# KTH-RPL/HiMo

Hardware: AMD Instinct MI355X
Metric: lidar_frames_per_sec_120k (higher is better)
Workload: dtype f16x2 (two-term split fp16, x = h + l with exact subnormals, on the matrix cores; float32 accumulate; ~22-bit products); 1 GPU; per-frame pipeline: pillarise 3 sweeps (512x512 grid) -> SeFlow++-style encoder/decoder + GRU head (random-init, self-specified: reference network source absent) -> per-point flow -> ego-motion removal + dt0 + flow2compDis -> comp_dis; points_per_frame=120000, sweeps_per_frame=3, parallelism=frames sharded x1, refined_output=False, batches_in_flight=3, matrix_arithmetic=f16x2, samples_per_backbone_launch=16, collectives=none (single process)

## Files before the change

himo_amd/csrc/pillar.hip:

```cpp
#include "himo_common.h"
#include "bf16x3.h"
#include <math.h>
#include <algorithm>
#include <vector>

namespace himo {

struct GridSpec {
    float xmin, ymin, zmin;
    float vx, vy, vz;
    float cx0, cy0, cz0;
    int W, H;
};

struct PillarArgs {
    int64_t n;
    const float* pts; int stride;
    float R[9], t[3];
    GridSpec g;
    const float* pfn_w;
    const float* pfn_scale;
    const float* pfn_shift;
    float* xyz_t;
    int* pid;
    float* offsets;
    float* image; int image_pitch;
    int image_split;
    int* cell_count;
    int* block_sum;
    int* cell_cursor;
    int* order2;
    float4* cell_rec;
    unsigned long long* occ;
};

constexpr int kMaxSweeps = 12;
struct PillarBatch { PillarArgs s[kMaxSweeps]; };

__global__ __launch_bounds__(256) void pillar_clear_kernel(PillarBatch m, int n_vec4) {
    int4* p = reinterpret_cast<int4*>(m.s[blockIdx.y].cell_count);
    for (int i = blockIdx.x * 256 + threadIdx.x; i < n_vec4; i += gridDim.x * 256) p[i] = make_int4(0, 0, 0, 0);
}

__global__ __launch_bounds__(256) void pillar_assign_kernel(PillarBatch m) {
    const PillarArgs& a = m.s[blockIdx.y];
    const int64_t i = (int64_t)blockIdx.x * 256 + threadIdx.x;
    if (i >= a.n) return;
    const float* p = a.pts + i * a.stride;
    const float x = p[0], y = p[1], z = p[2];
    const float tx = ((x * a.R[0] + y * a.R[1]) + z * a.R[2]) + a.t[0];
    const float ty = ((x * a.R[3] + y * a.R[4]) + z * a.R[5]) + a.t[1];
    const float tz = ((x * a.R[6] + y * a.R[7]) + z * a.R[8]) + a.t[2];
    a.xyz_t[i * 3] = tx; a.xyz_t[i * 3 + 1] = ty; a.xyz_t[i * 3 + 2] = tz;
    const float fx = floorf((tx - a.g.xmin) / a.g.vx);
    const float fy = floorf((ty - a.g.ymin) / a.g.vy);
    const float fz = floorf((tz - a.g.zmin) / a.g.vz);
    const bool ok = fx >= 0.f && fx < (float)a.g.W && fy >= 0.f && fy < (float)a.g.H && fz >= 0.f && fz < 1.f;
    int cell = -1;
    if (ok) {
        cell = (int)fy * a.g.W + (int)fx;
        a.order2[i] = atomicAdd(&a.cell_count[cell], 1);
    } else {
        a.offsets[i * 3] = 0.f; a.offsets[i * 3 + 1] = 0.f; a.offsets[i * 3 + 2] = 0.f;
    }
    a.pid[i] = cell;
}

constexpr int kScanBlock = 1024;

__global__ __launch_bounds__(256) void cell_scan_local_kernel(PillarBatch m) {
    int* v = m.s[blockIdx.y].cell_count;
    int* block_sum = m.s[blockIdx.y].block_sum;
    const int n = m.s[blockIdx.y].g.W * m.s[blockIdx.y].g.H;
    __shared__ int wsum[4];
    const int base = blockIdx.x * kScanBlock + threadIdx.x * 4;
    int x[4];
#pragma unroll
    for (int k = 0; k < 4; ++k) x[k] = base + k < n ? v[base + k] : 0;
    const int mine = x[0] + x[1] + x[2] + x[3];
    int incl = mine;
    const int lane = threadIdx.x & 63;
    for (int off = 1; off < 64; off <<= 1) {
        const int y = __shfl_up(incl, off, 64);
        if (lane >= off) incl += y;
    }
    if (lane == 63) wsum[threadIdx.x >> 6] = incl;
    __syncthreads();
    int run = incl - mine;
    for (int w = 0; w < (int)(threadIdx.x >> 6); ++w) run += wsum[w];
#pragma unroll
    for (int k = 0; k < 4; ++k) { if (base + k < n) v[base + k] = run; run += x[k]; }
    if (threadIdx.x == 255) block_sum[blockIdx.x] = run;
}

__global__ __launch_bounds__(1024) void cell_scan_top_kernel(PillarBatch m, int nblk) {
    int* block_sum = m.s[blockIdx.y].block_sum;
    __shared__ int part[1024];
    const int x = (int)threadIdx.x < nblk ? block_sum[threadIdx.x] : 0;
    part[threadIdx.x] = x;
    __syncthreads();
    for (int off = 1; off < 1024; off <<= 1) {
        const int y = threadIdx.x >= off ? part[threadIdx.x - off] : 0;
        __syncthreads();
        part[threadIdx.x] += y;
        __syncthreads();
    }
    if ((int)threadIdx.x < nblk) block_sum[threadIdx.x] = part[threadIdx.x] - x;
    if (threadIdx.x == 1023) block_sum[nblk] = part[1023];
}

__device__ inline int cell_offset(const PillarArgs& a, int cell);

__device__ inline int cell_offset(const PillarArgs& a, int cell) {
    const int n_cells = a.g.W * a.g.H;
    return cell >= n_cells ? a.block_sum[(n_cells + kScanBlock - 1) / kScanBlock]
                           : a.cell_count[cell] + a.block_sum[cell / kScanBlock];
}

__global__ __launch_bounds__(256) void pillar_fill_kernel(PillarBatch m) {
    const PillarArgs& a = m.s[blockIdx.y];
    const int64_t i = (int64_t)blockIdx.x * 256 + threadIdx.x;
    if (i >= a.n) return;
    const int cell = a.pid[i];
    if (cell < 0) return;
    const int at = cell_offset(a, cell) + a.order2[i];
    a.cell_rec[at] = make_float4(a.xyz_t[i * 3], a.xyz_t[i * 3 + 1], a.xyz_t[i * 3 + 2], __int_as_float((int)i));
}

constexpr int kCellsPerBlock = 8;

constexpr int kFeatCells = 64;

__device__ inline float shfl32(float v, int src) { return __shfl(v, src, 32); }
__device__ inline int shfl32(int v, int src) { return __shfl(v, src, 32); }

__global__ __launch_bounds__(256) void pillar_feature_kernel(PillarBatch m) {
    const PillarArgs& a = m.s[blockIdx.y];
    __shared__ int s_beg[kFeatCells + 1];
    __shared__ int s_list[kFeatCells];
    __shared__ int s_nlist;
    const int sub = threadIdx.x >> 5, c = threadIdx.x & 31;
    const int n_cells = a.g.W * a.g.H;
    const int cell0 = blockIdx.x * kFeatCells;
    static_assert(kFeatCells == 64, "one 64-bit occupancy word per block");
    const unsigned long long was = a.occ ? a.occ[blockIdx.x] : ~0ull;
    if (threadIdx.x <= kFeatCells) s_beg[threadIdx.x] = cell_offset(a, min(cell0 + (int)threadIdx.x, n_cells));
    __syncthreads();
    if (threadIdx.x < 64) {
        const int cnt = cell0 + (int)threadIdx.x < n_cells ? s_beg[threadIdx.x + 1] - s_beg[threadIdx.x] : 0;
        const unsigned long long one = __ballot(cnt == 1), many = __ballot(cnt > 1);
        const unsigned long long below = (1ull << threadIdx.x) - 1ull;
        if (cnt == 1) s_list[__popcll(one & below)] = threadIdx.x;
        if (cnt > 1) s_list[__popcll(one) + __popcll(many & below)] = threadIdx.x;
        if (threadIdx.x == 0) { s_nlist = __popcll(one | many); if (a.occ) a.occ[blockIdx.x] = one | many; }
    }
#pragma unroll
    for (int i = 0; i < kFeatCells / 32; ++i) {
        const int lc = i * 32 + (threadIdx.x >> 3);
        if (cell0 + lc < n_cells && s_beg[lc + 1] == s_beg[lc] && ((was >> lc) & 1ull))
            *reinterpret_cast<float4*>(a.image + (int64_t)(cell0 + lc) * a.image_pitch + (threadIdx.x & 7) * 4) = make_float4(0.f, 0.f, 0.f, 0.f);
    }
    __syncthreads();
    const int nlist = s_nlist;
    float w[9];
#pragma unroll
    for (int k = 0; k < 9; ++k) w[k] = a.pfn_w[k * 32 + c];
    const float scale = a.pfn_scale[c], shift = a.pfn_shift[c];

    for (int k = sub; k < nlist; k += kCellsPerBlock) {
        const int lc = s_list[k];
        const int cell = cell0 + lc;
        const int beg = s_beg[lc];
        const int cnt = s_beg[lc + 1] - beg;
        const int iy = cell / a.g.W, ix = cell - iy * a.g.W;
        const float ccx = (float)ix * a.g.vx + a.g.cx0, ccy = (float)iy * a.g.vy + a.g.cy0, ccz = 0.f * a.g.vz + a.g.cz0;
        const float fc = (float)cnt;
        float acc = 0.f;
        if (cnt == 1) {
            const float4 rc = a.cell_rec[beg];
            const int pj = __float_as_int(rc.w);
            const float x = rc.x, y = rc.y, z = rc.z;
            if (c == 0) a.order2[beg] = pj;
            const float f6[3] = {x - ccx, y - ccy, z - ccz};
            float v = x * w[0];
            v = fmaf(y, w[1], v); v = fmaf(z, w[2], v);
            v = fmaf(x - x, w[3], v); v = fmaf(y - y, w[4], v); v = fmaf(z - z, w[5], v);
            v = fmaf(f6[0], w[6], v); v = fmaf(f6[1], w[7], v); v = fmaf(f6[2], w[8], v);
            v = v * scale + shift;
            acc = 0.f + fmaxf(v, 0.f);
            if (c < 3) a.offsets[(int64_t)pj * 3 + c] = f6[c];
        } else if (cnt <= 32) {
            const bool have = c < cnt;
            const float4 rc = a.cell_rec[beg + (have ? c : 0)];
            const int idx = have ? __float_as_int(rc.w) : 0x7fffffff;
            const float ux = rc.x, uy = rc.y, uz = rc.z;
            int rank = 0;
            for (int j = 0; j < cnt; ++j) rank += shfl32(idx, j) < idx;
            int src = 0;
            for (int j = 0; j < cnt; ++j)
                if (shfl32(rank, j) == c) src = j;
            const int sidx = shfl32(idx, src);
            const float px = shfl32(ux, src), py = shfl32(uy, src), pz = shfl32(uz, src);
            if (have) a.order2[beg + c] = sidx;
            float sx = 0.f, sy = 0.f, sz = 0.f;
            for (int j = 0; j < cnt; ++j) { sx += shfl32(px, j); sy += shfl32(py, j); sz += shfl32(pz, j); }
            const float mx = sx / fc, my = sy / fc, mz = sz / fc;
            for (int j = 0; j < cnt; ++j) {
                const float x = shfl32(px, j), y = shfl32(py, j), z = shfl32(pz, j);
                const int pj = shfl32(sidx, j);
                const float f[9] = {x, y, z, x - mx, y - my, z - mz, x - ccx, y - ccy, z - ccz};
                float v = f[0] * w[0];
#pragma unroll
                for (int q = 1; q < 9; ++q) v = fmaf(f[q], w[q], v);
                v = v * scale + shift;
                acc += fmaxf(v, 0.f);
                if (c < 3) a.offsets[(int64_t)pj * 3 + c] = f[6 + c];
            }
        } else {
            for (int j0 = 0; j0 < cnt; j0 += 32) {
                const bool have = j0 + c < cnt;
                const int idx = have ? __float_as_int(a.cell_rec[beg + j0 + c].w) : 0x7fffffff;
                int rank = 0;
                for (int k0 = 0; k0 < cnt; k0 += 32) {
                    const int other = k0 + c < cnt ? __float_as_int(a.cell_rec[beg + k0 + c].w) : 0x7fffffff;
                    const int lim = min(32, cnt - k0);
                    for (int j = 0; j < lim; ++j) rank += shfl32(other, j) < idx;
                }
                if (have) a.order2[beg + rank] = idx;
            }
            __threadfence_block();
            float sx = 0.f, sy = 0.f, sz = 0.f;
            for (int j0 = 0; j0 < cnt; j0 += 32) {
                const bool have = j0 + c < cnt;
                const float* p = a.xyz_t + (int64_t)(have ? a.order2[beg + j0 + c] : 0) * 3;
                const float ux = have ? p[0] : 0.f, uy = have ? p[1] : 0.f, uz = have ? p[2] : 0.f;
                const int lim = min(32, cnt - j0);
                for (int j = 0; j < lim; ++j) { sx += shfl32(ux, j); sy += shfl32(uy, j); sz += shfl32(uz, j); }
            }
            const float mx = sx / fc, my = sy / fc, mz = sz / fc;
            for (int j0 = 0; j0 < cnt; j0 += 32) {
                const bool have = j0 + c < cnt;
                const int pidx = have ? a.order2[beg + j0 + c] : 0;
                const float* p = a.xyz_t + (int64_t)pidx * 3;
                const float ux = have ? p[0] : 0.f, uy = have ? p[1] : 0.f, uz = have ? p[2] : 0.f;
                const int lim = min(32, cnt - j0);
                for (int j = 0; j < lim; ++j) {
                    const float x = shfl32(ux, j), y = shfl32(uy, j), z = shfl32(uz, j);
                    const int pj = shfl32(pidx, j);
                    const float f[9] = {x, y, z, x - mx, y - my, z - mz, x - ccx, y - ccy, z - ccz};
                    float v = f[0] * w[0];
#pragma unroll
                    for (int q = 1; q < 9; ++q) v = fmaf(f[q], w[q], v);
                    v = v * scale + shift;
                    acc += fmaxf(v, 0.f);
                    if (c < 3) a.offsets[(int64_t)pj * 3 + c] = f[6 + c];
                }
            }
        }
        const float feat = acc / fc;
        if (a.image_split) {
            unsigned h, l;
            split2_rounded(feat, h, l);
            const bool odd = c & 1;
            const unsigned recv = (unsigned)__builtin_amdgcn_mov_dpp((int)(odd ? h : l), 0xB1, 0xF, 0xF, true);
            unsigned* rec = reinterpret_cast<unsigned*>(a.image + (int64_t)cell * a.image_pitch + (c & ~15));
            rec[(odd ? 8 : 0) + ((c & 15) >> 1)] = odd ? (recv | (l << 16)) : (h | (recv << 16));
        } else {
            a.image[(int64_t)cell * a.image_pitch + c] = feat;
        }
    }
}

struct PillarBwdArgs {
    GridSpec g;
    const int* cell_count; const int* block_sum; const int* order2;
    const float4* cell_rec;
    const float* xyz_t;
    const float* pfn_w; const float* pfn_scale; const float* pfn_shift;
    const float* d_image; int image_pitch;
    float* partial;
    const float* dhx; int dhx_pitch;
    float* d_b0; int b0_pitch; int group0, group1, n_groups;
    float* d_dec; int dec_pitch;
};

__device__ inline int cell_offset_b(const PillarBwdArgs& a, int cell) {
    const int n_cells = a.g.W * a.g.H;
    return cell >= n_cells ? a.block_sum[(n_cells + kScanBlock - 1) / kScanBlock]
                           : a.cell_count[cell] + a.block_sum[cell / kScanBlock];
}

__global__ __launch_bounds__(1024) void pfn_backward_reduce_kernel(const float* __restrict__ partial, int n_blocks, float* __restrict__ dw,
                                                                   int accumulate) {
    __shared__ float sh[32][32];
    const int c = threadIdx.x & 31, grp = threadIdx.x >> 5, k = blockIdx.x;
    {
        float t[4] = {0.f, 0.f, 0.f, 0.f};
        int b = grp;
        for (; b + 96 < n_blocks; b += 128) {
#pragma unroll
            for (int q = 0; q < 4; ++q) t[q] += partial[(int64_t)(b + 32 * q) * 288 + k * 32 + c];
        }
        for (; b < n_blocks; b += 32) t[0] += partial[(int64_t)b * 288 + k * 32 + c];
        sh[grp][c] = (t[0] + t[1]) + (t[2] + t[3]);
    }
    __syncthreads();
    if (grp == 0) {
        float r = sh[0][c];
#pragma unroll
        for (int g = 1; g < 32; ++g) r += sh[g][c];
        dw[k * 32 + c] = accumulate ? dw[k * 32 + c] + r : r;
    }
}

struct PfnBnArgs {
    PillarBwdArgs b;
    double* partial;
    const float* mean; const float* invstd;
    const float* coef;
};

struct PfnBnBatch { PfnBnArgs s[kMaxSweeps]; };
template <int KIND>
__global__ __launch_bounds__(256) void pfn_walk_kernel(PfnBnBatch m) {
    const PfnBnArgs& p = m.s[blockIdx.y];
    const PillarBwdArgs& a = p.b;
    constexpr int kChunk = 256;
    __shared__ int s_beg[kChunk + 1];
    __shared__ int s_list[kChunk];
    __shared__ int s_wn[4];
    constexpr bool kStats = KIND < 2;
    __shared__ double red_d[kStats ? 2 : 1][kStats ? kCellsPerBlock : 1][32];
    __shared__ float red_f[kStats ? 1 : kCellsPerBlock][kStats ? 1 : 9][32];
    const int sub = threadIdx.x >> 5, c = threadIdx.x & 31, wv = threadIdx.x >> 6, lane = threadIdx.x & 63;
    const int n_cells = a.g.W * a.g.H;
    float w[9], dw[9];
#pragma unroll
    for (int k = 0; k < 9; ++k) { w[k] = a.pfn_w[k * 32 + c]; dw[k] = 0.f; }
    const float scale = KIND ? a.pfn_scale[c] : 0.f, shift = KIND ? a.pfn_shift[c] : 0.f;
    const float mean = (KIND == 1 || KIND == 2) ? p.mean[c] : 0.f, invstd = (KIND == 1 || KIND == 2) ? p.invstd[c] : 0.f;
    const float k2 = KIND == 2 ? p.coef[c] : 0.f, k3 = KIND == 2 ? p.coef[32 + c] : 0.f;
    double s0 = 0.0, s1 = 0.0;
    for (int cell0 = blockIdx.x * kChunk; cell0 < n_cells; cell0 += gridDim.x * kChunk) {
        s_beg[threadIdx.x] = cell_offset_b(a, min(cell0 + (int)threadIdx.x, n_cells));
        if (threadIdx.x == 0) s_beg[kChunk] = cell_offset_b(a, min(cell0 + kChunk, n_cells));
        __syncthreads();
        const int my_cnt = cell0 + (int)threadIdx.x < n_cells ? s_beg[threadIdx.x + 1] - s_beg[threadIdx.x] : 0;
        const unsigned long long occ = __ballot(my_cnt > 0);
        if (lane == 0) s_wn[wv] = __popcll(occ);
        __syncthreads();
        int base = 0, nlist = 0;
#pragma unroll
        for (int u = 0; u < 4; ++u) { if (u < wv) base += s_wn[u]; nlist += s_wn[u]; }
        if (my_cnt > 0) s_list[base + __popcll(occ & ((1ull << lane) - 1ull))] = threadIdx.x;
        __syncthreads();
        for (int k = sub; k < nlist; k += kCellsPerBlock) {
            const int lc = s_list[k];
            const int cell = cell0 + lc;
            const int beg = s_beg[lc], cnt = s_beg[lc + 1] - beg;
            const float fc = (float)cnt;
            const float gi = KIND ? a.d_image[(int64_t)cell * a.image_pitch + c] / fc : 0.f;
            const int iy = cell / a.g.W, ix = cell - iy * a.g.W;
            const float ccx = (float)ix * a.g.vx + a.g.cx0, ccy = (float)iy * a.g.vy + a.g.cy0, ccz = 0.f * a.g.vz + a.g.cz0;
            auto point = [&](float x, float y, float z, float mx, float my, float mz) {
                const float f[9] = {x, y, z, x - mx, y - my, z - mz, x - ccx, y - ccy, z - ccz};
                float v = f[0] * w[0];
#pragma unroll
                for (int q = 1; q < 9; ++q) v = fmaf(f[q], w[q], v);
                if (KIND == 0) {
                    s0 += v; s1 += (double)v * v;
                } else if (KIND == 1) {
                    const float g = (v * scale + shift) > 0.f ? gi : 0.f;
                    s0 += g; s1 += (double)g * ((v - mean) * invstd);
                } else if (KIND == 2) {
                    const float g = (v * scale + shift) > 0.f ? gi : 0.f;
                    const float dy = scale * ((g - k2) - ((v - mean) * invstd) * k3);
#pragma unroll
                    for (int q = 0; q < 9; ++q) dw[q] += f[q] * dy;
                } else {
                    if ((v * scale + shift) > 0.f) {
                        const float g = gi * scale;
#pragma unroll
                        for (int q = 0; q < 9; ++q) dw[q] += f[q] * g;
                    }
                }
            };
            if (cnt == 1) {
                const float4 rc = a.cell_rec[beg];
                point(rc.x, rc.y, rc.z, rc.x, rc.y, rc.z);
                continue;
            }
            float sx = 0.f, sy = 0.f, sz = 0.f;
            float ux = 0.f, uy = 0.f, uz = 0.f;
            for (int j0 = 0; j0 < cnt; j0 += 32) {
                const bool have = j0 + c < cnt;
                const float* q = a.xyz_t + (int64_t)(have ? a.order2[beg + j0 + c] : 0) * 3;
                ux = have ? q[0] : 0.f; uy = have ? q[1] : 0.f; uz = have ? q[2] : 0.f;
                const int lim = min(32, cnt - j0);
                for (int j = 0; j < lim; ++j) { sx += shfl32(ux, j); sy += shfl32(uy, j); sz += shfl32(uz, j); }
            }
            const float mx = sx / fc, my = sy / fc, mz = sz / fc;
            for (int j0 = 0; j0 < cnt; j0 += 32) {
                if (cnt > 32) {
                    const bool have = j0 + c < cnt;
                    const float* q = a.xyz_t + (int64_t)(have ? a.order2[beg + j0 + c] : 0) * 3;
                    ux = have ? q[0] : 0.f; uy = have ? q[1] : 0.f; uz = have ? q[2] : 0.f;
                }
                const int lim = min(32, cnt - j0);
                for (int j = 0; j < lim; ++j) point(shfl32(ux, j), shfl32(uy, j), shfl32(uz, j), mx, my, mz);
            }
        }
        __syncthreads();
    }
    if (kStats) {
        red_d[0][sub][c] = s0; red_d[1][sub][c] = s1;
        __syncthreads();
        if (threadIdx.x < 64) {
            const int which = threadIdx.x >> 5;
            double t = red_d[which][0][c];
#pragma unroll
            for (int q = 1; q < kCellsPerBlock; ++q) t += red_d[which][q][c];
            p.partial[((int64_t)blockIdx.x * 2 + which) * 32 + c] = t;
        }
    } else {
#pragma unroll
        for (int k = 0; k < 9; ++k) red_f[sub][k][c] = dw[k];
        __syncthreads();
        for (int e = threadIdx.x; e < 9 * 32; e += 256) {
            float t = 0.f;
#pragma unroll
            for (int q = 0; q < kCellsPerBlock; ++q) t += red_f[q][e / 32][e % 32];
            a.partial[(int64_t)blockIdx.x * 288 + e] = t;
        }
    }
}

constexpr int kMaxGroup = 16;
struct PfnGroup { const double* partial[kMaxGroup]; const int* block_sum[kMaxGroup]; int n; };

template <int MODE>
__global__ __launch_bounds__(1024) void pfn_bn_finalize_kernel(PfnGroup grp_src, int n_blocks, int n_cells, const float* __restrict__ gamma,
                                                              const float* __restrict__ beta, float eps, float momentum,
                                                              float* __restrict__ running_mean, float* __restrict__ running_var,
                                                              float* __restrict__ out0, float* __restrict__ out1, float* __restrict__ out2,
                                                              float* __restrict__ out3, int accumulate) {
    __shared__ double sh[2][16][32];
    const int c = threadIdx.x & 31, which = (threadIdx.x >> 5) & 1, grp = threadIdx.x >> 6;
    {
        double all = 0.0;
        for (int m = 0; m < grp_src.n; ++m) {
            const double* __restrict__ partial = grp_src.partial[m];
            double t[4] = {0, 0, 0, 0};
            int b = grp;
            for (; b + 48 < n_blocks; b += 64) {
#pragma unroll
                for (int k = 0; k < 4; ++k) t[k] += partial[((int64_t)(b + 16 * k) * 2 + which) * 32 + c];
            }
            for (; b < n_blocks; b += 16) t[0] += partial[((int64_t)b * 2 + which) * 32 + c];
            all += (t[0] + t[1]) + (t[2] + t[3]);
        }
        sh[which][grp][c] = all;
    }
    __syncthreads();
    if (threadIdx.x >= 32) return;
    double count = 0.0;
    for (int m = 0; m < grp_src.n; ++m) count += (double)grp_src.block_sum[m][(n_cells + kScanBlock - 1) / kScanBlock];
    double a0 = 0.0, a1 = 0.0;
#pragma unroll
    for (int g = 0; g < 16; ++g) { a0 += sh[0][g][c]; a1 += sh[1][g][c]; }
    if (MODE == 0) {
        if (count < 1.0) {
            const float sc = gamma[c] / sqrtf((running_var ? running_var[c] : 1.f) + eps);
            out0[c] = sc; out1[c] = beta[c] - (running_mean ? running_mean[c] : 0.f) * sc; out2[c] = 0.f; out3[c] = 0.f;
            return;
        }
        const double mean = a0 / count;
        double var = a1 / count - mean * mean;
        if (var < 0.0) var = 0.0;
        const float invstd = (float)(1.0 / sqrt(var + (double)eps));
        const float sc = gamma[c] * invstd;
        out0[c] = sc;
        out1[c] = beta[c] - (float)mean * sc;
        out2[c] = (float)mean;
        out3[c] = invstd;
        if (running_mean) {
            const double unbiased = count > 1.0 ? var * count / (count - 1.0) : var;
            running_mean[c] = (float)((1.0 - (double)momentum) * (double)running_mean[c] + (double)momentum * mean);
            running_var[c] = (float)((1.0 - (double)momentum) * (double)running_var[c] + (double)momentum * unbiased);
        }
    } else {
        out0[c] = accumulate ? out0[c] + (float)a1 : (float)a1;
        out1[c] = accumulate ? out1[c] + (float)a0 : (float)a0;
        out2[c] = count > 0.0 ? (float)(a0 / count) : 0.f;
        out3[c] = count > 0.0 ? (float)(a1 / count) : 0.f;
    }
}

__global__ __launch_bounds__(256) void head_scatter_kernel(PillarBwdArgs a) {
    const int sub = threadIdx.x >> 5, c = threadIdx.x & 31;
    const int cell = blockIdx.x * kCellsPerBlock + sub;
    if (cell >= a.g.W * a.g.H) return;
    const int beg = cell_offset_b(a, cell);
    const int cnt = cell_offset_b(a, cell + 1) - beg;
    float s0 = 0.f, s1 = 0.f, s2 = 0.f, s3 = 0.f;
    for (int j = 0; j < cnt; ++j) {
        const float* r = a.dhx + (int64_t)a.order2[beg + j] * a.dhx_pitch;
        s0 += r[c]; s1 += r[32 + c]; s2 += r[64 + c]; s3 += r[96 + c];
    }
    float* b0 = a.d_b0 + (int64_t)cell * a.b0_pitch;
    for (int g = 0; g < a.n_groups; ++g) b0[g * 32 + c] = g == a.group0 ? s0 : g == a.group1 ? s1 : 0.f;
    float* dec = a.d_dec + (int64_t)cell * a.dec_pitch;
    dec[c] = s2; dec[32 + c] = s3;
}

}

using namespace himo;

static size_t ws_cells(int cells) { return round_up((size_t)cells * 4, 16); }
static size_t ws_blocks(int cells) { return round_up(((size_t)(cells + kScanBlock - 1) / kScanBlock + 1) * 4, 16); }
static size_t ws_points(int64_t n) { return round_up((size_t)(n > 0 ? n : 1) * 4, 16); }
static size_t pillar_ws(int64_t n, int cells) { return 2 * ws_cells(cells) + ws_blocks(cells) + 2 * ws_points(n) + 3 * ws_points(n); }
static size_t ws_occ(int cells) { return round_up(((size_t)cells + 63) / 64 * 8, 16); }

constexpr int64_t kMaxCells = (int64_t)kScanBlock * 1024;
static int64_t grid_cells(int grid_w, int grid_h) { return (int64_t)grid_w * (int64_t)grid_h; }
static int grid_status(int grid_w, int grid_h) {
    if (grid_w < 1 || grid_h < 1) return HIMO_ERR_INVALID_ARGUMENT;
    return grid_cells(grid_w, grid_h) > kMaxCells ? HIMO_ERR_UNSUPPORTED : HIMO_OK;
}

extern "C" size_t himo_pillar_workspace_bytes(int64_t max_points, int grid_w, int grid_h) {
    if (max_points < 0 || max_points > 0x7fffffff || grid_status(grid_w, grid_h) != HIMO_OK) return 0;
    const int cells = (int)grid_cells(grid_w, grid_h);
    return pillar_ws(max_points, cells) + 64 + ws_occ(cells);
}

extern "C" int himo_pillar_occupancy_reset(void* d_workspace, size_t workspace_bytes, int grid_w, int grid_h, void* stream) {
    if (!d_workspace || grid_w < 1 || grid_h < 1) return HIMO_ERR_INVALID_ARGUMENT;
    if (grid_status(grid_w, grid_h) != HIMO_OK) return HIMO_ERR_UNSUPPORTED;
    const int cells = (int)grid_cells(grid_w, grid_h);
    if (workspace_bytes < ws_occ(cells)) return HIMO_ERR_INVALID_ARGUMENT;
    const size_t nb = ws_occ(cells);
    HIMO_HIP(hipMemsetAsync(reinterpret_cast<char*>(d_workspace) + (workspace_bytes - nb), 0xFF, nb, (hipStream_t)stream));
    return HIMO_OK;
}

static int pillar_args(PillarArgs& a, int64_t n, const float* d_pts, int pc_stride, const float* h_transform, const float* h_range,
                       const float* h_voxel, const float* h_centre_offset, int grid_w, int grid_h, const float* d_pfn_weight,
                       const float* d_pfn_scale, const float* d_pfn_shift, float* d_xyz_t, int32_t* d_pid, float* d_offsets,
                       float* d_image, int image_pitch, void* d_workspace, size_t workspace_bytes, bool incremental = false) {
    if (n < 0 || pc_stride < 3 || grid_w < 1 || grid_h < 1 || !h_transform || !h_range || !h_voxel || !h_centre_offset)
        return HIMO_ERR_INVALID_ARGUMENT;
    if (!d_pfn_weight || !d_pfn_scale || !d_pfn_shift || !d_image || !d_workspace) return HIMO_ERR_INVALID_ARGUMENT;
    if (n > 0 && (!d_pts || !d_xyz_t || !d_pid || !d_offsets)) return HIMO_ERR_INVALID_ARGUMENT;
    if (n > 0x7fffffff || image_pitch < 32) return HIMO_ERR_UNSUPPORTED;
    if ((image_pitch & 3) || (reinterpret_cast<uintptr_t>(d_image) & 15)) return HIMO_ERR_UNSUPPORTED;
    if (grid_cells(grid_w, grid_h) > kMaxCells) return HIMO_ERR_UNSUPPORTED;
    const int cells = (int)grid_cells(grid_w, grid_h);
    if (workspace_bytes < pillar_ws(n, cells) || !aligned16(d_workspace)) return HIMO_ERR_WORKSPACE;
    if (incremental && ((workspace_bytes & 15) || workspace_bytes < pillar_ws(n, cells) + ws_occ(cells))) return HIMO_ERR_WORKSPACE;
    a = PillarArgs{};
    a.n = n; a.pts = d_pts; a.stride = pc_stride;
    for (int i = 0; i < 9; ++i) a.R[i] = h_transform[(i / 3) * 4 + (i % 3)];
    for (int i = 0; i < 3; ++i) a.t[i] = h_transform[i * 4 + 3];
    a.g.xmin = h_range[0]; a.g.ymin = h_range[1]; a.g.zmin = h_range[2];
    a.g.vx = h_voxel[0]; a.g.vy = h_voxel[1]; a.g.vz = h_voxel[2];
    a.g.cx0 = h_centre_offset[0]; a.g.cy0 = h_centre_offset[1]; a.g.cz0 = h_centre_offset[2];
    a.g.W = grid_w; a.g.H = grid_h;
    a.pfn_w = d_pfn_weight; a.pfn_scale = d_pfn_scale; a.pfn_shift = d_pfn_shift;
    a.xyz_t = d_xyz_t; a.pid = d_pid; a.offsets = d_offsets; a.image = d_image; a.image_pitch = image_pitch;
    char* ws = reinterpret_cast<char*>(d_workspace);
    a.cell_count = reinterpret_cast<int*>(ws);
    a.cell_cursor = reinterpret_cast<int*>(ws + ws_cells(cells));
    a.block_sum = reinterpret_cast<int*>(ws + 2 * ws_cells(cells));
    a.cell_rec = reinterpret_cast<float4*>(ws + 2 * ws_cells(cells) + ws_blocks(cells));
    a.order2 = reinterpret_cast<int*>(ws + 2 * ws_cells(cells) + ws_blocks(cells) + 4 * ws_points(n));
    if (incremental) a.occ = reinterpret_cast<unsigned long long*>(ws + (workspace_bytes - ws_occ(cells)));
    return HIMO_OK;
}

static int sweeps_status(int n_sweeps, const himo_sweep* h_sweeps, int image_pitch, int image_split, bool check_shared) {
    if (n_sweeps < 1 || n_sweeps > kMaxSweeps || !h_sweeps) return HIMO_ERR_INVALID_ARGUMENT;
    if (image_split && (image_pitch & 15)) return HIMO_ERR_INVALID_ARGUMENT;
    for (int i = 0; i < n_sweeps; ++i) {
        if (image_split && (reinterpret_cast<uintptr_t>(h_sweeps[i].d_image) & 63)) return HIMO_ERR_INVALID_ARGUMENT;
        for (int j = 0; check_shared && j < i; ++j)
            if (h_sweeps[j].d_workspace == h_sweeps[i].d_workspace) return HIMO_ERR_INVALID_ARGUMENT;
    }
    return HIMO_OK;
}

static int pillar_launch(const PillarBatch& m, int count, hipStream_t s) {
    const int cells = m.s[0].g.W * m.s[0].g.H;
    const int nblk = (cells + kScanBlock - 1) / kScanBlock;
    int64_t nmax = 0;
    for (int i = 0; i < count; ++i)
        if (m.s[i].n > nmax) nmax = m.s[i].n;
    {
        const int n_vec4 = (int)(ws_cells(cells) / 16);
        hipLaunchKernelGGL(pillar_clear_kernel, dim3(std::min((n_vec4 + 255) / 256, 512), count), dim3(256), 0, s, m, n_vec4);
    }
    HIMO_LAUNCH_CHECK("pillar_clear_kernel");
    const unsigned pblocks = (unsigned)((nmax + 255) / 256);
    if (nmax > 0) {
        ProfScope ps("pillar_assign_kernel", s);
        hipLaunchKernelGGL(pillar_assign_kernel, dim3(pblocks, count), dim3(256), 0, s, m);
    }
    HIMO_LAUNCH_CHECK("pillar_assign_kernel");
    {
        ProfScope ps("cell_scan_kernels", s);
        hipLaunchKernelGGL(cell_scan_local_kernel, dim3(nblk, count), dim3(256), 0, s, m);
        hipLaunchKernelGGL(cell_scan_top_kernel, dim3(1, count), dim3(1024), 0, s, m, nblk);
    }
    HIMO_LAUNCH_CHECK("cell_scan_kernels");
    if (nmax > 0) {
        ProfScope ps("pillar_fill_kernel", s);
        hipLaunchKernelGGL(pillar_fill_kernel, dim3(pblocks, count), dim3(256), 0, s, m);
    }
    HIMO_LAUNCH_CHECK("pillar_fill_kernel");
    {
        ProfScope ps("pillar_feature_kernel", s);
        hipLaunchKernelGGL(pillar_feature_kernel, dim3((cells + kFeatCells - 1) / kFeatCells, count), dim3(256), 0, s, m);
    }
    HIMO_LAUNCH_CHECK("pillar_feature_kernel");
    return HIMO_OK;
}

extern "C" int himo_pillarize(int64_t n, const float* d_pts, int pc_stride, const float* h_transform,
                              const float* h_range, const float* h_voxel, const float* h_centre_offset,
                              int grid_w, int grid_h,
                              const float* d_pfn_weight, const float* d_pfn_scale, const float* d_pfn_shift,
                              float* d_xyz_t, int32_t* d_pid, float* d_offsets, float* d_image, int image_pitch,
                              void* d_workspace, size_t workspace_bytes, void* stream) {
    PillarBatch m{};
    const int st = pillar_args(m.s[0], n, d_pts, pc_stride, h_transform, h_range, h_voxel, h_centre_offset, grid_w, grid_h, d_pfn_weight,
                               d_pfn_scale, d_pfn_shift, d_xyz_t, d_pid, d_offsets, d_image, image_pitch, d_workspace, workspace_bytes);
    if (st != HIMO_OK) return st;
    return pillar_launch(m, 1, (hipStream_t)stream);
}

extern "C" int himo_pillarize_multi(int n_sweeps, const himo_sweep* h_sweeps, const float* h_range, const float* h_voxel,
                                    const float* h_centre_offset, int grid_w, int grid_h, const float* d_pfn_weight,
                                    const float* d_pfn_scale, const float* d_pfn_shift, int image_pitch, size_t workspace_bytes,
                                    void* stream) {
    return himo_pillarize_multi_ex(n_sweeps, h_sweeps, h_range, h_voxel, h_centre_offset, grid_w, grid_h, d_pfn_weight, d_pfn_scale,
                                   d_pfn_shift, image_pitch, workspace_bytes, 0, stream);
}

extern "C" int himo_pillarize_multi_ex(int n_sweeps, const himo_sweep* h_sweeps, const float* h_range, const float* h_voxel,
                                       const float* h_centre_offset, int grid_w, int grid_h, const float* d_pfn_weight,
                                       const float* d_pfn_scale, const float* d_pfn_shift, int image_pitch, size_t workspace_bytes,
                                       int image_split, void* stream) {
    const bool incremental = (image_split & 2) != 0;
    image_split &= 1;
    const int st0 = sweeps_status(n_sweeps, h_sweeps, image_pitch, image_split, true);
    if (st0 != HIMO_OK) return st0;
    PillarBatch m{};
    for (int i = 0; i < n_sweeps; ++i) {
        const himo_sweep& w = h_sweeps[i];
        const int st = pillar_args(m.s[i], w.n, w.d_pts, w.pc_stride, w.transform, h_range, h_voxel, h_centre_offset, grid_w, grid_h,
                                   d_pfn_weight, d_pfn_scale, d_pfn_shift, w.d_xyz_t, w.d_pid, w.d_offsets, w.d_image, image_pitch,
                                   w.d_workspace, workspace_bytes, incremental);
        if (st != HIMO_OK) return st;
        m.s[i].image_split = image_split ? 1 : 0;
    }
    return pillar_launch(m, n_sweeps, (hipStream_t)stream);
}

static void carve_bwd(PillarBwdArgs& a, int64_t n, int cells, void* d_workspace) {
    char* ws = reinterpret_cast<char*>(d_workspace);
    a.cell_count = reinterpret_cast<const int*>(ws);
    a.block_sum = reinterpret_cast<const int*>(ws + 2 * ws_cells(cells));
    a.cell_rec = reinterpret_cast<const float4*>(ws + 2 * ws_cells(cells) + ws_blocks(cells));
    a.order2 = reinterpret_cast<const int*>(ws + 2 * ws_cells(cells) + ws_blocks(cells) + 4 * ws_points(n));
}

constexpr int kPfnBwdBlocks = 1024;

extern "C" size_t himo_pfn_backward_workspace_bytes(void) { return (size_t)kPfnBwdBlocks * 288 * 4 + 64; }

extern "C" int himo_pfn_backward(int64_t n, const float* h_voxel, const float* h_centre_offset, int grid_w, int grid_h,
                                 const float* d_pfn_weight, const float* d_pfn_scale, const float* d_pfn_shift,
                                 const float* d_xyz_t, const void* d_pillar_workspace, const float* d_dimage, int image_pitch,
                                 float* d_dweight, unsigned flags, void* d_workspace, size_t workspace_bytes, void* stream) {
    if (n < 0 || !h_voxel || !h_centre_offset || grid_w < 1 || grid_h < 1 || !d_pfn_weight || !d_pfn_scale || !d_pfn_shift ||
        !d_pillar_workspace || !d_dimage || !d_dweight || !d_workspace || image_pitch < 32)
        return HIMO_ERR_INVALID_ARGUMENT;
    if (n > 0 && !d_xyz_t) return HIMO_ERR_INVALID_ARGUMENT;
    if (n > 0x7fffffff || grid_status(grid_w, grid_h) != HIMO_OK) return HIMO_ERR_UNSUPPORTED;
    if (workspace_bytes < himo_pfn_backward_workspace_bytes()) return HIMO_ERR_WORKSPACE;
    PillarBwdArgs a{};
    a.g.vx = h_voxel[0]; a.g.vy = h_voxel[1]; a.g.vz = h_voxel[2];
    a.g.cx0 = h_centre_offset[0]; a.g.cy0 = h_centre_offset[1]; a.g.cz0 = h_centre_offset[2];
    a.g.W = grid_w; a.g.H = grid_h;
    carve_bwd(a, n, grid_w * grid_h, const_cast<void*>(d_pillar_workspace));
    a.xyz_t = d_xyz_t; a.pfn_w = d_pfn_weight; a.pfn_scale = d_pfn_scale; a.pfn_shift = d_pfn_shift;
    a.d_image = d_dimage; a.image_pitch = image_pitch;
    a.partial = reinterpret_cast<float*>(d_workspace);
    hipStream_t s = (hipStream_t)stream;
    {
        ProfScope ps("pfn_backward_kernel", s);
        PfnBnBatch m{};
        m.s[0].b = a;
        hipLaunchKernelGGL(pfn_walk_kernel<3>, dim3(kPfnBwdBlocks), dim3(256), 0, s, m);
    }
    hipLaunchKernelGGL(pfn_backward_reduce_kernel, dim3(9), dim3(1024), 0, s, a.partial, kPfnBwdBlocks, d_dweight, (flags & 1u) ? 1 : 0);
    HIMO_LAUNCH_CHECK("pfn_backward kernels");
    return HIMO_OK;
}

extern "C" size_t himo_pfn_bn_workspace_bytes(void) {
    return round_up((size_t)kPfnBwdBlocks * 288 * 4, 64) + (size_t)kPfnBwdBlocks * 2 * 32 * sizeof(double) + 64 * sizeof(float) + 64;
}

static int pfn_bn_args(PfnBnArgs& p, int64_t n, const float* h_voxel, const float* h_centre_offset, int grid_w, int grid_h,
                       const float* d_pfn_weight, const float* d_xyz_t, const void* d_pillar_workspace, void* d_workspace,
                       size_t workspace_bytes) {
    if (n < 0 || !h_voxel || !h_centre_offset || grid_w < 1 || grid_h < 1 || !d_pfn_weight || !d_pillar_workspace || !d_workspace)
        return HIMO_ERR_INVALID_ARGUMENT;
    if (n > 0 && !d_xyz_t) return HIMO_ERR_INVALID_ARGUMENT;
    if (n > 0x7fffffff || grid_status(grid_w, grid_h) != HIMO_OK) return HIMO_ERR_UNSUPPORTED;
    if (workspace_bytes < himo_pfn_bn_workspace_bytes() || !aligned16(d_workspace)) return HIMO_ERR_WORKSPACE;
    p = PfnBnArgs{};
    PillarBwdArgs& a = p.b;
    a.g.vx = h_voxel[0]; a.g.vy = h_voxel[1]; a.g.vz = h_voxel[2];
    a.g.cx0 = h_centre_offset[0]; a.g.cy0 = h_centre_offset[1]; a.g.cz0 = h_centre_offset[2];
    a.g.W = grid_w; a.g.H = grid_h;
    carve_bwd(a, n, grid_w * grid_h, const_cast<void*>(d_pillar_workspace));
    a.xyz_t = d_xyz_t; a.pfn_w = d_pfn_weight;
    a.partial = reinterpret_cast<float*>(d_workspace);
    p.partial = reinterpret_cast<double*>(reinterpret_cast<char*>(d_workspace) + round_up((size_t)kPfnBwdBlocks * 288 * 4, 64));
    return HIMO_OK;
}

extern "C" int himo_pfn_bn_stats_groups(int n_sweeps, int n_groups, const int64_t* h_n, const float* const* h_xyz_t,
                                        const void* const* h_pillar_workspace, const float* h_voxel, const float* h_centre_offset, int grid_w,
                                        int grid_h, const float* d_pfn_weight, const float* d_gamma, const float* d_beta, float eps,
                                        float momentum, float* d_running_mean, float* d_running_var, float* d_scale, float* d_shift,
                                        float* d_mean, float* d_invstd, void* d_workspace, size_t workspace_bytes, void* stream) {
    if (n_sweeps < 1 || n_groups < 1 || n_sweeps % n_groups || n_sweeps / n_groups > kMaxGroup || !h_n || !h_xyz_t || !h_pillar_workspace)
        return HIMO_ERR_INVALID_ARGUMENT;
    if (!d_gamma || !d_beta || !d_scale || !d_shift || !d_mean || !d_invstd || (d_running_mean == nullptr) != (d_running_var == nullptr))
        return HIMO_ERR_INVALID_ARGUMENT;
    if (grid_w < 1 || grid_h < 1) return HIMO_ERR_INVALID_ARGUMENT;
    if (n_groups > kMaxSweeps * kMaxGroup || grid_status(grid_w, grid_h) != HIMO_OK) return HIMO_ERR_UNSUPPORTED;
    const size_t one = himo_pfn_bn_workspace_bytes();
    if (workspace_bytes < one * n_sweeps) return HIMO_ERR_WORKSPACE;
    std::vector<PfnBnArgs> args((size_t)n_sweeps);
    PfnGroup groups[kMaxSweeps * kMaxGroup];
    for (int g = 0; g < n_groups; ++g) groups[g].n = 0;
    for (int i = 0; i < n_sweeps; ++i) {
        const int st = pfn_bn_args(args[i], h_n[i], h_voxel, h_centre_offset, grid_w, grid_h, d_pfn_weight, h_xyz_t[i], h_pillar_workspace[i],
                                   reinterpret_cast<char*>(d_workspace) + one * i, one);
        if (st != HIMO_OK) return st;
        PfnGroup& G = groups[i % n_groups];
        G.partial[G.n] = args[i].partial; G.block_sum[G.n] = args[i].b.block_sum; ++G.n;
    }
    hipStream_t s = (hipStream_t)stream;
    ProfScope ps("pfn_bn_stats_kernel", s);
    for (int lo = 0; lo < n_sweeps; lo += kMaxSweeps) {
        const int cnt = n_sweeps - lo < kMaxSweeps ? n_sweeps - lo : kMaxSweeps;
        PfnBnBatch m{};
        for (int j = 0; j < cnt; ++j) m.s[j] = args[lo + j];
        hipLaunchKernelGGL(pfn_walk_kernel<0>, dim3(kPfnBwdBlocks, cnt), dim3(256), 0, s, m);
    }
    for (int g = 0; g < n_groups; ++g)
        hipLaunchKernelGGL(pfn_bn_finalize_kernel<0>, dim3(1), dim3(1024), 0, s, groups[g], kPfnBwdBlocks, grid_w * grid_h, d_gamma, d_beta, eps,
                           momentum, d_running_mean, d_running_var, d_scale + 32 * g, d_shift + 32 * g, d_mean + 32 * g, d_invstd + 32 * g, 0);
    HIMO_LAUNCH_CHECK("pfn_bn_stats kernels");
    return HIMO_OK;
}

extern "C" int himo_pfn_bn_stats_multi(int n_sweeps, const int64_t* h_n, const float* const* h_xyz_t, const void* const* h_pillar_workspace,
                                       const float* h_voxel, const float* h_centre_offset, int grid_w, int grid_h,
                                       const float* d_pfn_weight, const float* d_gamma, const float* d_beta, float eps, float momentum,
                                       float* d_running_mean, float* d_running_var, float* d_scale, float* d_shift, float* d_mean,
                                       float* d_invstd, void* d_workspace, size_t workspace_bytes, void* stream) {
    if (n_sweeps > kMaxSweeps) return HIMO_ERR_INVALID_ARGUMENT;
    return himo_pfn_bn_stats_groups(n_sweeps, n_sweeps, h_n, h_xyz_t, h_pillar_workspace, h_voxel, h_centre_offset, grid_w, grid_h, d_pfn_weight,
                                    d_gamma, d_beta, eps, momentum, d_running_mean, d_running_var, d_scale, d_shift, d_mean, d_invstd,
                                    d_workspace, workspace_bytes, stream);
}

extern "C" int himo_pfn_bn_stats(int64_t n, const float* h_voxel, const float* h_centre_offset, int grid_w, int grid_h,
                                 const float* d_pfn_weight, const float* d_xyz_t, const void* d_pillar_workspace, const float* d_gamma,
                                 const float* d_beta, float eps, float momentum, float* d_running_mean, float* d_running_var,
                                 float* d_scale, float* d_shift, float* d_mean, float* d_invstd, void* d_workspace, size_t workspace_bytes,
                                 void* stream) {
    return himo_pfn_bn_stats_multi(1, &n, &d_xyz_t, &d_pillar_workspace, h_voxel, h_centre_offset, grid_w, grid_h, d_pfn_weight, d_gamma,
                                   d_beta, eps, momentum, d_running_mean, d_running_var, d_scale, d_shift, d_mean, d_invstd, d_workspace,
                                   workspace_bytes, stream);
}

extern "C" int himo_pillar_features_multi(int n_sweeps, const himo_sweep* h_sweeps, const float* h_range, const float* h_voxel,
                                          const float* h_centre_offset, int grid_w, int grid_h, const float* d_pfn_weight,
                                          const float* d_scale, const float* d_shift, int image_pitch, size_t workspace_bytes,
                                          int image_split, void* stream) {
    const bool incremental = (image_split & 2) != 0;
    image_split &= 1;
    if (!d_scale || !d_shift) return HIMO_ERR_INVALID_ARGUMENT;
    const int st0 = sweeps_status(n_sweeps, h_sweeps, image_pitch, image_split, false);
    if (st0 != HIMO_OK) return st0;
    PillarBatch m{};
    for (int i = 0; i < n_sweeps; ++i) {
        const himo_sweep& w = h_sweeps[i];
        const int st = pillar_args(m.s[i], w.n, w.d_pts, w.pc_stride, w.transform, h_range, h_voxel, h_centre_offset, grid_w, grid_h,
                                   d_pfn_weight, d_scale + 32 * i, d_shift + 32 * i, w.d_xyz_t, w.d_pid, w.d_offsets, w.d_image, image_pitch,
                                   w.d_workspace, workspace_bytes, incremental);
        if (st != HIMO_OK) return st;
        m.s[i].image_split = image_split ? 1 : 0;
    }
    hipStream_t s = (hipStream_t)stream;
    const int cells = grid_w * grid_h;
    {
        ProfScope ps("pillar_feature_kernel", s);
        hipLaunchKernelGGL(pillar_feature_kernel, dim3((cells + kFeatCells - 1) / kFeatCells, n_sweeps), dim3(256), 0, s, m);
    }
    HIMO_LAUNCH_CHECK("pillar_feature_kernel");
    return HIMO_OK;
}

extern "C" int himo_pfn_backward_bn_groups(int n_sweeps, int n_groups, const int64_t* h_n, const float* const* h_xyz_t,
                                           const void* const* h_pillar_workspace, const float* const* h_dimage, int image_pitch,
                                           const float* h_voxel, const float* h_centre_offset, int grid_w, int grid_h, const float* d_pfn_weight,
                                           const float* d_scale, const float* d_shift, const float* d_mean, const float* d_invstd,
                                           float* d_dweight, float* d_dgamma, float* d_dbeta, unsigned flags, void* d_workspace,
                                           size_t workspace_bytes, void* stream) {
    if (n_sweeps < 1 || n_groups < 1 || n_sweeps % n_groups || n_sweeps / n_groups > kMaxGroup || n_groups > kMaxSweeps * kMaxGroup ||
        n_sweeps > kMaxSweeps * kMaxGroup || !h_n || !h_xyz_t || !h_pillar_workspace || !h_dimage)
        return HIMO_ERR_INVALID_ARGUMENT;
    if (!d_scale || !d_shift || !d_mean || !d_invstd || !d_dweight || !d_dgamma || !d_dbeta || image_pitch < 32) return HIMO_ERR_INVALID_ARGUMENT;
    if (grid_w < 1 || grid_h < 1) return HIMO_ERR_INVALID_ARGUMENT;
    if (grid_status(grid_w, grid_h) != HIMO_OK) return HIMO_ERR_UNSUPPORTED;
    const size_t one = himo_pfn_bn_workspace_bytes();
    if (workspace_bytes < one * n_sweeps) return HIMO_ERR_WORKSPACE;
    static thread_local PfnBnArgs args[kMaxSweeps * kMaxGroup];
    PfnGroup groups[kMaxSweeps * kMaxGroup];
    for (int g = 0; g < n_groups; ++g) groups[g].n = 0;
    for (int i = 0; i < n_sweeps; ++i) {
        if (!h_dimage[i]) return HIMO_ERR_INVALID_ARGUMENT;
        PfnBnArgs& p = args[i];
        const int st = pfn_bn_args(p, h_n[i], h_voxel, h_centre_offset, grid_w, grid_h, d_pfn_weight, h_xyz_t[i], h_pillar_workspace[i],
                                   reinterpret_cast<char*>(d_workspace) + one * i, one);
        if (st != HIMO_OK) return st;
        const int g = i % n_groups;
        p.b.pfn_scale = d_scale + 32 * g; p.b.pfn_shift = d_shift + 32 * g; p.b.d_image = h_dimage[i]; p.b.image_pitch = image_pitch;
        p.mean = d_mean + 32 * g; p.invstd = d_invstd + 32 * g;
        p.coef = i < n_groups ? reinterpret_cast<float*>(p.partial + (size_t)kPfnBwdBlocks * 2 * 32) : args[g].coef;
        PfnGroup& G = groups[g];
        G.partial[G.n] = p.partial; G.block_sum[G.n] = p.b.block_sum; ++G.n;
    }
    hipStream_t s = (hipStream_t)stream;
    ProfScope ps("pfn_backward_kernel", s);
    auto walk = [&](auto kernel) {
        for (int lo = 0; lo < n_sweeps; lo += kMaxSweeps) {
            const int cnt = n_sweeps - lo < kMaxSweeps ? n_sweeps - lo : kMaxSweeps;
            PfnBnBatch m{};
            for (int j = 0; j < cnt; ++j) m.s[j] = args[lo + j];
            hipLaunchKernelGGL(kernel, dim3(kPfnBwdBlocks, cnt), dim3(256), 0, s, m);
        }
    };
    walk(pfn_walk_kernel<1>);
    for (int g = 0; g < n_groups; ++g) {
        float* coef = const_cast<float*>(args[g].coef);
        hipLaunchKernelGGL(pfn_bn_finalize_kernel<1>, dim3(1), dim3(1024), 0, s, groups[g], kPfnBwdBlocks, grid_w * grid_h, (const float*)nullptr,
                           (const float*)nullptr, 0.f, 0.f, (float*)nullptr, (float*)nullptr, d_dgamma, d_dbeta, coef, coef + 32,
                           (g > 0 || (flags & 1u)) ? 1 : 0);
    }
    walk(pfn_walk_kernel<2>);
    for (int i = 0; i < n_sweeps; ++i)
        hipLaunchKernelGGL(pfn_backward_reduce_kernel, dim3(9), dim3(1024), 0, s, args[i].b.partial, kPfnBwdBlocks, d_dweight,
                           (i > 0 || (flags & 1u)) ? 1 : 0);
    HIMO_LAUNCH_CHECK("pfn_backward_bn kernels");
    return HIMO_OK;
}

extern "C" int himo_pfn_backward_bn_multi(int n_sweeps, const int64_t* h_n, const float* const* h_xyz_t, const void* const* h_pillar_workspace,
                                          const float* const* h_dimage, int image_pitch, const float* h_voxel, const float* h_centre_offset,
                                          int grid_w, int grid_h, const float* d_pfn_weight, const float* d_scale, const float* d_shift,
                                          const float* d_mean, const float* d_invstd, float* d_dweight, float* d_dgamma, float* d_dbeta,
                                          unsigned flags, void* d_workspace, size_t workspace_bytes, void* stream) {
    if (n_sweeps > kMaxSweeps) return HIMO_ERR_INVALID_ARGUMENT;
    return himo_pfn_backward_bn_groups(n_sweeps, n_sweeps, h_n, h_xyz_t, h_pillar_workspace, h_dimage, image_pitch, h_voxel, h_centre_offset,
                                       grid_w, grid_h, d_pfn_weight, d_scale, d_shift, d_mean, d_invstd, d_dweight, d_dgamma, d_dbeta, flags,
                                       d_workspace, workspace_bytes, stream);
}

extern "C" int himo_pfn_backward_bn(int64_t n, const float* h_voxel, const float* h_centre_offset, int grid_w, int grid_h,
                                    const float* d_pfn_weight, const float* d_scale, const float* d_shift, const float* d_mean,
                                    const float* d_invstd, const float* d_xyz_t, const void* d_pillar_workspace, const float* d_dimage,
                                    int image_pitch, float* d_dweight, float* d_dgamma, float* d_dbeta, unsigned flags, void* d_workspace,
                                    size_t workspace_bytes, void* stream) {
    return himo_pfn_backward_bn_multi(1, &n, &d_xyz_t, &d_pillar_workspace, &d_dimage, image_pitch, h_voxel, h_centre_offset, grid_w, grid_h,
                                      d_pfn_weight, d_scale, d_shift, d_mean, d_invstd, d_dweight, d_dgamma, d_dbeta, flags, d_workspace,
                                      workspace_bytes, stream);
}

extern "C" int himo_head_scatter(int64_t n, int grid_w, int grid_h, const void* d_pillar_workspace, const float* d_dhx, int dhx_pitch,
                                 float* d_db0, int b0_pitch, int group0, int group1, int n_groups, float* d_ddec, int dec_pitch,
                                 void* stream) {
    if (n < 0 || grid_w < 1 || grid_h < 1 || !d_pillar_workspace || !d_db0 || !d_ddec || dhx_pitch < 128 || n_groups < 1 ||
        b0_pitch < 32 * n_groups || dec_pitch < 64 || (n > 0 && !d_dhx))
        return HIMO_ERR_INVALID_ARGUMENT;
    if (group0 < 0 || group0 >= n_groups || group1 < 0 || group1 >= n_groups || group0 == group1) return HIMO_ERR_INVALID_ARGUMENT;
    if (n > 0x7fffffff || grid_status(grid_w, grid_h) != HIMO_OK) return HIMO_ERR_UNSUPPORTED;
    PillarBwdArgs a{};
    a.g.W = grid_w; a.g.H = grid_h;
    carve_bwd(a, n, grid_w * grid_h, const_cast<void*>(d_pillar_workspace));
    a.dhx = d_dhx; a.dhx_pitch = dhx_pitch; a.d_b0 = d_db0; a.b0_pitch = b0_pitch; a.group0 = group0; a.group1 = group1;
    a.n_groups = n_groups; a.d_dec = d_ddec; a.dec_pitch = dec_pitch;
    hipStream_t s = (hipStream_t)stream;
    ProfScope ps("head_scatter_kernel", s);
    hipLaunchKernelGGL(head_scatter_kernel, dim3((grid_w * grid_h + kCellsPerBlock - 1) / kCellsPerBlock), dim3(256), 0, s, a);
    HIMO_LAUNCH_CHECK("head_scatter_kernel");
    return HIMO_OK;
}
```

himo_amd/seflow/model.py:

```python
from __future__ import annotations

import ctypes

import numpy as np
import torch

from .. import _lib
from . import spec

EPI_BIAS, EPI_BIAS_BN_GELU, EPI_BIAS_GELU, EPI_GRU_ZR, EPI_GRU_Q = range(5)


class ConvDesc(ctypes.Structure):
    _fields_ = [("x", ctypes.c_void_p), ("x_batch_stride", ctypes.c_int64), ("x_pitch", ctypes.c_int),
                ("w", ctypes.c_void_p), ("bias", ctypes.c_void_p), ("scale", ctypes.c_void_p), ("shift", ctypes.c_void_p),
                ("y", ctypes.c_void_p), ("y_batch_stride", ctypes.c_int64), ("y_pitch", ctypes.c_int),
                ("n", ctypes.c_int), ("h", ctypes.c_int), ("w_in", ctypes.c_int), ("cin", ctypes.c_int),
                ("cout", ctypes.c_int), ("ksize", ctypes.c_int), ("stride", ctypes.c_int), ("epilogue", ctypes.c_int),
                ("aux_in", ctypes.c_void_p), ("aux_in_pitch", ctypes.c_int),
                ("aux_out", ctypes.c_void_p), ("aux_out_pitch", ctypes.c_int), ("w_packed", ctypes.c_void_p),
                ("tile_hint", ctypes.c_int), ("packed_format", ctypes.c_int),
                ("n_outer", ctypes.c_int), ("x_outer_stride", ctypes.c_int64), ("y_outer_stride", ctypes.c_int64),
                ("act_layout", ctypes.c_int), ("range_seen", ctypes.c_void_p)]


ACT_SPLIT_IN, ACT_SPLIT_OUT = 1, 2
ACT_ACCUMULATE = 8
ACT_STUFFED_2X = 16


_lib.register({
    "himo_pillar_workspace_bytes": (ctypes.c_size_t, [ctypes.c_int64, ctypes.c_int, ctypes.c_int]),
    "himo_pillar_occupancy_reset": (ctypes.c_int, [ctypes.c_void_p, ctypes.c_size_t, ctypes.c_int, ctypes.c_int, ctypes.c_void_p]),
    "himo_pillarize": (ctypes.c_int, [ctypes.c_int64, ctypes.c_void_p, ctypes.c_int, ctypes.POINTER(ctypes.c_float),
                                      ctypes.POINTER(ctypes.c_float), ctypes.POINTER(ctypes.c_float),
                                      ctypes.POINTER(ctypes.c_float), ctypes.c_int, ctypes.c_int,
                                      ctypes.c_void_p, ctypes.c_void_p, ctypes.c_void_p,
                                      ctypes.c_void_p, ctypes.c_void_p, ctypes.c_void_p, ctypes.c_void_p,
                                      ctypes.c_int, ctypes.c_void_p, ctypes.c_size_t, ctypes.c_void_p]),
    "himo_conv2d": (ctypes.c_int, [ctypes.POINTER(ConvDesc), ctypes.c_void_p]),
    "himo_conv_packed_weight_bytes": (ctypes.c_size_t, [ctypes.c_int, ctypes.c_int, ctypes.c_int]),
    "himo_conv_pack_weights": (ctypes.c_int, [ctypes.c_void_p, ctypes.c_int, ctypes.c_int, ctypes.c_int, ctypes.c_void_p,
                                              ctypes.c_void_p]),
    "himo_upsample2x": (ctypes.c_int, [ctypes.c_void_p, ctypes.c_int, ctypes.c_int, ctypes.c_int, ctypes.c_int,
                                       ctypes.c_void_p, ctypes.c_int, ctypes.c_void_p]),
    "himo_upsample2x_batch": (ctypes.c_int, [ctypes.c_int, ctypes.c_void_p, ctypes.c_int64, ctypes.c_int, ctypes.c_int, ctypes.c_int,
                                             ctypes.c_int, ctypes.c_void_p, ctypes.c_int64, ctypes.c_int, ctypes.c_void_p]),
    "himo_upsample2x_batch_ex": (ctypes.c_int, [ctypes.c_int, ctypes.c_void_p, ctypes.c_int64, ctypes.c_int, ctypes.c_int, ctypes.c_int,
                                                ctypes.c_int, ctypes.c_void_p, ctypes.c_int64, ctypes.c_int, ctypes.c_int, ctypes.c_void_p]),
    "himo_conv_pack_weights_ex": (ctypes.c_int, [ctypes.c_void_p, ctypes.c_int, ctypes.c_int, ctypes.c_int, ctypes.c_int, ctypes.c_void_p,
                                                 ctypes.c_void_p]),
    "himo_gru_head": (ctypes.c_int, [ctypes.c_int64] + [ctypes.c_void_p] * 4 + [ctypes.c_int, ctypes.c_void_p, ctypes.c_int]
                      + [ctypes.c_void_p] * 12 + [ctypes.c_int, ctypes.c_void_p, ctypes.c_int, ctypes.c_int, ctypes.c_void_p]),
    "himo_gru_head_batch": (ctypes.c_int, [ctypes.c_int, ctypes.c_void_p, ctypes.c_int, ctypes.c_int] + [ctypes.c_void_p] * 10
                            + [ctypes.c_int, ctypes.c_int, ctypes.c_int, ctypes.c_void_p]),
    "himo_gru_head_batch_folded": (ctypes.c_int, [ctypes.c_int, ctypes.c_void_p, ctypes.c_int, ctypes.c_int] + [ctypes.c_void_p] * 8
                                   + [ctypes.c_int, ctypes.c_int, ctypes.c_int, ctypes.c_void_p]),
    "himo_gru_head_batch_guarded": (ctypes.c_int, [ctypes.c_int, ctypes.c_void_p, ctypes.c_int, ctypes.c_int] + [ctypes.c_void_p] * 10
                                    + [ctypes.c_int, ctypes.c_int, ctypes.c_int, ctypes.c_void_p, ctypes.c_void_p]),
    "himo_clear_u32": (ctypes.c_int, [ctypes.c_void_p, ctypes.c_int, ctypes.c_void_p]),
    "himo_head_gather": (ctypes.c_int, [ctypes.c_int64, ctypes.c_void_p, ctypes.c_void_p, ctypes.c_void_p, ctypes.c_void_p,
                                        ctypes.c_int, ctypes.c_void_p, ctypes.c_int, ctypes.c_void_p, ctypes.c_void_p,
                                        ctypes.c_void_p, ctypes.c_void_p, ctypes.c_int, ctypes.c_void_p]),
    "himo_head_final": (ctypes.c_int, [ctypes.c_int64, ctypes.c_void_p, ctypes.c_int, ctypes.c_void_p, ctypes.c_void_p,
                                       ctypes.c_void_p, ctypes.c_void_p, ctypes.c_void_p, ctypes.c_int, ctypes.c_void_p,
                                       ctypes.c_void_p]),
})


class HimoHeadSample(ctypes.Structure):
    _fields_ = [("n", ctypes.c_int64), ("d_pid", ctypes.c_void_p), ("d_offsets", ctypes.c_void_p), ("d_img0", ctypes.c_void_p),
                ("d_img1", ctypes.c_void_p), ("d_dec", ctypes.c_void_p), ("d_xyz_t", ctypes.c_void_p), ("d_pts", ctypes.c_void_p),
                ("pc_stride", ctypes.c_int), ("d_flow", ctypes.c_void_p)]


class HimoSweep(ctypes.Structure):
    _fields_ = [("n", ctypes.c_int64), ("d_pts", ctypes.c_void_p), ("pc_stride", ctypes.c_int), ("transform", ctypes.c_float * 16),
                ("d_xyz_t", ctypes.c_void_p), ("d_pid", ctypes.c_void_p), ("d_offsets", ctypes.c_void_p), ("d_image", ctypes.c_void_p),
                ("d_workspace", ctypes.c_void_p)]


class HimoOp(ctypes.Structure):
    _fields_ = [("kind", ctypes.c_int), ("conv", ConvDesc),
                ("up_x", ctypes.c_void_p), ("up_x_pitch", ctypes.c_int), ("up_h", ctypes.c_int), ("up_w", ctypes.c_int),
                ("up_c", ctypes.c_int), ("up_y", ctypes.c_void_p), ("up_y_pitch", ctypes.c_int),
                ("up_n", ctypes.c_int), ("up_x_batch_stride", ctypes.c_int64), ("up_y_batch_stride", ctypes.c_int64),
                ("up_out_split", ctypes.c_int)]


_lib.register({
    "himo_pillarize_multi": (ctypes.c_int, [ctypes.c_int, ctypes.c_void_p, ctypes.c_void_p, ctypes.c_void_p, ctypes.c_void_p, ctypes.c_int,
                                            ctypes.c_int, ctypes.c_void_p, ctypes.c_void_p, ctypes.c_void_p, ctypes.c_int, ctypes.c_size_t,
                                            ctypes.c_void_p]),
    "himo_pillarize_multi_ex": (ctypes.c_int, [ctypes.c_int, ctypes.c_void_p, ctypes.c_void_p, ctypes.c_void_p, ctypes.c_void_p, ctypes.c_int,
                                               ctypes.c_int, ctypes.c_void_p, ctypes.c_void_p, ctypes.c_void_p, ctypes.c_int, ctypes.c_size_t,
                                               ctypes.c_int, ctypes.c_void_p]),
    "himo_run_ops": (ctypes.c_int, [ctypes.c_void_p, ctypes.c_int, ctypes.c_uint, ctypes.c_void_p]),
    "himo_ops_release": (None, [ctypes.c_void_p]),
})


def _f32x(values):
    return (ctypes.c_float * len(values))(*[float(v) for v in values])


def fastest_tile_hint(lib, d: "ConvDesc", hints, warmup: int) -> int:
    stream = _lib.stream_handle()
    times = {}
    for _round in range(2):
        for hint in hints:
            d.tile_hint = hint
            if lib.himo_conv2d(ctypes.byref(d), stream) != 0:
                continue
            for _ in range(warmup - 1):
                lib.himo_conv2d(ctypes.byref(d), stream)
            e0, e1 = torch.cuda.Event(enable_timing=True), torch.cuda.Event(enable_timing=True)
            e0.record()
            for _ in range(3):
                lib.himo_conv2d(ctypes.byref(d), stream)
            e1.record()
            e1.synchronize()
            times[hint] = min(times.get(hint, float("inf")), e0.elapsed_time(e1))
    return min(times, key=times.get) if times else 0


class SeFlowNet:

    def __init__(self, params: dict | None = None, device=None, max_points: int = 140_000, seed: int = 0,
                 precision: str = "bf16x3", autotune: bool = True, max_batch: int = 1):
        if precision not in ("bf16x3", "f16x2", "f32"):
            raise ValueError(precision)
        if max_batch < 1:
            raise ValueError("max_batch")
        self.max_batch = max_batch
        self.precision = precision
        self.autotune = autotune
        self.keep_cell_lists = False
        self.fused_head = precision != "f32"
        self._incremental_images = True
        self.use_plan = True
        self.use_graph = True
        self._plans = {}
        self._recording = None
        self._nb = 1
        self.packed_format = 1 if precision == "f16x2" else 0
        self._split_acts = precision == "f16x2"
        self.tiles = {}
        self.lib = _lib.load()
        self.device = device if device is not None else _lib.require_gpu()
        params = spec.init_params(seed) if params is None else params
        shapes = spec.param_shapes()
        for k, shp in shapes.items():
            if k not in params or tuple(params[k].shape) != tuple(shp):
                raise KeyError(f"parameter {k} missing or of wrong shape (want {shp})")
        cpu = {k: torch.from_numpy(np.ascontiguousarray(params[k], dtype=np.float32)) for k in shapes}
        def fold(prefix, eps):
            scale = cpu[f"{prefix}.gamma"] / torch.sqrt(cpu[f"{prefix}.var"] + eps)
            return scale, cpu[f"{prefix}.beta"] - cpu[f"{prefix}.mean"] * scale
        derived = {}
        derived["pfn.scale"], derived["pfn.shift"] = fold("pfn.bn", spec.BN_EPS_PFN)
        for name, *_ in spec.ENCODER:
            derived[f"{name}.scale"], derived[f"{name}.shift"] = fold(f"{name}.bn", spec.BN_EPS)
        self.fold_decoder = True
        for a, b in (("dec1", "dec2"), ("dec2", "dec3")):
            w5, b5 = cpu[f"{a}.u5.weight"].double().numpy(), cpu[f"{a}.u5.bias"].double().numpy()
            w1, b1 = cpu[f"{b}.u1.weight"].double().numpy()[0, 0], cpu[f"{b}.u1.bias"].double().numpy()
            derived[f"{a}.u5>{b}.u1.weight"] = torch.from_numpy(np.ascontiguousarray(w5 @ w1, dtype=np.float32))
            derived[f"{a}.u5>{b}.u1.bias"] = torch.from_numpy(np.ascontiguousarray(b5 @ w1 + b1, dtype=np.float32))
        derived["head.gru.zr.weight"] = torch.cat([cpu["head.gru.z.weight"], cpu["head.gru.r.weight"]], dim=1).contiguous()
        derived["head.gru.zr.bias"] = torch.cat([cpu["head.gru.z.bias"], cpu["head.gru.r.bias"]]).contiguous()
        self.p = {k: v.to(self.device) for k, v in {**cpu, **derived}.items()}
        self.packed = {}
        if precision != "f32":
            for k, v in self.p.items():
                if k.endswith(".weight") and k != "pfn.weight" and not k.startswith("head.offset") and k != "head.dec2.weight":
                    w = v if v.dim() == 4 else v.reshape(1, 1, *v.shape)
                    ks, _, cin, cout = w.shape
                    fmt = self.packed_format
                    buf = torch.empty(int(self.lib.himo_conv_packed_weight_bytes(ks, cin, cout)), dtype=torch.uint8, device=self.device)
                    _lib.check(self.lib.himo_conv_pack_weights_ex(w.contiguous().data_ptr(), ks, cin, cout, fmt, buf.data_ptr(),
                                                                  _lib.stream_handle()), "himo_conv_pack_weights_ex")
                    self.packed[k] = buf

        self.fold_head = precision != "f32"
        if self.fold_head:
            w_off, b_off = cpu["head.offset.weight"].double().numpy(), cpu["head.offset.bias"].double().numpy()
            for name in ("head.gru.zr", "head.gru.q", "head.dec1"):
                wfull = (derived if name.endswith("zr") else cpu)[f"{name}.weight"].double().numpy()
                wh, wx = wfull[:spec.HIDDEN], wfull[spec.HIDDEN:]
                folded = np.concatenate([wh, w_off @ wx, (b_off @ wx)[None], np.zeros((12, wfull.shape[1]))], axis=0)
                wdev = torch.from_numpy(np.ascontiguousarray(folded, dtype=np.float32)).to(self.device)
                buf = torch.empty(int(self.lib.himo_conv_packed_weight_bytes(1, 144, wdev.shape[1])), dtype=torch.uint8, device=self.device)
                _lib.check(self.lib.himo_conv_pack_weights_ex(wdev.data_ptr(), 1, 144, wdev.shape[1], self.packed_format, buf.data_ptr(),
                                                              _lib.stream_handle()), "himo_conv_pack_weights_ex")
                torch.cuda.synchronize(self.device)
                self.packed[f"{name}.weight.h"] = buf

        H, W = spec.GRID
        F = spec.NUM_FRAMES
        self.H, self.W, self.F = H, W, F
        dev = self.device
        B = self.max_batch
        buf = lambda *shape: torch.empty((B, *shape), dtype=torch.float32, device=dev)
        self._B0 = buf(H * W, 32 * F)
        self.E1 = [buf(F, (H // 2) * (W // 2), 64) for _ in range(2)]
        self.F1 = buf((H // 2) * (W // 2), 64 * F)
        self.E2 = [buf(F, (H // 4) * (W // 4), 128) for _ in range(2)]
        self.F2 = buf((H // 4) * (W // 4), 128 * F)
        self.E3 = [buf(F, (H // 8) * (W // 8), 256) for _ in range(2)]
        self.F3 = buf((H // 8) * (W // 8), 256 * F)
        self.T1 = buf((H // 8) * (W // 8), 256)
        self.CAT1 = buf((H // 4) * (W // 4), 512)
        self.S = [buf((H // 4) * (W // 4), 256) for _ in range(2)]
        self.T2 = buf((H // 4) * (W // 4), 128)
        self.CAT2 = buf((H // 2) * (W // 2), 256)
        self.T = [buf((H // 2) * (W // 2), 128) for _ in range(2)]
        self.T3 = buf((H // 2) * (W // 2), 64)
        self.CAT3 = buf(H * W, 128)
        self.U = [buf(H * W, 64) for _ in range(2)]
        self.DEC = buf(H * W, 64)
        self.max_points = 0
        self._reserve_points(max_points)
        self.guard = torch.zeros(2 + self.MAX_RANGE_SLOTS, dtype=torch.int32, device=dev)
        self.nonfinite = self.guard[:1]
        self._ran_word = self.guard[-1:]
        self._range_slots = {}
        self._range = _f32x(spec.POINT_CLOUD_RANGE[:3])
        self._voxel = _f32x(spec.VOXEL_SIZE)
        r, v = spec.POINT_CLOUD_RANGE, spec.VOXEL_SIZE
        self._centre = _f32x([v[0] / 2 + r[0], v[1] / 2 + r[1], v[2] / 2 + r[2]])

    def _reserve_points(self, n: int):
        if n <= self.max_points:
            return
        dev = self.device
        self.max_points = n
        need = int(self.lib.himo_pillar_workspace_bytes(n, self.W, self.H))
        self._pt = [{"ws_slots": [torch.empty(need + 64, dtype=torch.uint8, device=dev) for _ in range(self.F)],
                     "xyz_t": torch.empty((self.F, n, 3), dtype=torch.float32, device=dev),
                     "pid": torch.empty((self.F, n), dtype=torch.int32, device=dev),
                     "offsets": torch.empty((self.F, n, 3), dtype=torch.float32, device=dev)} for _ in range(self.max_batch)]
        for st in self._pt:
            for ws in st["ws_slots"]:
                _lib.check(self.lib.himo_pillar_occupancy_reset(ws.data_ptr(), ws.numel(), self.W, self.H, _lib.stream_handle()),
                           "himo_pillar_occupancy_reset")
        self._use_sample(0)
        self.hx = torch.empty((n, 192), dtype=torch.float32, device=dev)
        self.rhx = torch.empty((n, 192), dtype=torch.float32, device=dev)
        self.zbuf = torch.empty((n, 128), dtype=torch.float32, device=dev)
        self.y1 = torch.empty((n, 32), dtype=torch.float32, device=dev)

    @property
    def incremental_images(self) -> bool:
        return self._incremental_images

    @incremental_images.setter
    def incremental_images(self, on: bool):
        on = bool(on)
        if on != self._incremental_images:
            self._incremental_images = on
            self.reset_images()

    @property
    def split_acts(self) -> bool:
        return self._split_acts

    @split_acts.setter
    def split_acts(self, on: bool):
        on = bool(on)
        if on != self._split_acts:
            self._split_acts = on
            self.drop_plan()
            self.reset_images()

    @property
    def B0(self):
        return self._B0

    @B0.setter
    def B0(self, buf):
        self._B0 = buf
        self.drop_plan()
        self.reset_images()

    MAX_RANGE_SLOTS = 63

    def clear_nonfinite(self):
        _lib.check(self.lib.himo_clear_u32(self.guard.data_ptr(), self.guard.numel(), _lib.stream_handle()), "himo_clear_u32")

    def _range_word(self, wname: str) -> int:
        k = self._range_slots.setdefault(wname, len(self._range_slots))
        if k >= self.MAX_RANGE_SLOTS:
            raise RuntimeError("more split-output layers than guard words")
        return self.guard.data_ptr() + 4 * (1 + k)

    def guard_verdict(self, words) -> str | None:
        w = [int(v) for v in words]
        if w[0] != 0:
            return "overflow"
        if w[-1] != 0 and any(w[1 + k] == 0 for k in self._range_slots.values()):
            return "underflow"
        return None

    def reset_images(self):
        for st in getattr(self, "_pt", ()):
            for ws in st["ws_slots"]:
                _lib.check(self.lib.himo_pillar_occupancy_reset(ws.data_ptr(), ws.numel(), self.W, self.H, _lib.stream_handle()),
                           "himo_pillar_occupancy_reset")

    def _use_sample(self, i: int):
        st = self._pt[i]
        self._sample = i
        self.ws_slots, self.xyz_t, self.pid, self.offsets = st["ws_slots"], st["xyz_t"], st["pid"], st["offsets"]

    def _conv(self, x, x_bs, x_pitch, wname, y, y_bs, y_pitch, n, h, w, cin, cout, ks, stride, epi, x_off=0, y_off=0,
              scale=None, shift=None, aux_in=None, aux_in_pitch=0, aux_out=None, aux_out_pitch=0, bias=None, batched=True,
              act=0):
        d = ConvDesc()
        d.x = x.data_ptr() + 4 * x_off; d.x_batch_stride = x_bs; d.x_pitch = x_pitch
        if batched and self._nb > 1:
            d.n_outer, d.x_outer_stride, d.y_outer_stride = self._nb, x.stride(0), y.stride(0)
        d.w = self.p[f"{wname}.weight"].data_ptr()
        d.bias = (self.p[f"{wname}.bias"] if bias is None else bias).data_ptr()
        d.scale = None if scale is None else scale.data_ptr()
        d.shift = None if shift is None else shift.data_ptr()
        d.y = y.data_ptr() + 4 * y_off; d.y_batch_stride = y_bs; d.y_pitch = y_pitch
        d.n, d.h, d.w_in, d.cin, d.cout, d.ksize, d.stride, d.epilogue = n, h, w, cin, cout, ks, stride, epi
        d.aux_in = None if aux_in is None else aux_in.data_ptr(); d.aux_in_pitch = aux_in_pitch
        d.aux_out = None if aux_out is None else aux_out.data_ptr(); d.aux_out_pitch = aux_out_pitch
        pk = self.packed.get(f"{wname}.weight")
        d.w_packed = None if pk is None else pk.data_ptr()
        d.packed_format = self.packed_format
        d.act_layout = act if self.split_acts else 0
        if (d.act_layout & ACT_SPLIT_OUT) and self.packed_format == 1 and epi in (EPI_BIAS, EPI_BIAS_BN_GELU):
            d.range_seen = self._range_word(wname)
        key = (n * max(d.n_outer, 1), h, w, cin, cout, ks, stride, epi, pk is not None, d.act_layout)
        if self.autotune and key not in self.tiles:
            self.tiles[key] = self._tune(d)
        d.tile_hint = self.tiles.get(key, 0)
        if self._recording is not None and epi not in (EPI_GRU_ZR, EPI_GRU_Q):
            op = HimoOp(); op.kind = 0; op.conv = d
            self._recording.append(op)
        _lib.check(self.lib.himo_conv2d(ctypes.byref(d), _lib.stream_handle()), f"himo_conv2d({wname})")

    def _tune(self, d: "ConvDesc") -> int:
        if d.epilogue in (EPI_GRU_ZR, EPI_GRU_Q):
            return 0
        cands = [(bn << 4) | mi for bn in (128, 64) if not (bn == 128 and d.cout % 128) for mi in (2, 1)]
        if d.act_layout:
            if d.stride == 2 and (d.act_layout & ACT_SPLIT_IN):
                return 0
            cands = [0x1000 | 4, 0x1000 | 2, 0x1000 | 1] if d.ksize == 1 else []
        if d.w_packed and d.ksize == 3:
            cands += [0x1000 | 4, 0x1000 | 2, 0x1000 | 1] if d.stride == 1 else [0x1000 | 2, 0x1000 | 1]
            if d.stride == 1 and (d.act_layout & ACT_SPLIT_IN) and self.packed_format == 1:
                cands.append(0x1000 | (8 if d.cout <= 64 else 12))
        if len(cands) < 2:
            return cands[0] if cands else 0
        return fastest_tile_hint(self.lib, d, cands, warmup=2)

    def _up(self, x, x_pitch, h, w, c, y, y_pitch, out_split=False):
        nb = self._nb
        osp = 1 if (out_split and self.split_acts) else 0
        if self._recording is not None:
            op = HimoOp(); op.kind = 1
            op.up_x, op.up_x_pitch, op.up_h, op.up_w, op.up_c, op.up_y, op.up_y_pitch = x.data_ptr(), x_pitch, h, w, c, y.data_ptr(), y_pitch
            op.up_n, op.up_x_batch_stride, op.up_y_batch_stride = nb, x.stride(0), y.stride(0)
            op.up_out_split = osp
            self._recording.append(op)
        _lib.check(self.lib.himo_upsample2x_batch_ex(nb, x.data_ptr(), x.stride(0) if nb > 1 else 0, x_pitch, h, w, c, y.data_ptr(),
                                                     y.stride(0) if nb > 1 else 0, y_pitch, osp, _lib.stream_handle()), "himo_upsample2x_batch_ex")

    def backbone(self, n_samples: int = 1):
        if not 1 <= n_samples <= self.max_batch:
            raise ValueError(f"n_samples must be in 1..{self.max_batch}")
        self._nb = n_samples
        if self.packed_format == 1:
            self._ran_word.fill_(1)
        plan = self._plans.get(n_samples)
        if self.use_plan and plan is not None:
            ops, n = plan
            _lib.check(self.lib.himo_run_ops(ctypes.addressof(ops), n, 1 if self.use_graph else 0, _lib.stream_handle()), "himo_run_ops")
            return self.DEC
        self._recording = [] if self.use_plan else None
        self.encoder()
        self.decoder()
        if self._recording is not None:
            rec, self._recording = self._recording, None
            self._plans[n_samples] = ((HimoOp * len(rec))(*rec), len(rec))
        return self.DEC

    def __del__(self):
        try:
            self.drop_plan()
        except Exception:
            pass

    def drop_plan(self):
        for plan in self._plans.values():
            self.lib.himo_ops_release(ctypes.addressof(plan[0]))
        self._plans = {}

    def encoder(self):
        H, W, F = self.H, self.W, self.F
        p = self.p
        stages = [("enc1", 4, 32, 64, H, W, self.E1, self.F1), ("enc2", 6, 64, 128, H // 2, W // 2, self.E2, self.F2),
                  ("enc3", 6, 128, 256, H // 4, W // 4, self.E3, self.F3)]
        src, src_bs, src_pitch = self.B0, 32, 32 * F
        for stage, n_conv, cin, cout, h, w, pingpong, catbuf in stages:
            ho, wo = h // 2, w // 2
            for i in range(n_conv):
                name = f"{stage}.{i}"
                last = i == n_conv - 1
                dst = catbuf if last else pingpong[i % 2]
                dst_bs, dst_pitch = (cout, cout * F) if last else (ho * wo * cout, cout)
                act = ACT_SPLIT_IN | ACT_SPLIT_OUT
                if i == 0:
                    self._conv(src, src_bs, src_pitch, name, dst, dst_bs, dst_pitch, F, h, w, cin, cout, 3, 2,
                               EPI_BIAS_BN_GELU, scale=p[f"{name}.scale"], shift=p[f"{name}.shift"], act=act)
                else:
                    self._conv(src, src_bs, src_pitch, name, dst, dst_bs, dst_pitch, F, ho, wo, cout, cout, 3, 1,
                               EPI_BIAS_BN_GELU, scale=p[f"{name}.scale"], shift=p[f"{name}.shift"], act=act)
                src, src_bs, src_pitch = dst, dst_bs, dst_pitch

    def decoder(self):
        H, W, F = self.H, self.W, self.F
        IN, IO = ACT_SPLIT_IN, ACT_SPLIT_IN | ACT_SPLIT_OUT
        fold = self.fold_decoder
        def block(name, coarse, c_in, ch, cw, tmp, cat, skip, skip_c, lat, out, work, nxt=None):
            if coarse is not None:
                self._conv(coarse, 0, c_in, f"{name}.u1", tmp, 0, lat, 1, 1, ch * cw, c_in, lat, 1, 1, EPI_BIAS, act=IN)
            self._up(tmp, lat, ch, cw, lat, cat, 2 * lat, out_split=True)
            self._conv(skip, 0, skip_c, f"{name}.u3", cat, 0, 2 * lat, 1, 1, 4 * ch * cw, skip_c, lat, 1, 1, EPI_BIAS, y_off=lat, act=IO)
            self._conv(cat, 0, 2 * lat, f"{name}.u4", work[0], 0, out, 1, 2 * ch, 2 * cw, 2 * lat, out, 3, 1, EPI_BIAS, act=IO)
            if fold and nxt is not None:
                nname, ntmp, nlat = nxt
                self._conv(work[0], 0, out, f"{name}.u5>{nname}.u1", ntmp, 0, nlat, 1, 2 * ch, 2 * cw, out, nlat, 3, 1, EPI_BIAS, act=IN)
                return None
            self._conv(work[0], 0, out, f"{name}.u5", work[1], 0, out, 1, 2 * ch, 2 * cw, out, out, 3, 1, EPI_BIAS, act=IO)
            return work[1]
        s = block("dec1", self.F3, 256 * F, H // 8, W // 8, self.T1, self.CAT1, self.F2, 128 * F, 256, 256, self.S, ("dec2", self.T2, 128))
        t = block("dec2", s, 256, H // 4, W // 4, self.T2, self.CAT2, self.F1, 64 * F, 128, 128, self.T, ("dec3", self.T3, 64))
        u = block("dec3", t, 128, H // 2, W // 2, self.T3, self.CAT3, self.B0, 32 * F, 64, 64, self.U)
        self._conv(u, 0, 64, "dec4", self.DEC, 0, 64, 1, H, W, 64, 64, 3, 1, EPI_BIAS, act=IN)
        return self.DEC

    def head(self, pc0: torch.Tensor, slot0: int = 1, slot1: int = 2, out: torch.Tensor | None = None) -> torch.Tensor:
        n = pc0.shape[0]
        p = self.p
        F = self.F
        B0, DEC = self.B0[self._sample], self.DEC[self._sample]
        if self.fused_head:
            flow = out if out is not None else torch.empty((n, 3), dtype=torch.float32, device=self.device)
            if flow.shape != (n, 3) or flow.dtype != torch.float32 or not flow.is_contiguous():
                raise ValueError("out must be a contiguous (N0,3) float32 tensor")
            self.head_batch([pc0], [flow], slot0, slot1, samples=[self._sample])
            return flow
        if self.split_acts:
            raise RuntimeError("the multi-launch head reads float32 pillar images: set split_acts = False (or use the fused head)")
        st = self.lib.himo_head_gather(n, self.pid[slot0].data_ptr(), self.offsets[slot0].data_ptr(),
                                       B0.data_ptr() + 4 * 32 * slot0, B0.data_ptr() + 4 * 32 * slot1, 32 * F,
                                       DEC.data_ptr(), 64, p["head.offset.weight"].data_ptr(),
                                       p["head.offset.bias"].data_ptr(), self.hx.data_ptr(), self.rhx.data_ptr(), 192,
                                       _lib.stream_handle())
        _lib.check(st, "himo_head_gather")
        for _ in range(spec.GRU_ITERS):
            self._conv(self.hx, 0, 192, "head.gru.zr", self.zbuf, 0, 128, 1, 1, n, 192, 256, 1, 1, EPI_GRU_ZR,
                       aux_in=self.hx, aux_in_pitch=192, aux_out=self.rhx, aux_out_pitch=192, batched=False)
            self._conv(self.rhx, 0, 192, "head.gru.q", self.zbuf, 0, 128, 1, 1, n, 192, 128, 1, 1, EPI_GRU_Q,
                       aux_in=self.zbuf, aux_in_pitch=128, aux_out=self.hx, aux_out_pitch=192, batched=False)
        self._conv(self.hx, 0, 192, "head.dec1", self.y1, 0, 32, 1, 1, n, 192, 32, 1, 1, EPI_BIAS_GELU, batched=False)
        flow = out if out is not None else torch.empty((n, 3), dtype=torch.float32, device=self.device)
        if flow.shape != (n, 3) or flow.dtype != torch.float32 or not flow.is_contiguous():
            raise ValueError("out must be a contiguous (N0,3) float32 tensor")
        st = self.lib.himo_head_final(n, self.y1.data_ptr(), 32, p["head.dec2.weight"].data_ptr(),
                                      p["head.dec2.bias"].data_ptr(), self.pid[slot0].data_ptr(),
                                      self.xyz_t[slot0].data_ptr(), pc0.data_ptr(), pc0.shape[1], flow.data_ptr(),
                                      _lib.stream_handle())
        _lib.check(st, "himo_head_final")
        return flow

    def forward(self, pch1, pc0, pc1, pose_h1, pose0, pose1) -> torch.Tensor:
        dev = self.device
        to_dev = lambda a: (a if isinstance(a, torch.Tensor) else torch.from_numpy(np.ascontiguousarray(a, dtype=np.float32))).to(dev, torch.float32).contiguous()
        return self.forward_device(to_dev(pch1), to_dev(pc0), to_dev(pc1), pose_h1, pose0, pose1)

    def forward_device(self, pch1, pc0, pc1, pose_h1, pose0, pose1, out: torch.Tensor | None = None) -> torch.Tensor:
        inv1 = np.linalg.inv(np.asarray(pose1, np.float64))
        T0 = inv1 @ np.asarray(pose0, np.float64)
        Th = inv1 @ np.asarray(pose_h1, np.float64)
        self._use_sample(0)
        self.pillarize_all((pch1, pc0, pc1), (Th, T0, np.eye(4)))
        self.backbone(1)
        return self.head(pc0, out=out)

    def forward_batch(self, samples, outs) -> None:
        if not 1 <= len(samples) <= self.max_batch:
            raise ValueError(f"forward_batch takes 1..{self.max_batch} samples")
        jobs = []
        for k, (pch1, pc0, pc1, pose_h1, pose0, pose1) in enumerate(samples):
            inv1 = np.linalg.inv(np.asarray(pose1, np.float64))
            jobs.append((k, (pch1, pc0, pc1), (inv1 @ np.asarray(pose_h1, np.float64), inv1 @ np.asarray(pose0, np.float64), np.eye(4))))
        self.pillarize_many(jobs)
        self.backbone(len(samples))
        if self.fused_head:
            self.head_batch([smp[1] for smp in samples], outs)
            return
        for k, smp in enumerate(samples):
            self._use_sample(k)
            self.head(smp[1], out=outs[k])

    MAX_HEAD_SAMPLES = 16

    def head_batch(self, pc0s, outs, slot0: int = 1, slot1: int = 2, samples=None) -> None:
        p, pk, F = self.p, self.packed, self.F
        samples = list(range(len(pc0s))) if samples is None else list(samples)
        for lo in range(0, len(pc0s), self.MAX_HEAD_SAMPLES):
            grp = range(lo, min(lo + self.MAX_HEAD_SAMPLES, len(pc0s)))
            arr = (HimoHeadSample * len(grp))()
            for j, i in enumerate(grp):
                k = samples[i]
                pc0, flow, st = pc0s[i], outs[i], self._pt[k]
                n = pc0.shape[0]
                if flow.shape != (n, 3) or flow.dtype != torch.float32 or not flow.is_contiguous():
                    raise ValueError("out must be a contiguous (N0,3) float32 tensor")
                h = arr[j]
                h.n, h.d_pid, h.d_offsets = n, st["pid"][slot0].data_ptr(), st["offsets"][slot0].data_ptr()
                h.d_img0, h.d_img1 = self.B0[k].data_ptr() + 4 * 32 * slot0, self.B0[k].data_ptr() + 4 * 32 * slot1
                h.d_dec, h.d_xyz_t = self.DEC[k].data_ptr(), st["xyz_t"][slot0].data_ptr()
                h.d_pts, h.pc_stride, h.d_flow = pc0.data_ptr(), pc0.shape[1], flow.data_ptr()
            tail = (p["head.dec2.weight"].data_ptr(), p["head.dec2.bias"].data_ptr(),
                    spec.GRU_ITERS, self.packed_format, 1 if self.split_acts else 0, self.nonfinite.data_ptr(), _lib.stream_handle())
            if self.fold_head:
                st = self.lib.himo_gru_head_batch_guarded(len(arr), ctypes.addressof(arr), 32 * F, 64, None, None,
                                                          pk["head.gru.zr.weight.h"].data_ptr(), p["head.gru.zr.bias"].data_ptr(),
                                                          pk["head.gru.q.weight.h"].data_ptr(), p["head.gru.q.bias"].data_ptr(),
                                                          pk["head.dec1.weight.h"].data_ptr(), p["head.dec1.bias"].data_ptr(), *tail)
            else:
                st = self.lib.himo_gru_head_batch_guarded(len(arr), ctypes.addressof(arr), 32 * F, 64,
                                                          p["head.offset.weight"].data_ptr(), p["head.offset.bias"].data_ptr(),
                                                          pk["head.gru.zr.weight"].data_ptr(), p["head.gru.zr.bias"].data_ptr(),
                                                          pk["head.gru.q.weight"].data_ptr(), p["head.gru.q.bias"].data_ptr(),
                                                          pk["head.dec1.weight"].data_ptr(), p["head.dec1.bias"].data_ptr(), *tail)
            _lib.check(st, "himo_gru_head_batch")

    def pillarize_all(self, sweeps, transforms):
        self.pillarize_many([(self._sample, sweeps, transforms)])

    MAX_SWEEPS = 12

    def pillarize_many(self, jobs):
        for _, sweeps, _ in jobs:
            for t in sweeps:
                self._reserve_points(t.shape[0])
        per_call = self.MAX_SWEEPS // self.F
        for lo in range(0, len(jobs), per_call):
            grp = jobs[lo:lo + per_call]
            arr = (HimoSweep * (len(grp) * self.F))()
            for j, (sample, sweeps, transforms) in enumerate(grp):
                st = self._pt[sample]
                for slot, (pts, T) in enumerate(zip(sweeps, transforms)):
                    w = arr[j * self.F + slot]
                    w.n, w.d_pts, w.pc_stride = pts.shape[0], pts.data_ptr(), pts.shape[1]
                    w.transform = _f32x(np.asarray(T, dtype=np.float32).reshape(-1))
                    w.d_xyz_t, w.d_pid, w.d_offsets = st["xyz_t"][slot].data_ptr(), st["pid"][slot].data_ptr(), st["offsets"][slot].data_ptr()
                    w.d_image = self.B0[sample].data_ptr() + 4 * 32 * slot
                    w.d_workspace = st["ws_slots"][slot].data_ptr()
            status = self.lib.himo_pillarize_multi_ex(len(arr), ctypes.addressof(arr), self._range, self._voxel, self._centre, self.W, self.H,
                                                      self.p["pfn.weight"].data_ptr(), self.p["pfn.scale"].data_ptr(),
                                                      self.p["pfn.shift"].data_ptr(), 32 * self.F, self._pt[0]["ws_slots"][0].numel(),
                                                      (1 if self.split_acts else 0) | (2 if self.incremental_images else 0), _lib.stream_handle())
            _lib.check(status, "himo_pillarize_multi_ex")

    def pillar_features(self, sweeps, transforms, scale: torch.Tensor, shift: torch.Tensor):
        arr = (HimoSweep * self.F)()
        st = self._pt[self._sample]
        for slot, (pts, T) in enumerate(zip(sweeps, transforms)):
            w = arr[slot]
            w.n, w.d_pts, w.pc_stride = pts.shape[0], pts.data_ptr(), pts.shape[1]
            w.transform = _f32x(np.asarray(T, dtype=np.float32).reshape(-1))
            w.d_xyz_t, w.d_pid, w.d_offsets = st["xyz_t"][slot].data_ptr(), st["pid"][slot].data_ptr(), st["offsets"][slot].data_ptr()
            w.d_image = self.B0[self._sample].data_ptr() + 4 * 32 * slot
            w.d_workspace = st["ws_slots"][slot].data_ptr()
        status = self.lib.himo_pillar_features_multi(self.F, ctypes.addressof(arr), self._range, self._voxel, self._centre, self.W, self.H,
                                                     self.p["pfn.weight"].data_ptr(), scale.data_ptr(), shift.data_ptr(), 32 * self.F,
                                                     st["ws_slots"][0].numel(),
                                                     (1 if self.split_acts else 0) | (2 if self.incremental_images else 0), _lib.stream_handle())
        _lib.check(status, "himo_pillar_features_multi")

    def pillarize_into(self, slot: int, pts: torch.Tensor, transform):
        n = pts.shape[0]
        self._reserve_points(n)
        arr = (HimoSweep * 1)()
        w = arr[0]
        w.n, w.d_pts, w.pc_stride = n, pts.data_ptr(), pts.shape[1]
        w.transform = _f32x(np.asarray(transform, dtype=np.float32).reshape(-1))
        w.d_xyz_t, w.d_pid, w.d_offsets = self.xyz_t[slot].data_ptr(), self.pid[slot].data_ptr(), self.offsets[slot].data_ptr()
        w.d_image = self.B0[self._sample].data_ptr() + 4 * 32 * slot
        w.d_workspace = self.ws_slots[slot].data_ptr()
        st = self.lib.himo_pillarize_multi_ex(1, ctypes.addressof(arr), self._range, self._voxel, self._centre, self.W, self.H,
                                              self.p["pfn.weight"].data_ptr(), self.p["pfn.scale"].data_ptr(),
                                              self.p["pfn.shift"].data_ptr(), 32 * self.F, self.ws_slots[slot].numel(),
                                              (1 if self.split_acts else 0) | (2 if self.incremental_images else 0), _lib.stream_handle())
        _lib.check(st, "himo_pillarize_multi_ex")


def conv2d_nhwc(x: torch.Tensor, weight: torch.Tensor, bias: torch.Tensor, stride: int = 1, epilogue: int = EPI_BIAS,
                scale: torch.Tensor | None = None, shift: torch.Tensor | None = None, precision: str = "f32",
                tile_hint: int = 0, act_layout: int = 0, out: torch.Tensor | None = None) -> torch.Tensor:
    lib = _lib.load()
    n, h, w, cin = x.shape
    k, _, _, cout = weight.shape
    stuffed = bool(act_layout & ACT_STUFFED_2X)
    if stuffed:
        h, w = 2 * h, 2 * w
    ho, wo = ((h + 1) // 2, (w + 1) // 2) if stride == 2 else (h, w)
    y = torch.empty((n, ho, wo, cout), dtype=torch.float32, device=x.device) if out is None else out
    d = ConvDesc()
    d.x = x.data_ptr(); d.x_batch_stride = (h * w * cin) // (4 if stuffed else 1); d.x_pitch = cin
    d.w = weight.data_ptr(); d.bias = bias.data_ptr()
    d.scale = None if scale is None else scale.data_ptr(); d.shift = None if shift is None else shift.data_ptr()
    d.y = y.data_ptr(); d.y_batch_stride = ho * wo * cout; d.y_pitch = cout
    if k == 1:
        d.n, d.h, d.w_in = n, 1, h * w
    else:
        d.n, d.h, d.w_in = n, h, w
    d.cin, d.cout, d.ksize, d.stride, d.epilogue = cin, cout, k, stride, epilogue
    d.tile_hint = tile_hint
    d.act_layout = act_layout
    if precision in ("bf16x3", "f16x2", "bf16x2") and (stride == 1 or k == 3):
        fmt = {"bf16x3": 0, "f16x2": 1, "bf16x2": 2}[precision]
        pk = torch.empty(int(lib.himo_conv_packed_weight_bytes(k, cin, cout)), dtype=torch.uint8, device=x.device)
        _lib.check(lib.himo_conv_pack_weights_ex(weight.contiguous().data_ptr(), k, cin, cout, fmt, pk.data_ptr(), _lib.stream_handle()),
                   "himo_conv_pack_weights_ex")
        d.w_packed = pk.data_ptr(); d.packed_format = fmt
    _lib.check(lib.himo_conv2d(ctypes.byref(d), _lib.stream_handle()), "himo_conv2d")
    return y


def upsample2x_nhwc(x: torch.Tensor) -> torch.Tensor:
    lib = _lib.load()
    h, w, c = x.shape
    y = torch.empty((2 * h, 2 * w, c), dtype=torch.float32, device=x.device)
    _lib.check(lib.himo_upsample2x(x.data_ptr(), c, h, w, c, y.data_ptr(), c, _lib.stream_handle()), "himo_upsample2x")
    return y
```

himo_amd/seflow/train.py:

```python
from __future__ import annotations

import ctypes
import itertools
import os

import numpy as np
import torch

from .. import _lib
from . import spec
from .model import ConvDesc, EPI_BIAS, fastest_tile_hint

c_p, c_i, c_l, c_f = ctypes.c_void_p, ctypes.c_int, ctypes.c_int64, ctypes.c_float
_lib.register({
    "himo_gru_gates_fwd": (c_i, [c_l, c_i, c_p, c_p, c_p, c_p, c_p, c_p, c_p, c_p]),
    "himo_gru_bwd1": (c_i, [c_l, c_p, c_p, c_p, c_p, c_p, c_p, c_p, c_p]),
    "himo_gru_bwd2": (c_i, [c_l, c_p, c_p, c_p, c_p, c_p, c_p, c_p, c_p, c_p]),
    "himo_gru_bwd3": (c_i, [c_l, c_p, c_p, c_p, c_p, c_p]),
    "himo_affine_gelu_fwd": (c_i, [c_l, c_i, c_p, c_i, c_p, c_p, c_p, c_i, c_p, c_i, c_p]),
    "himo_affine_gelu_bwd": (c_i, [c_l, c_i, c_p, c_i, c_p, c_i, c_p, c_p, c_i, c_p]),
    "himo_mask_rows": (c_i, [c_l, c_i, c_p, c_p, c_i, c_p]),
    "himo_wgrad_workspace_bytes_ex": (ctypes.c_size_t, [c_l, c_i, c_i]),
    "himo_linear_wgrad_ex": (c_i, [c_l, c_p, c_i, c_i, c_p, c_i, c_i, c_p, c_p, ctypes.c_uint, c_p, ctypes.c_size_t, c_p]),
    "himo_transpose": (c_i, [c_p, c_i, c_i, c_p, c_p]),
# ... 442 lines not shown

class SeFlowTrainer:

    def __init__(self, params: dict | None = None, device=None, max_points: int = 140_000, seed: int = 0,
                 precision: str = "bf16x3", batchnorm: str = "batch", batch: int = 1):
        from .model import SeFlowNet
        if precision not in ("bf16x3", "mixed", "f32"):
            raise ValueError(precision)
        if batchnorm not in ("batch", "frozen"):
            raise ValueError(batchnorm)
        if not 1 <= batch <= 16:
            raise ValueError("batch must be in 1..16")
        self.B = B = batch
        self.nb = 1
        self.precision = precision
        self.bn_batch = batchnorm == "batch"
        self.fwd_format = 1 if precision == "mixed" else 0
        self.wgrad_flags = 2 if precision == "mixed" else 0
        self.bwd3_format = 2 if precision == "mixed" else 0
        self.lib = _lib.load()
        self.device = dev = device if device is not None else _lib.require_gpu()
        params = spec.init_params(seed, fresh_bn=self.bn_batch) if params is None else params
        net = self.net = SeFlowNet(params, device=dev, max_points=1, precision="f32", autotune=False, max_batch=B)
        net.fold_decoder = False
        net.keep_cell_lists = True
        net.use_plan = False
        net.max_points = 0
        net._reserve_points(max_points)
        H, W, F = net.H, net.W, net.F
        host = {"pfn.weight": params["pfn.weight"]}
        for name, *_ in spec.ENCODER:
            host[f"{name}.weight"], host[f"{name}.bias"] = params[f"{name}.weight"], params[f"{name}.bias"]
        for name, *_ in spec.DECODER:
            for u in ("u1", "u3", "u4", "u5"):
                host[f"{name}.{u}.weight"], host[f"{name}.{u}.bias"] = params[f"{name}.{u}.weight"], params[f"{name}.{u}.bias"]
        host["dec4.weight"], host["dec4.bias"] = params["dec4.weight"], params["dec4.bias"]
        host["head.offset.weight"], host["head.offset.bias"] = params["head.offset.weight"], params["head.offset.bias"]
        for k, v in HeadTrainer.host_params(params).items():
            host[f"head.{k}"] = v
        self.bn_layers = [("pfn.bn", spec.BN_EPS_PFN, "pfn")] + [(f"{n}.bn", spec.BN_EPS, n) for n, *_ in spec.ENCODER]
        if self.bn_batch:
            for prefix, _, _ in self.bn_layers:
                host[f"{prefix}.gamma"], host[f"{prefix}.beta"] = params[f"{prefix}.gamma"], params[f"{prefix}.beta"]
        self.names = list(host)
        sizes = [int(np.prod(host[k].shape)) for k in self.names]
        pad = lambda n: (n + 3) // 4 * 4
        total = sum(pad(n) for n in sizes)
        self.flat_p = torch.zeros(total, dtype=torch.float32, device=dev)
        self.flat_g = torch.zeros_like(self.flat_p)
        self.flat_m = torch.zeros_like(self.flat_p)
        self.flat_v = torch.zeros_like(self.flat_p)
        self.p, self.g = {}, {}
        o, offsets = 0, {}
        for k, n in zip(self.names, sizes):
            shp = tuple(host[k].shape)
            self.p[k] = self.flat_p[o:o + n].view(shp)
            self.g[k] = self.flat_g[o:o + n].view(shp)
            self.p[k].copy_(torch.from_numpy(np.ascontiguousarray(host[k], dtype=np.float32)))
            offsets[k] = (o, o + pad(n))
            o += pad(n)
        self.buckets = bucket_ranges(self.names, offsets)
        self.overlap_allreduce = os.environ.get("HIMO_TRAIN_OVERLAP_ALLREDUCE", "1") != "0"
        for k in self.names:
            if not k.startswith("head.") or k.startswith("head.offset"):
                net.p[k] = self.p[k]
        hp = {k[5:]: v for k, v in self.p.items() if k.startswith("head.") and not k.startswith("head.offset")}
        hg = {k[5:]: v for k, v in self.g.items() if k.startswith("head.") and not k.startswith("head.offset")}
        self.heads = [HeadTrainer(device=dev, p=hp, g=hg, precision=precision) for _ in range(B)]
        self.head = self.heads[0]
        for h_ in self.heads[1:]:
            h_.PK, h_.PKT, h_.WT, h_.accumulate = self.head.PK, self.head.PKT, self.head.WT, True
        self.step_count = 0
        self._descs = {}
        buf = lambda *shape: torch.empty(shape, dtype=torch.float32, device=dev)
        self.layers = []
        h, w = H, W
        for i, (name, cin, cout, stride) in enumerate(spec.ENCODER):
            ho, wo = (h // 2, w // 2) if stride == 2 else (h, w)
            last = i + 1 == len(spec.ENCODER) or spec.ENCODER[i + 1][3] == 2
            self.layers.append((name, cin, cout, stride, h, w, ho, wo, last))
            h, w = ho, wo
        BF = B * F
        self.PRE = [buf(BF, L[6] * L[7], L[2]) for L in self.layers]
        self.Y = [None if L[8] else buf(BF, L[6] * L[7], L[2]) for L in self.layers]
        self.B0p, self.F1p, self.F2p, self.F3p = (t.data_ptr() for t in (net._B0, net.F1, net.F2, net.F3))
        self.dB0, self.dDEC = buf(H * W, 32 * BF), buf(B * H * W, 64)
        self.dF1, self.dF2, self.dF3 = buf(H * W // 4, 64 * BF), buf(H * W // 16, 128 * BF), buf(H * W // 64, 256 * BF)
        big = BF * (H // 2) * (W // 2) * 64
        self.dA, self.dB, self.DP, self.DP2 = buf(big), buf(big), buf(big), buf(big)
        self._Z = None
        self.TMP = buf(max(B * H * W * 128, BF * H * W * 32))
        self.dWORK = [buf(B * H * W * 64) for _ in range(2)]
        self.dCAT = buf(B * H * W * 128)
        self.dTMPc = buf(B * (H // 2) * (W // 2) * 64)
        self.dCO = [buf(B * (H // 2) * (W // 2) * 128) for _ in range(2)]
        self.WF = buf(3 * 3 * 512 * 256) if precision == "f32" else None
        ws = max(int(self.lib.himo_conv_wgrad_workspace_bytes(H // 4, W // 4, 512, 256)),
                 max(int(self.lib.himo_conv_wgrad_batch_workspace_bytes(n, h_, w_, ci, co, st)) for n, h_, w_, ci, co, st in
                     [(BF, H // 2, W // 2, 64, 64, 1), (BF, H // 4, W // 4, 128, 128, 1), (BF, H // 8, W // 8, 256, 256, 1),
                      (B, H // 4, W // 4, 512, 256, 1), (B, H // 4, W // 4, 256, 256, 1), (B, H // 2, W // 2, 256, 128, 1),
                      (B, H // 2, W // 2, 128, 128, 1), (B, H, W, 128, 64, 1), (B, H, W, 64, 64, 1),
                      (BF, H, W, 32, 64, 2), (BF, H // 2, W // 2, 64, 128, 2), (BF, H // 4, W // 4, 128, 256, 2)]),
                 int(self.lib.himo_conv_wgrad_workspace_bytes(H, W, 128, 64)),
                 int(self.lib.himo_conv_wgrad_workspace_bytes(H // 2, W // 2, 256, 128)),
                 int(self.lib.himo_wgrad_workspace_bytes_ex(B * H * W, 96, 64)),
                 int(self.lib.himo_wgrad_workspace_bytes_ex(B * H * W // 4, 192, 128)),
                 int(self.lib.himo_wgrad_workspace_bytes_ex(B * H * W // 16, 384, 256)),
                 int(self.lib.himo_wgrad_workspace_bytes_ex(max_points, 192, 256)),
                 int(self.lib.himo_pfn_backward_workspace_bytes()))
        ws = max(ws, BF * int(self.lib.himo_pfn_bn_workspace_bytes()),
                 max(int(self.lib.himo_bn_workspace_bytes(BF * L[6] * L[7], L[2])) for L in self.layers))
        self.ws = torch.empty(ws + 64, dtype=torch.uint8, device=dev)
        self.overlap_wgrad = self._side_streams_built = os.environ.get("HIMO_TRAIN_SIDE_STREAM", "1") != "0"
        self.tune_tiles = os.environ.get("HIMO_TRAIN_TUNE_TILES", "1") != "0"
        self._tile_hints = {}
        if self.tune_tiles and precision != "f32":
            net.autotune = True
            net._tune = lambda d: self._tune_tile(d) if (d.ksize == 3 and d.w_packed) else 0
        self.side, self.side2, self.side3 = _lib.shared_streams(dev, "side", 3)
        self.ws_side = torch.empty(ws + 64, dtype=torch.uint8, device=dev)
        self.overlap_decoder = self.overlap_wgrad and os.environ.get("HIMO_TRAIN_SIDE_STREAM_DECODER", "1") != "0"
        self._skip_done = []
        self.ws_side2 = torch.empty(ws + 64, dtype=torch.uint8, device=dev) if self.overlap_decoder else None
        for h_ in self.heads:
            h_.wgrad_stream = self.side2 if self.overlap_decoder else None
        if self.overlap_decoder:
            self.TMP3 = buf(H * W * 32 * BF)
            self.dIN = {"dec3": buf(B * H * W * 64), "dec2": buf(B * H * W // 4 * 128), "dec1": buf(B * H * W // 16 * 256)}
            self.dCATb = {"dec3": self.dCAT, "dec2": buf(B * H * W // 4 * 256), "dec1": buf(B * H * W // 16 * 512)}
            self.dTMPb = {"dec3": self.dTMPc, "dec2": buf(B * H * W // 16 * 128), "dec1": buf(B * H * W // 64 * 256)}
        self.zero_bias = torch.zeros(1024, dtype=torch.float32, device=dev)
        self._bn_bias_zeroed = set()
        self.wgrad_leave_room = True
        self.bn_from_x = True
        self._bn_fwd_from_x = True
        self.stuffed_dgrad = True
        self.bn_mean = torch.zeros((len(self.layers), 256), dtype=torch.float32, device=dev)
        self.bn_invstd = torch.zeros((len(self.layers), 256), dtype=torch.float32, device=dev)
        self.pfn_scale, self.pfn_shift, self.pfn_mean, self.pfn_invstd = (torch.zeros((F, 32), dtype=torch.float32, device=dev) for _ in range(4))
        self._dres = [None] * B
        self._bn_folded = True
        self.packed = {}
        if precision != "f32":
            for k in self.names:
                v = self.p[k]
                if k.endswith(".weight") and v.dim() == 4:
                    ks, _, cin, cout = v.shape
                    self.packed[k] = torch.empty(int(self.lib.himo_conv_packed_weight_bytes(ks, cin, cout)), dtype=torch.uint8, device=dev)
            self.packed_flip = {k: torch.empty_like(v) for k, v in self.packed.items()}
            self._flip_ptrs = {v.data_ptr() for v in self.packed_flip.values()}
            net.packed = self.packed
            net.packed_format = self.fwd_format
            jobs = []
            for k, buf in self.packed.items():
                ks, _, cin, cout = self.p[k].shape
                jobs.append((self.p[k], ks, cin, cout, self.fwd_format, 0, buf))
                jobs.append((self.p[k], ks, cin, cout, self.bwd3_format, 1, self.packed_flip[k]))
            jobs += self.head.weight_jobs()
            for h_ in self.heads:
                h_.external_pack = True
            table = np.zeros(len(jobs), dtype=np.dtype([("w", "<u8"), ("packed", "<u8"), ("ksize", "<i4"), ("cin", "<i4"), ("cout", "<i4"),
                                                        ("format", "<i4"), ("flip", "<i4"), ("first_block", "<i4")]))
            blocks = 0
            for i, (w, ks, cin, cout, fmt, flip, dst) in enumerate(jobs):
                nb = int(self.lib.himo_weight_job_blocks(ks, cin, cout, flip))
                if nb < 1:
                    raise ValueError(f"weight job {i}: {ks}x{ks} {cin}->{cout}")
                table[i] = (w.data_ptr(), dst.data_ptr(), ks, cin, cout, fmt, flip, blocks)
                blocks += nb
            self._jobs = torch.from_numpy(table.view(np.uint8).copy()).to(dev)
            self._n_jobs, self._job_blocks = len(jobs), blocks
        self._repack()

    def _repack(self):
        if self.precision == "f32":
            return
        _lib.check(self.lib.himo_weight_prepare_batch(self._jobs.data_ptr(), self._n_jobs, self._job_blocks, _lib.stream_handle()),
                   "weight_prepare_batch")

    def _conv(self, x, x_bs, x_pitch, w, bias, y, y_bs, y_pitch, n, h, wd, cin, cout, ks, stride=1, packed=None, fmt=0, accumulate=False,
              stuffed=False):
        if packed is not None and self.precision != "f32" and packed in self._flip_ptrs:
            fmt = self.bwd3_format
        key = (x, x_bs, x_pitch, w, bias, y, y_bs, y_pitch, n, h, wd, cin, cout, ks, stride, packed, fmt, accumulate, stuffed)
        d = self._descs.get(key)
        if d is None:
            d = ConvDesc()
            d.x, d.x_batch_stride, d.x_pitch = x, x_bs, x_pitch
            d.w = w; d.bias = bias
            d.w_packed = packed; d.packed_format = fmt
            d.y, d.y_batch_stride, d.y_pitch = y, y_bs, y_pitch
            d.n, d.h, d.w_in, d.cin, d.cout, d.ksize, d.stride, d.epilogue = n, h, wd, cin, cout, ks, stride, EPI_BIAS
            d.act_layout = (8 if accumulate else 0) | (16 if stuffed else 0)
            if self.tune_tiles and ks == 3 and packed is not None and self.precision != "f32":
                tkey = (n, h, wd, cin, cout, stride, fmt, bool(accumulate), bool(stuffed))
                if tkey not in self._tile_hints:
                    self._tile_hints[tkey] = self._tune_tile(d)
                d.tile_hint = self._tile_hints[tkey]
            if len(self._descs) > 4096:
                self._descs.clear()
            self._descs[key] = d
        _lib.check(self.lib.himo_conv2d(ctypes.byref(d), _lib.stream_handle()), "himo_conv2d(train)")

    TILE_HINTS = (0, 0x1004, 0x1002, 0x1001, 0x1005, 0x1006, 0x1009, 0x100A)

    def _tune_tile(self, d) -> int:
        t = ConvDesc.from_buffer_copy(d)
        if t.act_layout & 8:
            ho, wo = ((t.h + 1) // 2, (t.w_in + 1) // 2) if t.stride == 2 else (t.h, t.w_in)
            if t.n * ho * wo * t.cout > self.TMP.numel():
                return 0
            t.act_layout &= ~8
            t.y, t.y_batch_stride, t.y_pitch = self.TMP.data_ptr(), ho * wo * t.cout, t.cout
        return fastest_tile_hint(self.lib, t, self.TILE_HINTS, warmup=1)

    def _wgrad3_batch(self, n, x, x_bs, x_pitch, h, w, cin, dy, dy_bs, dy_pitch, cout, gname, stride=1, ws=None):
        flags = self.wgrad_flags | self._beside_flag(ws)
        ws = self.ws if ws is None else ws
        _lib.check(self.lib.himo_conv3x3_wgrad_batch(n, x, x_bs, x_pitch, h, w, cin, dy, dy_bs, dy_pitch, cout, stride,
                                                     self.g[gname].data_ptr(), flags, ws.data_ptr(), ws.numel(),
                                                     _lib.stream_handle()), "conv3x3_wgrad_batch")

    def _beside_flag(self, ws) -> int:
        return 4 if (self.wgrad_leave_room and ws is not None and ws is not self.ws) else 0

    def _wgrad3(self, x, x_pitch, h, w, cin, dy, dy_pitch, cout, stride, gname, acc, ws=None):
        if stride == 1 and not acc:
            return self._wgrad3_batch(1, x, 0, x_pitch, h, w, cin, dy, 0, dy_pitch, cout, gname, ws=ws)
        ws = self.ws if ws is None else ws
        _lib.check(self.lib.himo_conv3x3_wgrad(x, x_pitch, h, w, cin, dy, dy_pitch, cout, stride, self.g[gname].data_ptr(),
                                               1 if acc else 0, ws.data_ptr(), ws.numel(), _lib.stream_handle()), "conv3x3_wgrad")

    def _wgrad3_bias(self, n, x, x_bs, x_pitch, h, w, cin, dy, dy_bs, dy_pitch, cout, wname, bname, ws=None):
        w_ = self.ws if ws is None else ws
        if self.wgrad_flags & 2:
            st = self.lib.himo_conv3x3_wgrad_batch_bias(n, x, x_bs, x_pitch, h, w, cin, dy, dy_bs, dy_pitch, cout, 1, self.g[wname].data_ptr(),
                                                        self.g[bname].data_ptr(), self.wgrad_flags | self._beside_flag(ws), w_.data_ptr(), w_.numel(),
                                                        _lib.stream_handle())
            if st == 0:
                return
        if n == 1:
            self._wgrad3(x, x_pitch, h, w, cin, dy, dy_pitch, cout, 1, wname, False, ws=ws)
        else:
            self._wgrad3_batch(n, x, x_bs, x_pitch, h, w, cin, dy, dy_bs, dy_pitch, cout, wname, ws=ws)
        if n > 1 and (dy_bs != h * w * dy_pitch):
            raise ValueError("bias gradient over a batch needs consecutive images")
        self._colsum(n * h * w, dy, dy_pitch, cout, bname, ws=ws)

    def set_side_streams(self, on: bool):
        self.overlap_wgrad = bool(on) and self._side_streams_built
        self.overlap_decoder = self.overlap_wgrad and self.ws_side2 is not None
        for h_ in self.heads:
            h_.wgrad_stream = self.side2 if self.overlap_decoder else None

    def _beside(self, fn):
        if not self.overlap_decoder:
            return fn(self.ws)
        ready = torch.cuda.Event()
        ready.record(torch.cuda.current_stream(self.device))
        with torch.cuda.stream(self.side2):
            self.side2.wait_event(ready)
            fn(self.ws_side2)

    def _zero_bn_bias(self, name):
        if name not in self._bn_bias_zeroed:
            self.g[f"{name}.bias"].zero_()
            self._bn_bias_zeroed.add(name)

    def _colsum(self, rows, z, pitch, cout, gname, acc=False, ws=None):
        self._bn_bias_zeroed.discard(gname.rsplit(".", 1)[0])
        ws = self.ws if ws is None else ws
        _lib.check(self.lib.himo_colsum(rows, z, pitch, cout, self.g[gname].data_ptr(), 1 if acc else 0, ws.data_ptr(),
                                        ws.numel(), _lib.stream_handle()), "colsum")

    def _wgrad1(self, rows, x, x_pitch, cin, dz, z_pitch, cout, name, ws=None, acc=False):
        ws = self.ws if ws is None else ws
        _lib.check(self.lib.himo_linear_wgrad_ex(rows, x, x_pitch, cin, dz, z_pitch, cout, self.g[f"{name}.weight"].data_ptr(),
                                                 self.g[f"{name}.bias"].data_ptr(), self.wgrad_flags | (1 if acc else 0), ws.data_ptr(), ws.numel(),
                                                 _lib.stream_handle()), "linear_wgrad")

    def _flip(self, name, ks, cin, cout):
        if self.precision != "f32":
            return self.p[f"{name}.weight"].data_ptr(), self.packed_flip[f"{name}.weight"].data_ptr()
        _lib.check(self.lib.himo_weight_flip(self.p[f"{name}.weight"].data_ptr(), ks, cin, cout, self.WF.data_ptr(), _lib.stream_handle()), "flip")
        return self.WF.data_ptr(), None

    def _add2d(self, rows, cols, b, b_pitch, y, y_pitch):
        _lib.check(self.lib.himo_add2d(rows, cols, b, b_pitch, y, y_pitch, _lib.stream_handle()), "add2d")

    def fold_batchnorm(self):
        net = self.net
        for prefix, eps, out in self.bn_layers:
            ch = net.p[f"{prefix}.gamma"].numel()
            _lib.check(self.lib.himo_bn_fold(ch, net.p[f"{prefix}.gamma"].data_ptr(), net.p[f"{prefix}.beta"].data_ptr(),
                                             net.p[f"{prefix}.mean"].data_ptr(), net.p[f"{prefix}.var"].data_ptr(), eps,
                                             net.p[f"{out}.scale"].data_ptr(), net.p[f"{out}.shift"].data_ptr(), _lib.stream_handle()), "bn_fold")
        self._bn_folded = True

    def forward(self, pch1, pc0, pc1, pose_h1, pose0, pose1, training: bool = True, after_pillarize=None) -> torch.Tensor:
        return self.forward_batch([(pch1, pc0, pc1, pose_h1, pose0, pose1)], training=training, after_pillarize=after_pillarize)[0]

    def _pillar_stage(self, jobs, constants=None):
        net, lib, F = self.net, self.lib, self.net.F
        from .model import HimoSweep, _f32x
        pitch = 32 * F * self.B
        flat = [(b, slot, pts, T) for b, sweeps, transforms in jobs for slot, (pts, T) in enumerate(zip(sweeps, transforms))]
        flags = (1 if net.split_acts else 0) | (2 if net.incremental_images else 0)
        for lo in range(0, len(flat), net.MAX_SWEEPS):
            grp = flat[lo:lo + net.MAX_SWEEPS]
            arr = (HimoSweep * len(grp))()
            for j, (b, slot, pts, T) in enumerate(grp):
                st, w = net._pt[b], arr[j]
                w.n, w.d_pts, w.pc_stride = pts.shape[0], pts.data_ptr(), pts.shape[1]
                w.transform = _f32x(np.asarray(T, dtype=np.float32).reshape(-1))
                w.d_xyz_t, w.d_pid, w.d_offsets = st["xyz_t"][slot].data_ptr(), st["pid"][slot].data_ptr(), st["offsets"][slot].data_ptr()
                w.d_image = self.B0p + 4 * 32 * (b * F + slot)
                w.d_workspace = st["ws_slots"][slot].data_ptr()
            ws_bytes = net._pt[0]["ws_slots"][0].numel()
            if constants is None:
                _lib.check(lib.himo_pillarize_multi_ex(len(arr), ctypes.addressof(arr), net._range, net._voxel, net._centre, net.W, net.H,
                                                       self.p["pfn.weight"].data_ptr(), net.p["pfn.scale"].data_ptr(), net.p["pfn.shift"].data_ptr(),
                                                       pitch, ws_bytes, flags, _lib.stream_handle()), "himo_pillarize_multi_ex")
            else:
                _lib.check(lib.himo_pillar_features_multi(len(arr), ctypes.addressof(arr), net._range, net._voxel, net._centre, net.W, net.H,
                                                          self.p["pfn.weight"].data_ptr(), constants[0].data_ptr() + 4 * 32 * lo,
                                                          constants[1].data_ptr() + 4 * 32 * lo, pitch, ws_bytes, flags, _lib.stream_handle()),
                           "himo_pillar_features_multi")

    def _per_sweep(self, t: torch.Tensor) -> torch.Tensor:
        return t if self.nb == 1 else t.repeat(self.nb, 1)

    def forward_batch(self, samples, training: bool = True, after_pillarize=None) -> list:
        net, lib, s = self.net, self.lib, _lib.stream_handle
        dev = self.device
        nb = len(samples)
        if not 1 <= nb <= self.B:
            raise ValueError(f"forward_batch takes 1..{self.B} samples (SeFlowTrainer(batch=...))")
        self.nb = nb
        batch = self.bn_batch and training
        self._fwd_batch = batch
        self._bn_fwd_from_x = self.bn_from_x
        if self.bn_batch and not training and not self._bn_folded:
            self.fold_batchnorm()
        to_dev = lambda a: (a if isinstance(a, torch.Tensor) else torch.from_numpy(np.ascontiguousarray(a, dtype=np.float32))).to(dev, torch.float32).contiguous()
        jobs, self.n_pts_b = [], []
        for b_, (pch1, pc0, pc1, pose_h1, pose0, pose1) in enumerate(samples):
            pch1, pc0, pc1 = to_dev(pch1), to_dev(pc0), to_dev(pc1)
            inv1 = np.linalg.inv(np.asarray(pose1, np.float64))
            jobs.append((b_, (pch1, pc0, pc1), (inv1 @ np.asarray(pose_h1, np.float64), inv1 @ np.asarray(pose0, np.float64), np.eye(4))))
            self.n_pts_b.append([pch1.shape[0], pc0.shape[0], pc1.shape[0]])
            for t in (pch1, pc0, pc1):
                net._reserve_points(t.shape[0])
        self.n_pts = self.n_pts_b[0]
        self._fwd_jobs = jobs
        self._pillar_stage(jobs)
        if after_pillarize is not None:
            after_pillarize()
        F, B = net.F, self.B
        NI = nb * F
        if batch:
            self._bn_folded = False
            g, b = net.p["pfn.bn.gamma"].data_ptr(), net.p["pfn.bn.beta"].data_ptr()
            rm, rv = net.p["pfn.bn.mean"].data_ptr(), net.p["pfn.bn.var"].data_ptr()
            ns, xs, wss = self._pfn_sweep_arrays()
            _lib.check(lib.himo_pfn_bn_stats_groups(NI, F, ns, xs, wss, net._voxel, net._centre, net.W, net.H, self.p["pfn.weight"].data_ptr(),
                                                    g, b, spec.BN_EPS_PFN, BN_MOMENTUM, rm, rv, self.pfn_scale.data_ptr(),
                                                    self.pfn_shift.data_ptr(), self.pfn_mean.data_ptr(), self.pfn_invstd.data_ptr(),
                                                    self.ws.data_ptr(), self.ws.numel(), s()), "pfn_bn_stats_groups")
            self._pillar_stage(jobs, constants=(self._per_sweep(self.pfn_scale), self._per_sweep(self.pfn_shift)))
        src, src_bs, src_pitch = self.B0p, 32, 32 * F * B
        cat = {64: self.F1p, 128: self.F2p, 256: self.F3p}
        self.inputs = []
        for li, (name, cin, cout, stride, h, w, ho, wo, last) in enumerate(self.layers):
            self.inputs.append((src, src_bs, src_pitch))
            pre = self.PRE[li]
            pk = self.packed.get(f"{name}.weight")
            self._conv(src, src_bs, src_pitch, self.p[f"{name}.weight"].data_ptr(), self.p[f"{name}.bias"].data_ptr(),
                       pre.data_ptr(), ho * wo * cout, cout, NI, h, w, cin, cout, 3, stride, packed=None if pk is None else pk.data_ptr(),
                       fmt=self.fwd_format)
            if last:
                y_ptr, y_bs, y_pitch = cat[cout], cout, cout * F * B
            else:
                y_ptr, y_bs, y_pitch = self.Y[li].data_ptr(), ho * wo * cout, cout
            if batch:
                pfx = f"{name}.bn"
                _lib.check(lib.himo_bn_train_fwd(NI, ho * wo, cout, pre.data_ptr(), ho * wo * cout, cout, net.p[f"{pfx}.gamma"].data_ptr(),
                                                 net.p[f"{pfx}.beta"].data_ptr(), spec.BN_EPS, BN_MOMENTUM, net.p[f"{pfx}.mean"].data_ptr(),
                                                 net.p[f"{pfx}.var"].data_ptr(), self.bn_mean[li].data_ptr(), self.bn_invstd[li].data_ptr(),
                                                 None if self.bn_from_x else pre.data_ptr(), ho * wo * cout, cout, y_ptr, y_bs, y_pitch,
                                                 self.ws.data_ptr(), self.ws.numel(), s()), "bn_train_fwd")
            else:
                sc, sh = net.p[f"{name}.scale"].data_ptr(), net.p[f"{name}.shift"].data_ptr()
                if last:
                    for i in range(NI):
                        _lib.check(lib.himo_affine_gelu_fwd(ho * wo, cout, pre[i].data_ptr(), cout, sc, sh, pre[i].data_ptr(), cout,
                                                            y_ptr + 4 * cout * i, y_pitch, s()), "affine_gelu_fwd")
                else:
                    _lib.check(lib.himo_affine_gelu_fwd(NI * ho * wo, cout, pre.data_ptr(), cout, sc, sh, pre.data_ptr(), cout,
                                                        y_ptr, cout, s()), "affine_gelu_fwd")
            src, src_bs, src_pitch = y_ptr, y_bs, y_pitch
        self._decoder_fwd()
        H, W = net.H, net.W
        out = []
        self.n0_b = []
        for b_, (_, (pch1, pc0, pc1), _) in enumerate(jobs):
            st, head = net._pt[b_], self.heads[b_]
            n0 = pc0.shape[0]
            self.n0_b.append(n0)
            img0, img1 = self.B0p + 4 * 32 * (b_ * F + 1), self.B0p + 4 * 32 * (b_ * F + 2)
            dec = net.DEC.data_ptr() + 4 * b_ * H * W * 64
            if self.precision != "f32" and n0 > 0:
                out.append(head.forward_fused(n0, st["pid"][1].data_ptr(), st["offsets"][1].data_ptr(), img0, img1, 32 * F * B, dec, 64,
                                              self.p["head.offset.weight"].data_ptr(), self.p["head.offset.bias"].data_ptr()))
                continue
            hx0 = torch.empty((n0, 192), dtype=torch.float32, device=dev)
            rhx = torch.empty((n0, 192), dtype=torch.float32, device=dev)
            _lib.check(lib.himo_head_gather(n0, st["pid"][1].data_ptr(), st["offsets"][1].data_ptr(), img0, img1, 32 * F * B, dec, 64,
                                            self.p["head.offset.weight"].data_ptr(), self.p["head.offset.bias"].data_ptr(),
                                            hx0.data_ptr(), rhx.data_ptr(), 192, s()), "himo_head_gather")
            res = head.forward(hx0)
            _lib.check(lib.himo_mask_rows(n0, 4, st["pid"][1].data_ptr(), res.data_ptr(), 4, s()), "mask_rows")
            out.append(res)
        self.n0 = self.n0_b[0]
        return out

    def _fwd_conv(self, x, x_bs, x_pitch, name, y, y_bs, y_pitch, h, w, cin, cout, ks):
        pk = self.packed.get(f"{name}.weight")
        self._conv(x, x_bs, x_pitch, self.p[f"{name}.weight"].data_ptr(), self.p[f"{name}.bias"].data_ptr(), y, y_bs, y_pitch, self.nb, h, w,
                   cin, cout, ks, 1, packed=None if pk is None else pk.data_ptr(), fmt=self.fwd_format)

    def _decoder_fwd(self):
        net, nb = self.net, self.nb
        H, W, F, B = net.H, net.W, net.F, self.B
        conv = self._fwd_conv

        def block(name, coarse, coarse_bs, coarse_pitch, c_in, ch, cw, tmp, cat, skip, skip_c, lat, out, work):
            Pc, P = ch * cw, 4 * ch * cw
            conv(coarse, coarse_bs, coarse_pitch, f"{name}.u1", tmp.data_ptr(), Pc * lat, lat, 1, Pc, c_in, lat, 1)
            _lib.check(self.lib.himo_upsample2x_batch_ex(nb, tmp.data_ptr(), Pc * lat if nb > 1 else 0, lat, ch, cw, lat, cat.data_ptr(),
                                                         P * 2 * lat if nb > 1 else 0, 2 * lat, 0, _lib.stream_handle()), "himo_upsample2x_batch_ex")
            conv(skip, skip_c, skip_c * B, f"{name}.u3", cat.data_ptr() + 4 * lat, P * 2 * lat, 2 * lat, 1, P, skip_c, lat, 1)
            conv(cat.data_ptr(), P * 2 * lat, 2 * lat, f"{name}.u4", work[0].data_ptr(), P * out, out, 2 * ch, 2 * cw, 2 * lat, out, 3)
            conv(work[0].data_ptr(), P * out, out, f"{name}.u5", work[1].data_ptr(), P * out, out, 2 * ch, 2 * cw, out, out, 3)
            return work[1]
        s_ = block("dec1", self.F3p, 256 * F, 256 * F * B, 256 * F, H // 8, W // 8, net.T1, net.CAT1, self.F2p, 128 * F, 256, 256, net.S)
        t_ = block("dec2", s_.data_ptr(), (H // 4) * (W // 4) * 256, 256, 256, H // 4, W // 4, net.T2, net.CAT2, self.F1p, 64 * F, 128, 128, net.T)
        u_ = block("dec3", t_.data_ptr(), (H // 2) * (W // 2) * 128, 128, 128, H // 2, W // 2, net.T3, net.CAT3, self.B0p, 32 * F, 64, 64, net.U)
        conv(u_.data_ptr(), H * W * 64, 64, "dec4", net.DEC.data_ptr(), H * W * 64, 64, H, W, 64, 64, 3)

    def _block_bwd(self, name, coarse, coarse_bs, coarse_pitch, c_in, ch, cw, skip, skip_c, lat, out, cat, work0, d_out, d_in,
                   d_coarse, dc_bs, dc_pitch, d_skip, skip_acc):
        lib, s = self.lib, _lib.stream_handle
        nb, B = self.nb, self.B
        h2, w2 = 2 * ch, 2 * cw
        P, Pc = h2 * w2, ch * cw
        zb = self.zero_bias.data_ptr()
        if self.overlap_decoder:
            d_in = self.dIN[name].data_ptr()
        dcat = (self.dCATb[name] if self.overlap_decoder else self.dCAT).data_ptr()
        dtmp = (self.dTMPb[name] if self.overlap_decoder else self.dTMPc).data_ptr()
        self._beside(lambda ws: self._wgrad3_bias(nb, work0.data_ptr(), P * out, out, h2, w2, out, d_out, P * out, out, out,
                                                  f"{name}.u5.weight", f"{name}.u5.bias", ws=ws))
        wf, wp = self._flip(f"{name}.u5", 3, out, out)
        self._conv(d_out, P * out, out, wf, zb, d_in, P * out, out, nb, h2, w2, out, out, 3, packed=wp)
        self._beside(lambda ws: self._wgrad3_bias(nb, cat.data_ptr(), P * 2 * lat, 2 * lat, h2, w2, 2 * lat, d_in, P * out, out, out,
                                                  f"{name}.u4.weight", f"{name}.u4.bias", ws=ws))
        wf, wp = self._flip(f"{name}.u4", 3, 2 * lat, out)
        self._conv(d_in, P * out, out, wf, zb, dcat, P * 2 * lat, 2 * lat, nb, h2, w2, out, 2 * lat, 3, packed=wp)
        def u3_weight_gradient(ws):
            for b_ in range(nb):
                self._wgrad1(P, skip + 4 * skip_c * b_, skip_c * B, skip_c, dcat + 4 * (b_ * P * 2 * lat + lat), 2 * lat, lat, f"{name}.u3", ws=ws,
                             acc=b_ > 0)
        self._beside(u3_weight_gradient)
        wt, wp = self._flip(f"{name}.u3", 1, skip_c, lat)

        def skip_gradient(tmp):
            if skip_acc and wp is not None:
                self._conv(dcat + 4 * lat, P * 2 * lat, 2 * lat, wt, zb, d_skip, skip_c, skip_c * B, nb, 1, P, lat, skip_c, 1, packed=wp, accumulate=True)
            elif skip_acc:
                self._conv(dcat + 4 * lat, P * 2 * lat, 2 * lat, wt, zb, tmp, skip_c, skip_c * B, nb, 1, P, lat, skip_c, 1, packed=wp)
                self._add2d(P, skip_c * nb, tmp, skip_c * B, d_skip, skip_c * B)
            else:
                self._conv(dcat + 4 * lat, P * 2 * lat, 2 * lat, wt, zb, d_skip, skip_c, skip_c * B, nb, 1, P, lat, skip_c, 1, packed=wp)
        if self.overlap_decoder and self.precision != "f32":
            ready = torch.cuda.Event()
            ready.record(torch.cuda.current_stream(self.device))
            with torch.cuda.stream(self.side3):
                self.side3.wait_event(ready)
                skip_gradient(self.TMP3.data_ptr())
                ev = torch.cuda.Event()
                ev.record(self.side3)
            self._skip_done.append(ev)
        else:
            skip_gradient(self.TMP.data_ptr())
        for b_ in range(nb):
            _lib.check(lib.himo_upsample2x_bwd(dcat + 4 * b_ * P * 2 * lat, 2 * lat, ch, cw, lat, dtmp + 4 * b_ * Pc * lat, lat, s()), "upsample2x_bwd")
        if coarse_bs == Pc * c_in and coarse_pitch == c_in:
            self._beside(lambda ws: self._wgrad1(nb * Pc, coarse, c_in, c_in, dtmp, lat, lat, f"{name}.u1", ws=ws))
        else:
            def u1_weight_gradient(ws):
                for b_ in range(nb):
                    self._wgrad1(Pc, coarse + 4 * coarse_bs * b_, coarse_pitch, c_in, dtmp + 4 * b_ * Pc * lat, lat, lat, f"{name}.u1", ws=ws, acc=b_ > 0)
            self._beside(u1_weight_gradient)
        wt, wp = self._flip(f"{name}.u1", 1, c_in, lat)
        self._conv(dtmp, Pc * lat, lat, wt, zb, d_coarse, dc_bs, dc_pitch, nb, 1, Pc, lat, c_in, 1, packed=wp)

    def backward(self, dres: torch.Tensor):
        return self.backward_batch([dres])

    def _bucket_done(self, exchange, k: int, streams):
        if exchange is None:
            return
        events = []
        for st in streams:
            ev = torch.cuda.Event()
            ev.record(st)
            events.append(ev)
        exchange.launch(k, events)

    def backward_batch(self, dres_list, exchange: BucketedAllReduce | None = None):
        net, lib, s = self.net, self.lib, _lib.stream_handle
        H, W, F, B, nb = net.H, net.W, net.F, self.B, self.nb
        if len(dres_list) != nb:
            raise ValueError(f"backward_batch: {len(dres_list)} gradients for the {nb} samples of the last forward pass")
        NI = nb * F
        for b_ in range(nb):
            st, head, n0 = net._pt[b_], self.heads[b_], self.n0_b[b_]
            dres = self._dres[b_] = dres_list[b_].contiguous().clone()
            _lib.check(lib.himo_mask_rows(n0, 4, st["pid"][1].data_ptr(), dres.data_ptr(), 4, s()), "mask_rows")
            head.accumulate = b_ > 0
            dhx0 = head.backward(dres)
            self._beside(lambda ws, n0=n0, st=st, dhx0=dhx0, acc=1 if b_ > 0 else 0: _lib.check(lib.himo_linear_wgrad_ex(
                n0, st["offsets"][1].data_ptr(), 3, 3, dhx0.data_ptr() + 4 * 128, 192, 64, self.g["head.offset.weight"].data_ptr(),
                self.g["head.offset.bias"].data_ptr(), acc, ws.data_ptr(), ws.numel(), s()), "offset wgrad"))
            _lib.check(lib.himo_head_scatter(n0, W, H, st["ws_slots"][1].data_ptr(), dhx0.data_ptr(), 192, self.dB0.data_ptr() + 4 * 32 * F * b_,
                                             32 * F * B, 1, 2, F, self.dDEC.data_ptr() + 4 * b_ * H * W * 64, 64, s()), "head_scatter")
        zb = self.zero_bias.data_ptr()
        P, P2, P4, P8 = H * W, (H // 2) * (W // 2), (H // 4) * (W // 4), (H // 8) * (W // 8)
        u = net.U[1]
        self._beside(lambda ws: self._wgrad3_bias(nb, u.data_ptr(), P * 64, 64, H, W, 64, self.dDEC.data_ptr(), P * 64, 64, 64, "dec4.weight", "dec4.bias", ws=ws))
        d_u = self.dWORK[0].data_ptr()
        wf, wp = self._flip("dec4", 3, 64, 64)
        self._conv(self.dDEC.data_ptr(), P * 64, 64, wf, zb, d_u, P * 64, 64, nb, H, W, 64, 64, 3, packed=wp)
        d_t, d_s = self.dCO[0].data_ptr(), self.dCO[1].data_ptr()
        self._block_bwd("dec3", net.T[1].data_ptr(), P2 * 128, 128, 128, H // 2, W // 2, self.B0p, 32 * F, 64, 64, net.CAT3, net.U[0], d_u,
                        self.dWORK[1].data_ptr(), d_t, P2 * 128, 128, self.dB0.data_ptr(), True)
        self._block_bwd("dec2", net.S[1].data_ptr(), P4 * 256, 256, 256, H // 4, W // 4, self.F1p, 64 * F, 128, 128, net.CAT2, net.T[0], d_t,
                        self.dWORK[1].data_ptr(), d_s, P4 * 256, 256, self.dF1.data_ptr(), False)
        self._block_bwd("dec1", self.F3p, 256 * F, 256 * F * B, 256 * F, H // 8, W // 8, self.F2p, 128 * F, 256, 256, net.CAT1, net.S[0], d_s,
                        self.dWORK[1].data_ptr(), self.dF3.data_ptr(), 256 * F, 256 * F * B, self.dF2.data_ptr(), False)
        dcat = {256: self.dF3, 128: self.dF2, 64: self.dF1, 32: self.dB0}
        dy = None
        main = torch.cuda.current_stream(self.device)
        self._bucket_done(exchange, 0, (main, self.side2))
        while self._skip_done:
            main.wait_event(self._skip_done.pop())
        side_done = {}
        for li in range(len(self.layers) - 1, -1, -1):
            name, cin, cout, stride, h, w, ho, wo, last = self.layers[li]
            pre = self.PRE[li]
            sc = net.p[f"{name}.scale"].data_ptr()
            dp = (self.DP2 if (self.overlap_wgrad and li & 1) else self.DP).data_ptr()
            if li + 2 in side_done:
                main.wait_event(side_done.pop(li + 2))
            if self._fwd_batch:
                pfx = f"{name}.bn"
                dy_ptr, dy_bs, dy_pitch = (dcat[cout].data_ptr(), cout, cout * F * B) if last else (dy, ho * wo * cout, cout)
                if not self._bn_fwd_from_x:
                    _lib.check(lib.himo_bn_train_bwd(NI, ho * wo, cout, dy_ptr, dy_bs, dy_pitch, pre.data_ptr(), ho * wo * cout, cout,
                                                     net.p[f"{pfx}.gamma"].data_ptr(), net.p[f"{pfx}.beta"].data_ptr(), self.bn_invstd[li].data_ptr(),
                                                     dp, ho * wo * cout, cout, self.g[f"{pfx}.gamma"].data_ptr(), self.g[f"{pfx}.beta"].data_ptr(),
                                                     0, self.ws.data_ptr(), self.ws.numel(), s()), "bn_train_bwd")
                else:
                    _lib.check(lib.himo_bn_train_bwd_x(NI, ho * wo, cout, dy_ptr, dy_bs, dy_pitch, pre.data_ptr(), ho * wo * cout, cout,
                                                       net.p[f"{pfx}.gamma"].data_ptr(), net.p[f"{pfx}.beta"].data_ptr(), self.bn_mean[li].data_ptr(),
                                                       self.bn_invstd[li].data_ptr(), dp, ho * wo * cout, cout, self.g[f"{pfx}.gamma"].data_ptr(),
                                                       self.g[f"{pfx}.beta"].data_ptr(), 0, self.ws.data_ptr(), self.ws.numel(), s()), "bn_train_bwd_x")
            elif last:
                src = dcat[cout]
                for i in range(NI):
                    _lib.check(lib.himo_affine_gelu_bwd(ho * wo, cout, src.data_ptr() + 4 * cout * i, cout * F * B, pre[i].data_ptr(), cout, sc,
                                                        dp + 4 * i * ho * wo * cout, cout, s()), "affine_gelu_bwd")
            else:
                _lib.check(lib.himo_affine_gelu_bwd(NI * ho * wo, cout, dy, cout, pre.data_ptr(), cout, sc, dp, cout, s()), "affine_gelu_bwd")
            x, x_bs, x_pitch = self.inputs[li]
            if self.overlap_wgrad:
                ready = torch.cuda.Event()
                ready.record(main)
                with torch.cuda.stream(self.side):
                    self.side.wait_event(ready)
                    if not self._fwd_batch:
                        self._colsum(NI * ho * wo, dp, cout, cout, f"{name}.bias", ws=self.ws_side)
                    self._wgrad3_batch(NI, x, x_bs, x_pitch, h, w, cin, dp, ho * wo * cout, cout, cout, f"{name}.weight", stride, ws=self.ws_side)
                    side_done[li] = torch.cuda.Event()
                    side_done[li].record(self.side)
                if self._fwd_batch:
                    self._zero_bn_bias(name)
            else:
                if not self._fwd_batch:
                    self._colsum(NI * ho * wo, dp, cout, cout, f"{name}.bias")
                else:
                    self._zero_bn_bias(name)
                self._wgrad3_batch(NI, x, x_bs, x_pitch, h, w, cin, dp, ho * wo * cout, cout, cout, f"{name}.weight", stride)
            if name == "enc2.0":
                self._bucket_done(exchange, 1, (main, self.side))
            wf, wp = self._flip(name, 3, cin, cout)
            if stride == 2:
                dst = dcat[cin]
                if self.bwd3_format == 2 and self.stuffed_dgrad and h % 2 == 0 and w % 2 == 0:
                    self._conv(dp, ho * wo * cout, cout, wf, zb, dst.data_ptr(), cin, cin * F * B, NI, h, w, cout, cin, 3, packed=wp, accumulate=True,
# ... 239 lines not shown
```

include/himo_amd.h:

```cpp
#ifndef HIMO_AMD_H
#define HIMO_AMD_H

#include <stddef.h>
#include <stdint.h>

#ifdef __cplusplus
extern "C" {
#endif

#define HIMO_ABI_VERSION 1

typedef enum himo_status {
    HIMO_OK = 0,
    HIMO_ERR_INVALID_ARGUMENT = 1,
    HIMO_ERR_EMPTY_FRAME = 2,
    HIMO_ERR_WORKSPACE = 3,
    HIMO_ERR_SINGULAR_POSE = 4,
    HIMO_ERR_HIP = 5,
    HIMO_ERR_UNSUPPORTED = 6
} himo_status;

#define HIMO_FLAG_F32_CHAIN 0x1u
#define HIMO_FLAG_RAW 0x2u
#define HIMO_FLAG_SCANIA 0x4u
#define HIMO_FLAG_POSE_IS_EGO 0x8u

int himo_abi_version(void);
size_t himo_abi_sizeof(const char* struct_name);
const char* himo_status_string(int status);
const char* himo_last_hip_error(void);

void himo_prof_enable(int on);
void himo_prof_filter(const char* substr);
void himo_prof_reset(void);
size_t himo_prof_summary(char* buf, size_t cap);
int himo_mfma_sustained_tflops(int kind, int zero_operands, double min_seconds, double* tflops, void* stream);

size_t himo_compdis_workspace_bytes(int n_frames);

int himo_compdis_batch(int n_frames, int64_t total_points,
                       const int64_t* d_offsets, const double* d_pose0, const double* d_pose1,
                       const float* d_pc0, int pc_stride, const float* d_flow, const float* d_lidar_dt,
                       double sensor_dt, unsigned flags,
                       float* d_comp_dis, float* d_refined,
                       uint8_t* d_eval_mask, const uint8_t* d_gm0, const uint8_t* d_flow_is_valid,
                       const float* h_mask_bounds, float close_distance,
                       void* d_workspace, size_t workspace_bytes, void* stream);

int himo_compdis_frame(int64_t n_points, const double* h_pose0, const double* h_pose1,
                       const float* d_pc0, int pc_stride, const float* d_flow, const float* d_lidar_dt,
                       double sensor_dt, unsigned flags,
                       float* d_comp_dis, float* d_refined,
                       void* d_workspace, size_t workspace_bytes, void* stream);

#define HIMO_GT_HAS_CATEGORY 0x1u
#define HIMO_GT_HAS_INSTANCE 0x2u
#define HIMO_GT_MAX_COLUMNS 10

size_t himo_gt_body_bytes(int64_t n_points, unsigned columns);
size_t himo_gt_column_starts(int64_t n_points, unsigned columns, int64_t* h_starts);

int himo_compdis_gt_batch(int n_frames, int64_t total_points,
                          const int64_t* d_offsets, const double* d_pose0, const double* d_pose1,
                          const float* d_pc0, int pc_stride, const float* d_flow, const float* d_lidar_dt,
                          double sensor_dt, unsigned flags,
                          const uint8_t* d_gm0, const uint8_t* d_flow_is_valid,
                          const uint8_t* d_category, const uint32_t* d_instance, unsigned columns,
                          const float* h_mask_bounds, float close_distance,
                          const int64_t* d_body_offsets, uint8_t* d_body,
                          void* d_workspace, size_t workspace_bytes, void* stream);

int himo_flow2compdis(int64_t n, const void* d_flow, const void* d_dt0, double sensor_dt,
                      int dtype_flags, void* d_out, void* stream);
int himo_refine_pts(int64_t n, const float* d_pc, int pc_stride, const void* d_ds,
                    int dtype_is_f64, void* d_out, void* stream);
int himo_ego_pts_mask(int64_t n, const float* d_pts, int pc_stride, const float* h_bounds,
                      uint8_t* d_out, void* stream);
int himo_dt0(int64_t n, const float* d_lidar_dt, float* d_dt0, void* d_workspace, void* stream);

int himo_nn_search(int n_segments, const int64_t* d_q_offsets, const int64_t* d_r_offsets,
                   int64_t nq, int64_t nr, const void* d_q, const void* d_r, int dtype_is_f64,
                   void* d_dist2, int32_t* d_idx, void* stream);
int himo_sqrt_inplace(int64_t n, void* d_values, int dtype_is_f64, void* stream);

typedef struct himo_instance_record {
    int32_t frame;
    int32_t group;
    int64_t instance;
    int64_t num_pts;
    double vel;
    double dis;
    double mpe;
    double cham;
} himo_instance_record;

#define HIMO_EVAL_FLOW 0
#define HIMO_EVAL_COMPDIS 1
#define HIMO_EVAL_RAW 2
#define HIMO_EVAL_SCORE 3

#define HIMO_EVAL_DIRECT 4
#define HIMO_EVAL_DIRECT_EST_IS_DIS 0x100u

size_t himo_eval_workspace_bytes(int n_frames, int64_t total_points, int64_t max_records);

int himo_eval_instances(int n_frames, int64_t total_points,
                        const int64_t* d_offsets, const double* d_pose0, const double* d_pose1,
                        const float* d_pc0, int pc_stride, const void* d_gt, const void* d_est,
                        const float* d_lidar_dt, const uint8_t* d_category, const int64_t* d_instance,
                        const uint8_t* d_eval_mask, const uint8_t* h_class_lut,
                        double sensor_dt, int mode, unsigned flags,
                        himo_instance_record* d_records, int64_t max_records, int64_t* d_counts,
                        void* d_workspace, size_t workspace_bytes, void* stream);

#define HIMO_SEG_MAX_RESULTS 8
int himo_seg_confusion(int64_t total_points, const uint8_t* d_gt, const uint8_t* const* h_pred, int n_results,
                       const uint8_t* d_seg_valid, const uint8_t* h_class_lut, int64_t* d_conf, void* stream);

int himo_box_label_batch(int n_frames, int64_t total_points, const int64_t* h_offsets, const int64_t* d_offsets,
                         const double* d_ego1_SE3_ego0, const float* d_pc, int n_boxes, const int* h_box_offsets,
                         const int* d_box_offsets, const double* d_box_geom, const float* d_box_flow,
                         const uint8_t* d_box_class, const uint8_t* d_box_vel_finite, int background_class,
                         float* d_flow, uint8_t* d_flow_is_valid, uint8_t* d_category, uint32_t* d_instance, void* stream);

typedef struct himo_ground_params {
    float sensor_height;
    float r_min;
    float bin_size;
    int32_t n_bins;
    int32_t K;
    float max_slope;
    float step_tol;
    float ground_thresh;
} himo_ground_params;

size_t himo_ground_seg_workspace_bytes(int n_frames, const himo_ground_params* params);
int himo_ground_seg_batch(int n_frames, int64_t total_points, const int64_t* h_offsets, const int64_t* d_offsets,
                          const float* d_xyz, int pitch, const himo_ground_params* params, uint8_t* d_mask,
                          float* d_cell_ground, void* d_workspace, size_t workspace_bytes, void* stream);

typedef struct himo_icp_params {
    float bin;
    int32_t half;
    float z_gate;
    float max_dist;
    int32_t min_inliers;
    float min_ratio;
    int32_t iters;
} himo_icp_params;

#define HIMO_ICP_ACCEPTED 0
#define HIMO_ICP_FAILED 1
#define HIMO_ICP_REJECTED 2
#define HIMO_ICP_MOVED 0
#define HIMO_ICP_FLOW 1

size_t himo_icp_workspace_bytes(int64_t n_target, int n_clusters);
int himo_icp_vote(int64_t n, const float* d_pts, int pitch, int n_clusters, const int64_t* h_offsets, const int64_t* d_offsets,
                  int64_t n_target, const float* d_target, const himo_icp_params* params, int32_t* d_counts, int32_t* d_peak,
                  double* d_transform, int32_t* d_status, void* d_workspace, size_t workspace_bytes, void* stream);
int himo_icp_step(int64_t n, const float* d_moved, int n_clusters, const int64_t* h_offsets, const int64_t* d_offsets,
                  int64_t n_target, const float* d_target, const int32_t* d_nn_idx, const float* d_nn_dist2,
                  const himo_icp_params* params, int final_pass, double* d_transform, int32_t* d_status, uint8_t* d_inlier,
                  void* d_workspace, size_t workspace_bytes, void* stream);
int himo_icp_apply(int64_t n, const float* d_pts, int pitch, const int32_t* d_labels, int n_clusters, const double* d_transform,
                   const int32_t* d_status, int mode, const float* d_base, int base_pitch, float* d_out, void* stream);

size_t himo_pillar_workspace_bytes(int64_t max_points, int grid_w, int grid_h);
int himo_pillarize(int64_t n, const float* d_pts, int pc_stride, const float* h_transform,
                   const float* h_range, const float* h_voxel, const float* h_centre_offset,
                   int grid_w, int grid_h,
                   const float* d_pfn_weight, const float* d_pfn_scale, const float* d_pfn_shift,
                   float* d_xyz_t, int32_t* d_pid, float* d_offsets, float* d_image, int image_pitch,
                   void* d_workspace, size_t workspace_bytes, void* stream);
typedef struct himo_sweep {
    int64_t n; const float* d_pts; int pc_stride;
    float transform[16];
    float* d_xyz_t; int32_t* d_pid; float* d_offsets;
    float* d_image;
    void* d_workspace;
} himo_sweep;
int himo_pillarize_multi(int n_sweeps, const himo_sweep* h_sweeps, const float* h_range, const float* h_voxel,
                         const float* h_centre_offset, int grid_w, int grid_h, const float* d_pfn_weight,
                         const float* d_pfn_scale, const float* d_pfn_shift, int image_pitch, size_t workspace_bytes,
                         void* stream);
#define HIMO_IMAGE_SPLIT 1
#define HIMO_IMAGE_INCREMENTAL 2
int himo_pillar_occupancy_reset(void* d_workspace, size_t workspace_bytes, int grid_w, int grid_h, void* stream);
int himo_pillarize_multi_ex(int n_sweeps, const himo_sweep* h_sweeps, const float* h_range, const float* h_voxel,
                         const float* h_centre_offset, int grid_w, int grid_h, const float* d_pfn_weight,
                         const float* d_pfn_scale, const float* d_pfn_shift, int image_pitch, size_t workspace_bytes, int image_split,
                         void* stream);

#define HIMO_EPI_BIAS 0
#define HIMO_EPI_BIAS_BN_GELU 1
#define HIMO_EPI_BIAS_GELU 2
#define HIMO_EPI_GRU_ZR 3
#define HIMO_EPI_GRU_Q 4
#define HIMO_EPI_BIAS_RELU 5
#define HIMO_EPI_RELU_MASK 6
typedef struct himo_conv_desc {
    const float* x; int64_t x_batch_stride; int x_pitch;
    const float* w;
    const float* bias; const float* scale; const float* shift;
    float* y; int64_t y_batch_stride; int y_pitch;
    int n, h, w_in, cin, cout, ksize, stride, epilogue;
    const float* aux_in; int aux_in_pitch;
    float* aux_out; int aux_out_pitch;
    const void* w_packed;
    int tile_hint;
    int packed_format;
    int n_outer;
    int64_t x_outer_stride, y_outer_stride;
    int act_layout;
    uint32_t* d_range_seen;
} himo_conv_desc;
#define HIMO_ACT_SPLIT_IN 1
#define HIMO_ACT_SPLIT_OUT 2
#define HIMO_ACT_ACCUMULATE 8
#define HIMO_ACT_STUFFED_2X 16
int himo_conv2d(const himo_conv_desc* h_desc, void* stream);
size_t himo_conv_packed_weight_bytes(int ksize, int cin, int cout);
int himo_conv_pack_weights(const float* d_w, int ksize, int cin, int cout, void* d_packed, void* stream);
#define HIMO_PACK_BF16X3 0
#define HIMO_PACK_F16X2 1
#define HIMO_PACK_BF16X2 2
int himo_conv_pack_weights_ex(const float* d_w, int ksize, int cin, int cout, int format, void* d_packed, void* stream);

int himo_upsample2x(const float* d_x, int x_pitch, int h, int w, int c, float* d_y, int y_pitch, void* stream);
int himo_upsample2x_batch(int n, const float* d_x, int64_t x_batch_stride, int x_pitch, int h, int w, int c, float* d_y,
                          int64_t y_batch_stride, int y_pitch, void* stream);
int himo_upsample2x_batch_ex(int n, const float* d_x, int64_t x_batch_stride, int x_pitch, int h, int w, int c, float* d_y,
                             int64_t y_batch_stride, int y_pitch, int out_split, void* stream);

#define HIMO_OP_CONV 0
#define HIMO_OP_UPSAMPLE2X 1
#define HIMO_OPS_GRAPH 0x1u
typedef struct himo_op {
    int kind;
    himo_conv_desc conv;
    const float* up_x; int up_x_pitch, up_h, up_w, up_c;
    float* up_y; int up_y_pitch;
    int up_n; int64_t up_x_batch_stride, up_y_batch_stride;
    int up_out_split;
} himo_op;
int himo_run_ops(const himo_op* h_ops, int n_ops, unsigned flags, void* stream);
void himo_ops_release(const himo_op* h_ops);

int himo_gru_head(int64_t n, const int32_t* d_pid, const float* d_offsets, const float* d_img0, const float* d_img1,
                  int img_pitch, const float* d_dec, int dec_pitch, const float* d_w_off, const float* d_b_off,
                  const void* d_wzr_packed, const float* d_bzr, const void* d_wq_packed, const float* d_bq,
                  const void* d_w1_packed, const float* d_b1, const float* d_w2, const float* d_b2,
                  const float* d_xyz_t, const float* d_pts, int pc_stride, float* d_flow, int iters, int packed_format,
                  void* stream);
typedef struct himo_head_sample {
    int64_t n;
    const int32_t* d_pid; const float* d_offsets; const float* d_img0; const float* d_img1; const float* d_dec;
    const float* d_xyz_t; const float* d_pts; int pc_stride; float* d_flow;
} himo_head_sample;
int himo_gru_head_batch(int n_samples, const himo_head_sample* h_samples, int img_pitch, int dec_pitch,
                        const float* d_w_off, const float* d_b_off,
                        const void* d_wzr_packed, const float* d_bzr, const void* d_wq_packed, const float* d_bq,
                        const void* d_w1_packed, const float* d_b1, const float* d_w2, const float* d_b2,
                        int iters, int packed_format, int img_split, void* stream);
int himo_gru_head_batch_folded(int n_samples, const himo_head_sample* h_samples, int img_pitch, int dec_pitch,
                               const void* d_wzr_packed, const float* d_bzr, const void* d_wq_packed, const float* d_bq,
                               const void* d_w1_packed, const float* d_b1, const float* d_w2, const float* d_b2,
                               int iters, int packed_format, int img_split, void* stream);
int himo_gru_head_batch_guarded(int n_samples, const himo_head_sample* h_samples, int img_pitch, int dec_pitch,
                                const float* d_w_off, const float* d_b_off,
                                const void* d_wzr_packed, const float* d_bzr, const void* d_wq_packed, const float* d_bq,
                                const void* d_w1_packed, const float* d_b1, const float* d_w2, const float* d_b2,
                                int iters, int packed_format, int img_split, uint32_t* d_nonfinite, void* stream);
typedef struct himo_head_saved {
    int64_t rows;
    float* d_hx;
    float* d_rhx;
    float* d_z; float* d_r; float* d_q;
    float* d_pre1; float* d_y1;
    float* d_res;
} himo_head_saved;
int himo_gru_head_train(int64_t n, const int32_t* d_pid, const float* d_offsets, const float* d_img0, const float* d_img1,
                        int img_pitch, const float* d_dec, int dec_pitch, const float* d_w_off, const float* d_b_off,
                        const void* d_wzr_packed, const float* d_bzr, const void* d_wq_packed, const float* d_bq,
                        const void* d_w1_packed, const float* d_b1, const float* d_w2, int w2_pitch, const float* d_b2,
                        int iters, int packed_format, const himo_head_saved* h_saved, uint32_t* d_nonfinite, void* stream);
int himo_gru_head_backward(int64_t n, int iters, const float* d_dhx_last, const himo_head_saved* h_saved,
                           const void* d_wq_t_packed, const void* d_wzr_t_packed, int packed_format, float* d_daq,
                           float* d_dazr, float* d_dhx0, void* stream);
int himo_clear_u32(uint32_t* d_words, int n, void* stream);

int himo_head_gather(int64_t n, const int32_t* d_pid, const float* d_offsets, const float* d_img0,
                     const float* d_img1, int img_pitch, const float* d_dec, int dec_pitch,
                     const float* d_w_off, const float* d_b_off, float* d_hx, float* d_rhx, int pitch, void* stream);
int himo_head_final(int64_t n, const float* d_y1, int y1_pitch, const float* d_w2, const float* d_b2,
                    const int32_t* d_pid, const float* d_xyz_t, const float* d_pts, int pc_stride,
                    float* d_flow, void* stream);

size_t himo_nn_grid_workspace_bytes(int64_t n_max, int grid_w, int grid_h);
int himo_nn_grid(int64_t nq, const float* d_q, int64_t nr, const float* d_r, float x0, float y0, float cell,
                 int grid_w, int grid_h, float* d_dist2, int32_t* d_idx, void* d_workspace,
                 size_t workspace_bytes, void* stream);
size_t himo_ssl_loss_workspace_bytes(int n0, int n1, int n_labels, int grid_w, int grid_h);
int himo_ssl_loss(int n0, int n1, const float* d_pc0, const float* d_pc1, const float* d_flow,
                  const int32_t* d_label0, const int32_t* d_label1, int n_labels,
                  float grid_x0, float grid_y0, float grid_cell, int grid_w, int grid_h,
                  double* d_loss, float* d_grad_flow, void* d_workspace, size_t workspace_bytes, void* stream);
int himo_ssl_loss_ex(int n0, int n1, const float* d_pc0, const float* d_pc1, const float* d_flow,
                     const int32_t* d_label0, const int32_t* d_label1, int n_labels,
                     float grid_x0, float grid_y0, float grid_cell, int grid_w, int grid_h,
                     const float* d_raw_dist2, const int32_t* d_raw_idx,
                     double* d_loss, float* d_grad_flow, void* d_workspace, size_t workspace_bytes, void* stream);
int himo_ssl_dyn_sizes(int n0, const int32_t* d_label0, int n1, const int32_t* d_label1, int32_t* d_counts, void* stream);
int himo_ssl_loss_presized(int n0, int n1, const float* d_pc0, const float* d_pc1, const float* d_flow,
                           const int32_t* d_label0, const int32_t* d_label1, int n_labels,
                           float grid_x0, float grid_y0, float grid_cell, int grid_w, int grid_h,
                           const float* d_raw_dist2, const int32_t* d_raw_idx, int n_dyn0, int n_dyn1,
                           double* d_loss, float* d_grad_flow, void* d_workspace, size_t workspace_bytes, void* stream);

size_t himo_wgrad_workspace_bytes(int64_t n_rows);
int himo_linear_wgrad(int64_t n, const float* d_x, int x_pitch, int cin, const float* d_dz, int z_pitch, int cout,
                      float* d_dw, float* d_db, void* d_workspace, size_t workspace_bytes, void* stream);
size_t himo_wgrad_workspace_bytes_ex(int64_t n_rows, int cin, int cout);
int himo_linear_wgrad_ex(int64_t n, const float* d_x, int x_pitch, int cin, const float* d_dz, int z_pitch, int cout,
                         float* d_dw, float* d_db, unsigned flags, void* d_workspace, size_t workspace_bytes, void* stream);
int himo_transpose(const float* d_w, int rows, int cols, float* d_wt, void* stream);
int himo_adam_step(int64_t n, float* d_param, const float* d_grad, float* d_m, float* d_v, float lr, float beta1,
                   float beta2, float eps, int step, void* stream);
size_t himo_chamfer_trunc_workspace_bytes(int n0, int n1);
int himo_chamfer_trunc(int n0, int n1, const float* d_moved, const float* d_pc1, const float* d_dist_a,
                       const int32_t* d_idx_a, const float* d_dist_b, const int32_t* d_idx_b, float trunc_dist,
                       double* d_loss, float* d_grad_moved, void* d_workspace, size_t workspace_bytes, void* stream);
int himo_rows_add(int64_t n, int cols, const float* d_a, int a_pitch, const float* d_b, int b_pitch, float b_scale,
                  float* d_y, int y_pitch, int zero_tail, void* stream);
int himo_rigid_transform(int64_t n, const float* d_pts, int pc_stride, const float* d_transform, float* d_out,
                         int out_pitch, void* stream);

int himo_gru_gates_fwd(int64_t n, int which, const float* d_pre, const float* d_z_in, const float* d_hx,
                       float* d_z, float* d_r, float* d_q, float* d_out, void* stream);
int himo_gru_bwd1(int64_t n, const float* d_dh_next, const float* d_z, const float* d_q, const float* d_hx,
                  float* d_daq, float* d_dz, float* d_dhp, void* stream);
int himo_gru_bwd2(int64_t n, const float* d_d_rhx, const float* d_hx, const float* d_z, const float* d_r,
                  const float* d_dz, float* d_dhp, float* d_dazr, float* d_dx, void* stream);
int himo_gru_bwd3(int64_t n, const float* d_d_hx, const float* d_dhp, float* d_dh, float* d_dx, void* stream);
int himo_affine_gelu_fwd(int64_t rows, int ch, const float* d_x, int x_pitch, const float* d_scale, const float* d_shift,
                         float* d_pre, int pre_pitch, float* d_y, int y_pitch, void* stream);
int himo_affine_gelu_bwd(int64_t rows, int ch, const float* d_dy, int dy_pitch, const float* d_pre, int pre_pitch,
                         const float* d_scale, float* d_dx, int dx_pitch, void* stream);
int himo_mask_rows(int64_t n, int cols, const int32_t* d_pid, float* d_v, int pitch, void* stream);
int himo_weight_flip(const float* d_w, int ksize, int cin, int cout, float* d_wf, void* stream);
int himo_zero_stuff2x(int n_img, int h, int w, int c, const float* d_dy, int64_t dy_batch_stride, int dy_pitch,
                      float* d_z, int64_t z_batch_stride, int z_pitch, void* stream);
int himo_upsample2x_bwd(const float* d_dy, int dy_pitch, int h, int w, int c, float* d_dx, int dx_pitch, void* stream);
int himo_add2d(int64_t rows, int cols, const float* d_b, int b_pitch, float* d_y, int y_pitch, void* stream);
int himo_colsum(int64_t n, const float* d_z, int z_pitch, int cout, float* d_out, unsigned flags, void* d_workspace,
                size_t workspace_bytes, void* stream);
size_t himo_pfn_backward_workspace_bytes(void);
int himo_pfn_backward(int64_t n, const float* h_voxel, const float* h_centre_offset, int grid_w, int grid_h,
                      const float* d_pfn_weight, const float* d_pfn_scale, const float* d_pfn_shift,
                      const float* d_xyz_t, const void* d_pillar_workspace, const float* d_dimage, int image_pitch,
                      float* d_dweight, unsigned flags, void* d_workspace, size_t workspace_bytes, void* stream);
int himo_head_scatter(int64_t n, int grid_w, int grid_h, const void* d_pillar_workspace, const float* d_dhx, int dhx_pitch,
                      float* d_db0, int b0_pitch, int group0, int group1, int n_groups, float* d_ddec, int dec_pitch,
                      void* stream);

typedef struct himo_weight_job {
    const float* w;
    void* packed;
    int ksize, cin, cout;
    int format;
    int flip;
    int first_block;
} himo_weight_job;
int himo_weight_job_blocks(int ksize, int cin, int cout, int flip);
int himo_weight_prepare_batch(const himo_weight_job* d_jobs, int n_jobs, int total_blocks, void* stream);

int himo_mlp_repack(int n_layers, const float* const* h_w, const int* h_cin, const int* h_cout, void* const* h_fwd_packed,
                    void* const* h_bwd_packed, void* stream);

size_t himo_dbscan_workspace_bytes(int n, int grid_w, int grid_h);
int himo_dbscan(int n, const float* d_xyz, int pitch, const unsigned char* d_skip, float eps, int min_pts, float x0, float y0, float cell,
                int grid_w, int grid_h, int32_t* d_labels, int32_t* d_n_clusters, void* d_workspace, size_t workspace_bytes, void* stream);

int64_t himo_nsf_padded_rows(int64_t n);
size_t himo_nsf_spill_bytes(int64_t n, int n_hidden);
int himo_nsf_backward_blocks(int64_t n);
int himo_nsf_forward(int64_t n, const float* d_x0, int n_hidden, const float* d_w_first, const float* d_b_first,
                     const void* const* h_w_hidden_packed, const float* const* h_b_hidden, const float* d_w_last, const float* d_b_last,
                     void* d_spill, float* d_out, const float* h_origin, float cell, const int* h_dims, int window, const void* d_volume,
                     float trunc_dist, float* d_dout, double* d_loss_partial, int* d_count_partial, void* stream);
int himo_nsf_backward(int64_t n, const float* d_x0, const float* d_dout, int n_hidden, const void* const* h_wT_hidden_packed,
                      const float* d_w_last, const void* d_spill, const int* h_off_w, const int* h_off_b, int64_t partial_stride,
                      float* d_partial, void* stream);
int himo_nsf_update(int total, int n_partials, int64_t partial_stride, const float* d_partial, int n_fwd_blocks,
                    const double* d_loss_partial, const int* d_count_partial, float* d_param, float* d_grad, float* d_m, float* d_v,
                    float lr, float beta1, float beta2, float eps, int step, int n_hidden, const int* h_off_w, void* const* h_fwd_packed,
                    void* const* h_bwd_packed, double* d_loss, int* d_count, void* stream);

int himo_mlp_forward_fused(int64_t n, const float* d_x0, int n_hidden, const float* d_w_first, const float* d_b_first,
                           const void* const* h_w_hidden_packed, const float* const* h_b_hidden, const float* d_w_last,
                           const float* d_b_last, float* const* h_H, float* d_out, void* stream);
int himo_mlp_backward_fused(int64_t n, const float* d_dout, int n_hidden, const void* const* h_wT_hidden_packed,
                            const float* d_w_last, float* const* h_H, float* const* h_dZ, void* stream);
size_t himo_mlp_bias_workspace_bytes(int64_t n, int n_hidden);
int himo_mlp_backward_fused_bias(int64_t n, const float* d_dout, int n_hidden, const void* const* h_wT_hidden_packed,
                                 const float* d_w_last, float* const* h_H, float* const* h_dZ, float* const* h_db,
                                 void* d_workspace, size_t workspace_bytes, void* stream);

size_t himo_dt_volume_bytes(const int* h_dims);
int himo_dt_build(int n1, const float* d_pc1, const float* h_origin, float cell, const int* h_dims, int window,
                  void* d_volume, size_t volume_bytes, void* stream);
size_t himo_dt_loss_workspace_bytes(int n);
int himo_dt_loss(int n, const float* d_moved, const float* h_origin, float cell, const int* h_dims, int window,
                 const void* d_volume, float trunc_dist, double* d_loss, float* d_grad_moved, void* d_workspace,
                 size_t workspace_bytes, void* stream);

size_t himo_bn_workspace_bytes(int64_t total_rows, int ch);
int himo_bn_train_fwd(int n_img, int64_t rows, int ch, const float* d_x, int64_t x_img_stride, int x_pitch,
                      const float* d_gamma, const float* d_beta, float eps, float momentum, float* d_running_mean,
                      float* d_running_var, float* d_mean, float* d_invstd, float* d_xhat, int64_t xhat_img_stride, int xhat_pitch,
                      float* d_y, int64_t y_img_stride, int y_pitch, void* d_workspace, size_t workspace_bytes, void* stream);
int himo_bn_train_bwd(int n_img, int64_t rows, int ch, const float* d_dy, int64_t dy_img_stride, int dy_pitch,
                      const float* d_xhat, int64_t xhat_img_stride, int xhat_pitch, const float* d_gamma, const float* d_beta,
                      const float* d_invstd, float* d_dx, int64_t dx_img_stride, int dx_pitch, float* d_dgamma, float* d_dbeta,
                      unsigned flags, void* d_workspace, size_t workspace_bytes, void* stream);
int himo_bn_train_bwd_x(int n_img, int64_t rows, int ch, const float* d_dy, int64_t dy_img_stride, int dy_pitch,
                        const float* d_x, int64_t x_img_stride, int x_pitch, const float* d_gamma, const float* d_beta,
                        const float* d_mean, const float* d_invstd, float* d_dx, int64_t dx_img_stride, int dx_pitch,
                        float* d_dgamma, float* d_dbeta, unsigned flags, void* d_workspace, size_t workspace_bytes, void* stream);
int himo_bn_fold(int ch, const float* d_gamma, const float* d_beta, const float* d_mean, const float* d_var, float eps,
                 float* d_scale, float* d_shift, void* stream);
size_t himo_pfn_bn_workspace_bytes(void);
int himo_pfn_bn_stats_groups(int n_sweeps, int n_groups, const int64_t* h_n, const float* const* h_xyz_t,
                             const void* const* h_pillar_workspace, const float* h_voxel, const float* h_centre_offset, int grid_w,
                             int grid_h, const float* d_pfn_weight, const float* d_gamma, const float* d_beta, float eps, float momentum,
                             float* d_running_mean, float* d_running_var, float* d_scale, float* d_shift, float* d_mean, float* d_invstd,
                             void* d_workspace, size_t workspace_bytes, void* stream);
int himo_pfn_backward_bn_groups(int n_sweeps, int n_groups, const int64_t* h_n, const float* const* h_xyz_t,
                                const void* const* h_pillar_workspace, const float* const* h_dimage, int image_pitch, const float* h_voxel,
                                const float* h_centre_offset, int grid_w, int grid_h, const float* d_pfn_weight, const float* d_scale,
                                const float* d_shift, const float* d_mean, const float* d_invstd, float* d_dweight, float* d_dgamma,
                                float* d_dbeta, unsigned flags, void* d_workspace, size_t workspace_bytes, void* stream);
int himo_pfn_bn_stats_multi(int n_sweeps, const int64_t* h_n, const float* const* h_xyz_t, const void* const* h_pillar_workspace,
                            const float* h_voxel, const float* h_centre_offset, int grid_w, int grid_h,
                            const float* d_pfn_weight, const float* d_gamma, const float* d_beta, float eps, float momentum,
                            float* d_running_mean, float* d_running_var, float* d_scale, float* d_shift, float* d_mean,
                            float* d_invstd, void* d_workspace, size_t workspace_bytes, void* stream);
int himo_pfn_backward_bn_multi(int n_sweeps, const int64_t* h_n, const float* const* h_xyz_t, const void* const* h_pillar_workspace,
                               const float* const* h_dimage, int image_pitch, const float* h_voxel, const float* h_centre_offset,
                               int grid_w, int grid_h, const float* d_pfn_weight, const float* d_scale, const float* d_shift,
                               const float* d_mean, const float* d_invstd, float* d_dweight, float* d_dgamma, float* d_dbeta,
                               unsigned flags, void* d_workspace, size_t workspace_bytes, void* stream);
int himo_pfn_bn_stats(int64_t n, const float* h_voxel, const float* h_centre_offset, int grid_w, int grid_h,
                      const float* d_pfn_weight, const float* d_xyz_t, const void* d_pillar_workspace, const float* d_gamma,
                      const float* d_beta, float eps, float momentum, float* d_running_mean, float* d_running_var,
                      float* d_scale, float* d_shift, float* d_mean, float* d_invstd, void* d_workspace, size_t workspace_bytes,
                      void* stream);
int himo_pillar_features_multi(int n_sweeps, const himo_sweep* h_sweeps, const float* h_range, const float* h_voxel,
                               const float* h_centre_offset, int grid_w, int grid_h, const float* d_pfn_weight,
                               const float* d_scale, const float* d_shift, int image_pitch, size_t workspace_bytes,
                               int image_split, void* stream);
int himo_pfn_backward_bn(int64_t n, const float* h_voxel, const float* h_centre_offset, int grid_w, int grid_h,
                         const float* d_pfn_weight, const float* d_scale, const float* d_shift, const float* d_mean,
                         const float* d_invstd, const float* d_xyz_t, const void* d_pillar_workspace, const float* d_dimage,
                         int image_pitch, float* d_dweight, float* d_dgamma, float* d_dbeta, unsigned flags, void* d_workspace,
                         size_t workspace_bytes, void* stream);
size_t himo_conv_wgrad_batch_workspace_bytes(int n_img, int h, int w, int cin, int cout, int stride);
int himo_conv3x3_wgrad_batch(int n_img, const float* d_x, int64_t x_batch_stride, int x_pitch, int h, int w, int cin,
                             const float* d_dy, int64_t dy_batch_stride, int dy_pitch, int cout, int stride, float* d_dw,
                             unsigned flags, void* d_workspace, size_t workspace_bytes, void* stream);
int himo_conv3x3_wgrad_batch_bias(int n_img, const float* d_x, int64_t x_batch_stride, int x_pitch, int h, int w, int cin,
                                  const float* d_dy, int64_t dy_batch_stride, int dy_pitch, int cout, int stride, float* d_dw,
                                  float* d_db, unsigned flags, void* d_workspace, size_t workspace_bytes, void* stream);
size_t himo_conv_wgrad_workspace_bytes(int ho, int wo, int cin, int cout);
int himo_conv3x3_wgrad(const float* d_x, int x_pitch, int h, int w, int cin, const float* d_dy, int dy_pitch, int cout,
                       int stride, float* d_dw, unsigned flags, void* d_workspace, size_t workspace_bytes, void* stream);

int64_t himo_lz4_frame_decompress(const void* h_src, int64_t n, void* h_dst, int64_t capacity);

#ifdef __cplusplus
}
#endif
#endif
```

Before: 755.9 frames/s.

## Compact pillar launch args to batch 24 sweeps and specialise small cells

Splits the per-sweep pillar argument struct into shared grid/PFN fields plus a slim per-sweep record holding one workspace base pointer, so up to 24 sweeps fit in one launch's argument segment. This halves the number of pillarisation launch groups when many frames are in flight (16 samples x 3 sweeps). The feature kernel also prefetches the next cell's records, adds a register sorting-network path for cells with 2-4 points, and replaces the inverse-rank search with a ds_permute push. The cost is more register pressure and branches in the feature kernel, plus a new wide-group flag that the Python callers now always set.

Result: no change. 748.5 frames/s (-1.0%).

```diff
diff --git a/himo_amd/csrc/pillar.hip b/himo_amd/csrc/pillar.hip
--- a/himo_amd/csrc/pillar.hip
+++ b/himo_amd/csrc/pillar.hip
@@ -13,37 +13,47 @@
     int W, H;
 };
 
-struct PillarArgs {
-    int64_t n;
-    const float* pts; int stride;
-    float R[9], t[3];
+struct PillarShared {
     GridSpec g;
+    int image_pitch;
+    int image_split;
+    int const_stride;
     const float* pfn_w;
     const float* pfn_scale;
     const float* pfn_shift;
+    int off_block_sum, off_cell_rec;
+    int64_t off_occ;
+};
+
+struct PillarSweep {
+    int n, stride;
+    const float* pts;
+    float R[9], t[3];
     float* xyz_t;
     int* pid;
     float* offsets;
-    float* image; int image_pitch;
-    int image_split;
-    int* cell_count;
-    int* block_sum;
-    int* cell_cursor;
+    float* image;
+    char* ws;
     int* order2;
-    float4* cell_rec;
-    unsigned long long* occ;
 };
 
-constexpr int kMaxSweeps = 12;
-struct PillarBatch { PillarArgs s[kMaxSweeps]; };
+constexpr int kMaxSweeps = 24;
+constexpr int kBaseSweeps = 12;
+struct PillarBatch { PillarShared h; PillarSweep s[kMaxSweeps]; };
+static_assert(sizeof(PillarBatch) <= 3072, "the launch's arguments must stay well inside the 4 KB kernel-argument segment");
+
+__device__ inline int* sweep_cell_count(const PillarSweep& a) { return reinterpret_cast<int*>(a.ws); }
+__device__ inline int* sweep_block_sum(const PillarShared& h, const PillarSweep& a) { return reinterpret_cast<int*>(a.ws + h.off_block_sum); }
+__device__ inline float4* sweep_cell_rec(const PillarShared& h, const PillarSweep& a) { return reinterpret_cast<float4*>(a.ws + h.off_cell_rec); }
 
 __global__ __launch_bounds__(256) void pillar_clear_kernel(PillarBatch m, int n_vec4) {
-    int4* p = reinterpret_cast<int4*>(m.s[blockIdx.y].cell_count);
+    int4* p = reinterpret_cast<int4*>(m.s[blockIdx.y].ws);
     for (int i = blockIdx.x * 256 + threadIdx.x; i < n_vec4; i += gridDim.x * 256) p[i] = make_int4(0, 0, 0, 0);
 }
 
 __global__ __launch_bounds__(256) void pillar_assign_kernel(PillarBatch m) {
-    const PillarArgs& a = m.s[blockIdx.y];
+    const PillarShared& h = m.h;
+    const PillarSweep& a = m.s[blockIdx.y];
     const int64_t i = (int64_t)blockIdx.x * 256 + threadIdx.x;
     if (i >= a.n) return;
     const float* p = a.pts + i * a.stride;
@@ -52,14 +62,14 @@
     const float ty = ((x * a.R[3] + y * a.R[4]) + z * a.R[5]) + a.t[1];
     const float tz = ((x * a.R[6] + y * a.R[7]) + z * a.R[8]) + a.t[2];
     a.xyz_t[i * 3] = tx; a.xyz_t[i * 3 + 1] = ty; a.xyz_t[i * 3 + 2] = tz;
-    const float fx = floorf((tx - a.g.xmin) / a.g.vx);
-    const float fy = floorf((ty - a.g.ymin) / a.g.vy);
-    const float fz = floorf((tz - a.g.zmin) / a.g.vz);
-    const bool ok = fx >= 0.f && fx < (float)a.g.W && fy >= 0.f && fy < (float)a.g.H && fz >= 0.f && fz < 1.f;
+    const float fx = floorf((tx - h.g.xmin) / h.g.vx);
+    const float fy = floorf((ty - h.g.ymin) / h.g.vy);
+    const float fz = floorf((tz - h.g.zmin) / h.g.vz);
+    const bool ok = fx >= 0.f && fx < (float)h.g.W && fy >= 0.f && fy < (float)h.g.H && fz >= 0.f && fz < 1.f;
     int cell = -1;
     if (ok) {
-        cell = (int)fy * a.g.W + (int)fx;
-        a.order2[i] = atomicAdd(&a.cell_count[cell], 1);
+        cell = (int)fy * h.g.W + (int)fx;
+        a.order2[i] = atomicAdd(&sweep_cell_count(a)[cell], 1);
     } else {
         a.offsets[i * 3] = 0.f; a.offsets[i * 3 + 1] = 0.f; a.offsets[i * 3 + 2] = 0.f;
     }
@@ -69,9 +79,9 @@
 constexpr int kScanBlock = 1024;
 
 __global__ __launch_bounds__(256) void cell_scan_local_kernel(PillarBatch m) {
-    int* v = m.s[blockIdx.y].cell_count;
-    int* block_sum = m.s[blockIdx.y].block_sum;
-    const int n = m.s[blockIdx.y].g.W * m.s[blockIdx.y].g.H;
+    int* v = sweep_cell_count(m.s[blockIdx.y]);
+    int* block_sum = sweep_block_sum(m.h, m.s[blockIdx.y]);
+    const int n = m.h.g.W * m.h.g.H;
     __shared__ int wsum[4];
     const int base = blockIdx.x * kScanBlock + threadIdx.x * 4;
     int x[4];
@@ -94,7 +104,7 @@
 }
 
 __global__ __launch_bounds__(1024) void cell_scan_top_kernel(PillarBatch m, int nblk) {
-    int* block_sum = m.s[blockIdx.y].block_sum;
+    int* block_sum = sweep_block_sum(m.h, m.s[blockIdx.y]);
     __shared__ int part[1024];
     const int x = (int)threadIdx.x < nblk ? block_sum[threadIdx.x] : 0;
     part[threadIdx.x] = x;
@@ -109,22 +119,20 @@
     if (threadIdx.x == 1023) block_sum[nblk] = part[1023];
 }
 
-__device__ inline int cell_offset(const PillarArgs& a, int cell);
-
-__device__ inline int cell_offset(const PillarArgs& a, int cell) {
-    const int n_cells = a.g.W * a.g.H;
-    return cell >= n_cells ? a.block_sum[(n_cells + kScanBlock - 1) / kScanBlock]
-                           : a.cell_count[cell] + a.block_sum[cell / kScanBlock];
+__device__ inline int cell_offset(const int* cell_count, const int* block_sum, int n_cells, int cell) {
+    return cell >= n_cells ? block_sum[(n_cells + kScanBlock - 1) / kScanBlock]
+                           : cell_count[cell] + block_sum[cell / kScanBlock];
 }
 
 __global__ __launch_bounds__(256) void pillar_fill_kernel(PillarBatch m) {
-    const PillarArgs& a = m.s[blockIdx.y];
+    const PillarShared& h = m.h;
+    const PillarSweep& a = m.s[blockIdx.y];
     const int64_t i = (int64_t)blockIdx.x * 256 + threadIdx.x;
     if (i >= a.n) return;
     const int cell = a.pid[i];
     if (cell < 0) return;
-    const int at = cell_offset(a, cell) + a.order2[i];
-    a.cell_rec[at] = make_float4(a.xyz_t[i * 3], a.xyz_t[i * 3 + 1], a.xyz_t[i * 3 + 2], __int_as_float((int)i));
+    const int at = cell_offset(sweep_cell_count(a), sweep_block_sum(h, a), h.g.W * h.g.H, cell) + a.order2[i];
+    sweep_cell_rec(h, a)[at] = make_float4(a.xyz_t[i * 3], a.xyz_t[i * 3 + 1], a.xyz_t[i * 3 + 2], __int_as_float((int)i));
 }
 
 constexpr int kCellsPerBlock = 8;
@@ -133,18 +141,37 @@
 
 __device__ inline float shfl32(float v, int src) { return __shfl(v, src, 32); }
 __device__ inline int shfl32(int v, int src) { return __shfl(v, src, 32); }
+__device__ inline int push32(int v, int dst) {
+    return __builtin_amdgcn_ds_permute((int)(((threadIdx.x & 32u) + (unsigned)dst) << 2), v);
+}
+__device__ inline float push32(float v, int dst) { return __int_as_float(push32(__float_as_int(v), dst)); }
+
+struct CellPoint { float x, y, z; int idx; };
+__device__ inline void order_pair(CellPoint& p, CellPoint& q) {
+    const bool sw = q.idx < p.idx;
+    const CellPoint lo = {sw ? q.x : p.x, sw ? q.y : p.y, sw ? q.z : p.z, sw ? q.idx : p.idx};
+    const CellPoint hi = {sw ? p.x : q.x, sw ? p.y : q.y, sw ? p.z : q.z, sw ? p.idx : q.idx};
+    p = lo; q = hi;
+}
 
 __global__ __launch_bounds__(256) void pillar_feature_kernel(PillarBatch m) {
-    const PillarArgs& a = m.s[blockIdx.y];
+    const PillarShared& h = m.h;
+    const PillarSweep& a = m.s[blockIdx.y];
     __shared__ int s_beg[kFeatCells + 1];
     __shared__ int s_list[kFeatCells];
     __shared__ int s_nlist;
     const int sub = threadIdx.x >> 5, c = threadIdx.x & 31;
-    const int n_cells = a.g.W * a.g.H;
+    const int W = h.g.W;
+    const int n_cells = W * h.g.H;
     const int cell0 = blockIdx.x * kFeatCells;
     static_assert(kFeatCells == 64, "one 64-bit occupancy word per block");
-    const unsigned long long was = a.occ ? a.occ[blockIdx.x] : ~0ull;
-    if (threadIdx.x <= kFeatCells) s_beg[threadIdx.x] = cell_offset(a, min(cell0 + (int)threadIdx.x, n_cells));
+    const int* cell_count = sweep_cell_count(a);
+    const int* block_sum = sweep_block_sum(h, a);
+    const float4* cell_rec = sweep_cell_rec(h, a);
+    unsigned long long* occ = h.off_occ >= 0 ? reinterpret_cast<unsigned long long*>(a.ws + h.off_occ) : nullptr;
+    const int image_pitch = h.image_pitch;
+    const unsigned long long was = occ ? occ[blockIdx.x] : ~0ull;
+    if (threadIdx.x <= kFeatCells) s_beg[threadIdx.x] = cell_offset(cell_count, block_sum, n_cells, min(cell0 + (int)threadIdx.x, n_cells));
     __syncthreads();
     if (threadIdx.x < 64) {
         const int cnt = cell0 + (int)threadIdx.x < n_cells ? s_beg[threadIdx.x + 1] - s_beg[threadIdx.x] : 0;
@@ -152,35 +179,61 @@
         const unsigned long long below = (1ull << threadIdx.x) - 1ull;
         if (cnt == 1) s_list[__popcll(one & below)] = threadIdx.x;
         if (cnt > 1) s_list[__popcll(one) + __popcll(many & below)] = threadIdx.x;
-        if (threadIdx.x == 0) { s_nlist = __popcll(one | many); if (a.occ) a.occ[blockIdx.x] = one | many; }
+        if (threadIdx.x == 0) { s_nlist = __popcll(one | many); if (occ) occ[blockIdx.x] = one | many; }
     }
 #pragma unroll
     for (int i = 0; i < kFeatCells / 32; ++i) {
         const int lc = i * 32 + (threadIdx.x >> 3);
         if (cell0 + lc < n_cells && s_beg[lc + 1] == s_beg[lc] && ((was >> lc) & 1ull))
-            *reinterpret_cast<float4*>(a.image + (int64_t)(cell0 + lc) * a.image_pitch + (threadIdx.x & 7) * 4) = make_float4(0.f, 0.f, 0.f, 0.f);
+            *reinterpret_cast<float4*>(a.image + (int64_t)(cell0 + lc) * image_pitch + (threadIdx.x & 7) * 4) = make_float4(0.f, 0.f, 0.f, 0.f);
     }
     __syncthreads();
     const int nlist = s_nlist;
+    if (sub >= nlist) return;
     float w[9];
 #pragma unroll
-    for (int k = 0; k < 9; ++k) w[k] = a.pfn_w[k * 32 + c];
-    const float scale = a.pfn_scale[c], shift = a.pfn_shift[c];
-
+    for (int k = 0; k < 9; ++k) w[k] = h.pfn_w[k * 32 + c];
+    const float scale = h.pfn_scale[blockIdx.y * h.const_stride + c], shift = h.pfn_shift[blockIdx.y * h.const_stride + c];
+    const int iy0 = cell0 / W, ix0 = cell0 - iy0 * W;
+    const float vx = h.g.vx, vy = h.g.vy, cx0 = h.g.cx0, cy0 = h.g.cy0;
+    const float ccz = 0.f * h.g.vz + h.g.cz0;
+
+    int lc = s_list[sub], beg = s_beg[lc], cnt = s_beg[lc + 1] - beg;
+    float4 r[4] = {};
+    r[0] = cell_rec[beg];
+#pragma unroll
+    for (int j = 1; j < 4; ++j)
+        if (j < cnt && cnt <= 4) r[j] = cell_rec[beg + j];
     for (int k = sub; k < nlist; k += kCellsPerBlock) {
-        const int lc = s_list[k];
         const int cell = cell0 + lc;
-        const int beg = s_beg[lc];
-        const int cnt = s_beg[lc + 1] - beg;
-        const int iy = cell / a.g.W, ix = cell - iy * a.g.W;
-        const float ccx = (float)ix * a.g.vx + a.g.cx0, ccy = (float)iy * a.g.vy + a.g.cy0, ccz = 0.f * a.g.vz + a.g.cz0;
-        const float fc = (float)cnt;
+        const int cur_beg = beg, cur_cnt = cnt;
+        CellPoint p[4];
+#pragma unroll
+        for (int j = 0; j < 4; ++j) {
+            const bool have = j < cur_cnt;
+            p[j].x = have ? r[j].x : 0.f; p[j].y = have ? r[j].y : 0.f; p[j].z = have ? r[j].z : 0.f;
+            p[j].idx = have ? __float_as_int(r[j].w) : 0x7fffffff;
+        }
+        if (k + kCellsPerBlock < nlist) {
+            lc = s_list[k + kCellsPerBlock]; beg = s_beg[lc]; cnt = s_beg[lc + 1] - beg;
+            r[0] = cell_rec[beg];
+#pragma unroll
+            for (int j = 1; j < 4; ++j)
+                if (j < cnt && cnt <= 4) r[j] = cell_rec[beg + j];
+        }
+        int ix = ix0 + (cell - cell0), iy = iy0;
+        if (W >= kFeatCells) {
+            if (ix >= W) { ix -= W; ++iy; }
+        } else {
+            iy = cell / W; ix = cell - iy * W;
+        }
+        const float ccx = (float)ix * vx + cx0, ccy = (float)iy * vy + cy0;
+        const float fc = (float)cur_cnt;
         float acc = 0.f;
-        if (cnt == 1) {
-            const float4 rc = a.cell_rec[beg];
-            const int pj = __float_as_int(rc.w);
-            const float x = rc.x, y = rc.y, z = rc.z;
-            if (c == 0) a.order2[beg] = pj;
+        if (cur_cnt == 1) {
+            const int pj = p[0].idx;
+            const float x = p[0].x, y = p[0].y, z = p[0].z;
+            if (c == 0) a.order2[cur_beg] = pj;
             const float f6[3] = {x - ccx, y - ccy, z - ccz};
             float v = x * w[0];
             v = fmaf(y, w[1], v); v = fmaf(z, w[2], v);
@@ -189,23 +242,40 @@
             v = v * scale + shift;
             acc = 0.f + fmaxf(v, 0.f);
             if (c < 3) a.offsets[(int64_t)pj * 3 + c] = f6[c];
-        } else if (cnt <= 32) {
-            const bool have = c < cnt;
-            const float4 rc = a.cell_rec[beg + (have ? c : 0)];
+        } else if (cur_cnt <= 4) {
+            order_pair(p[0], p[1]); order_pair(p[2], p[3]); order_pair(p[0], p[2]); order_pair(p[1], p[3]); order_pair(p[1], p[2]);
+            if (c < cur_cnt) a.order2[cur_beg + c] = c == 0 ? p[0].idx : c == 1 ? p[1].idx : c == 2 ? p[2].idx : p[3].idx;
+            float sx = 0.f, sy = 0.f, sz = 0.f;
+#pragma unroll
+            for (int j = 0; j < 4; ++j) { sx += p[j].x; sy += p[j].y; sz += p[j].z; }
+            const float mx = sx / fc, my = sy / fc, mz = sz / fc;
+#pragma unroll
+            for (int j = 0; j < 4; ++j) {
+                if (j < cur_cnt) {
+                    const float x = p[j].x, y = p[j].y, z = p[j].z;
+                    const float f[9] = {x, y, z, x - mx, y - my, z - mz, x - ccx, y - ccy, z - ccz};
+                    float v = f[0] * w[0];
+#pragma unroll
+                    for (int q = 1; q < 9; ++q) v = fmaf(f[q], w[q], v);
+                    v = v * scale + shift;
+                    acc += fmaxf(v, 0.f);
+                    if (c < 3) a.offsets[(int64_t)p[j].idx * 3 + c] = c == 0 ? f[6] : c == 1 ? f[7] : f[8];
+                }
+            }
+        } else if (cur_cnt <= 32) {
+            const bool have = c < cur_cnt;
+            const float4 rc = cell_rec[cur_beg + (have ? c : 0)];
             const int idx = have ? __float_as_int(rc.w) : 0x7fffffff;
-            const float ux = rc.x, uy = rc.y, uz = rc.z;
             int rank = 0;
-            for (int j = 0; j < cnt; ++j) rank += shfl32(idx, j) < idx;
-            int src = 0;
-            for (int j = 0; j < cnt; ++j)
-                if (shfl32(rank, j) == c) src = j;
-            const int sidx = shfl32(idx, src);
-            const float px = shfl32(ux, src), py = shfl32(uy, src), pz = shfl32(uz, src);
-            if (have) a.order2[beg + c] = sidx;
+            for (int j = 0; j < cur_cnt; ++j) rank += shfl32(idx, j) < idx;
+            rank &= 31;
+            const int sidx = push32(idx, rank);
+            const float px = push32(rc.x, rank), py = push32(rc.y, rank), pz = push32(rc.z, rank);
+            if (have) a.order2[cur_beg + c] = sidx;
             float sx = 0.f, sy = 0.f, sz = 0.f;
-            for (int j = 0; j < cnt; ++j) { sx += shfl32(px, j); sy += shfl32(py, j); sz += shfl32(pz, j); }
+            for (int j = 0; j < cur_cnt; ++j) { sx += shfl32(px, j); sy += shfl32(py, j); sz += shfl32(pz, j); }
             const float mx = sx / fc, my = sy / fc, mz = sz / fc;
-            for (int j = 0; j < cnt; ++j) {
+            for (int j = 0; j < cur_cnt; ++j) {
                 const float x = shfl32(px, j), y = shfl32(py, j), z = shfl32(pz, j);
                 const int pj = shfl32(sidx, j);
                 const float f[9] = {x, y, z, x - mx, y - my, z - mz, x - ccx, y - ccy, z - ccz};
@@ -217,40 +287,40 @@
                 if (c < 3) a.offsets[(int64_t)pj * 3 + c] = f[6 + c];
             }
         } else {
-            for (int j0 = 0; j0 < cnt; j0 += 32) {
-                const bool have = j0 + c < cnt;
-                const int idx = have ? __float_as_int(a.cell_rec[beg + j0 + c].w) : 0x7fffffff;
+            for (int j0 = 0; j0 < cur_cnt; j0 += 32) {
+                const bool have = j0 + c < cur_cnt;
+                const int idx = have ? __float_as_int(cell_rec[cur_beg + j0 + c].w) : 0x7fffffff;
                 int rank = 0;
-                for (int k0 = 0; k0 < cnt; k0 += 32) {
-                    const int other = k0 + c < cnt ? __float_as_int(a.cell_rec[beg + k0 + c].w) : 0x7fffffff;
-                    const int lim = min(32, cnt - k0);
+                for (int k0 = 0; k0 < cur_cnt; k0 += 32) {
+                    const int other = k0 + c < cur_cnt ? __float_as_int(cell_rec[cur_beg + k0 + c].w) : 0x7fffffff;
+                    const int lim = min(32, cur_cnt - k0);
                     for (int j = 0; j < lim; ++j) rank += shfl32(other, j) < idx;
                 }
-                if (have) a.order2[beg + rank] = idx;
+                if (have) a.order2[cur_beg + rank] = idx;
             }
             __threadfence_block();
             float sx = 0.f, sy = 0.f, sz = 0.f;
-            for (int j0 = 0; j0 < cnt; j0 += 32) {
-                const bool have = j0 + c < cnt;
-                const float* p = a.xyz_t + (int64_t)(have ? a.order2[beg + j0 + c] : 0) * 3;
-                const float ux = have ? p[0] : 0.f, uy = have ? p[1] : 0.f, uz = have ? p[2] : 0.f;
-                const int lim = min(32, cnt - j0);
+            for (int j0 = 0; j0 < cur_cnt; j0 += 32) {
+                const bool have = j0 + c < cur_cnt;
+                const float* q = a.xyz_t + (int64_t)(have ? a.order2[cur_beg + j0 + c] : 0) * 3;
+                const float ux = have ? q[0] : 0.f, uy = have ? q[1] : 0.f, uz = have ? q[2] : 0.f;
+                const int lim = min(32, cur_cnt - j0);
                 for (int j = 0; j < lim; ++j) { sx += shfl32(ux, j); sy += shfl32(uy, j); sz += shfl32(uz, j); }
             }
             const float mx = sx / fc, my = sy / fc, mz = sz / fc;
-            for (int j0 = 0; j0 < cnt; j0 += 32) {
-                const bool have = j0 + c < cnt;
-                const int pidx = have ? a.order2[beg + j0 + c] : 0;
-                const float* p = a.xyz_t + (int64_t)pidx * 3;
-                const float ux = have ? p[0] : 0.f, uy = have ? p[1] : 0.f, uz = have ? p[2] : 0.f;
-                const int lim = min(32, cnt - j0);
+            for (int j0 = 0; j0 < cur_cnt; j0 += 32) {
+                const bool have = j0 + c < cur_cnt;
+                const int pidx = have ? a.order2[cur_beg + j0 + c] : 0;
+                const float* q = a.xyz_t + (int64_t)pidx * 3;
+                const float ux = have ? q[0] : 0.f, uy = have ? q[1] : 0.f, uz = have ? q[2] : 0.f;
+                const int lim = min(32, cur_cnt - j0);
                 for (int j = 0; j < lim; ++j) {
                     const float x = shfl32(ux, j), y = shfl32(uy, j), z = shfl32(uz, j);
                     const int pj = shfl32(pidx, j);
                     const float f[9] = {x, y, z, x - mx, y - my, z - mz, x - ccx, y - ccy, z - ccz};
                     float v = f[0] * w[0];
 #pragma unroll
-                    for (int q = 1; q < 9; ++q) v = fmaf(f[q], w[q], v);
+                    for (int q2 = 1; q2 < 9; ++q2) v = fmaf(f[q2], w[q2], v);
                     v = v * scale + shift;
                     acc += fmaxf(v, 0.f);
                     if (c < 3) a.offsets[(int64_t)pj * 3 + c] = f[6 + c];
@@ -258,15 +328,15 @@
             }
         }
         const float feat = acc / fc;
-        if (a.image_split) {
-            unsigned h, l;
-            split2_rounded(feat, h, l);
+        if (h.image_split) {
+            unsigned hi, lo;
+            split2_rounded(feat, hi, lo);
             const bool odd = c & 1;
-            const unsigned recv = (unsigned)__builtin_amdgcn_mov_dpp((int)(odd ? h : l), 0xB1, 0xF, 0xF, true);
-            unsigned* rec = reinterpret_cast<unsigned*>(a.image + (int64_t)cell * a.image_pitch + (c & ~15));
-            rec[(odd ? 8 : 0) + ((c & 15) >> 1)] = odd ? (recv | (l << 16)) : (h | (recv << 16));
+            const unsigned recv = (unsigned)__builtin_amdgcn_mov_dpp((int)(odd ? hi : lo), 0xB1, 0xF, 0xF, true);
+            unsigned* rec = reinterpret_cast<unsigned*>(a.image + (int64_t)cell * image_pitch + (c & ~15));
+            rec[(odd ? 8 : 0) + ((c & 15) >> 1)] = odd ? (recv | (lo << 16)) : (hi | (recv << 16));
         } else {
-            a.image[(int64_t)cell * a.image_pitch + c] = feat;
+            a.image[(int64_t)cell * image_pitch + c] = feat;
         }
     }
 }
@@ -320,7 +390,8 @@
     const float* coef;
 };
 
-struct PfnBnBatch { PfnBnArgs s[kMaxSweeps]; };
+constexpr int kMaxWalkSweeps = 12;
+struct PfnBnBatch { PfnBnArgs s[kMaxWalkSweeps]; };
 template <int KIND>
 __global__ __launch_bounds__(256) void pfn_walk_kernel(PfnBnBatch m) {
     const PfnBnArgs& p = m.s[blockIdx.y];
@@ -546,7 +617,24 @@
     return HIMO_OK;
 }
 
-static int pillar_args(PillarArgs& a, int64_t n, const float* d_pts, int pc_stride, const float* h_transform, const float* h_range,
+static int pillar_shared(PillarShared& h, int64_t nmax, const float* h_range, const float* h_voxel, const float* h_centre_offset, int grid_w,
+                         int grid_h, const float* d_pfn_weight, const float* d_pfn_scale, const float* d_pfn_shift, int image_pitch,
+                         size_t workspace_bytes, bool incremental) {
+    h = PillarShared{};
+    h.g.xmin = h_range[0]; h.g.ymin = h_range[1]; h.g.zmin = h_range[2];
+    h.g.vx = h_voxel[0]; h.g.vy = h_voxel[1]; h.g.vz = h_voxel[2];
+    h.g.cx0 = h_centre_offset[0]; h.g.cy0 = h_centre_offset[1]; h.g.cz0 = h_centre_offset[2];
+    h.g.W = grid_w; h.g.H = grid_h;
+    h.pfn_w = d_pfn_weight; h.pfn_scale = d_pfn_scale; h.pfn_shift = d_pfn_shift;
+    h.image_pitch = image_pitch;
+    const int cells = (int)grid_cells(grid_w, grid_h);
+    h.off_block_sum = (int)(2 * ws_cells(cells));
+    h.off_cell_rec = (int)(2 * ws_cells(cells) + ws_blocks(cells));
+    h.off_occ = incremental ? (int64_t)(workspace_bytes - ws_occ(cells)) : -1;
+    return HIMO_OK;
+}
+
+static int pillar_args(PillarSweep& a, int64_t n, const float* d_pts, int pc_stride, const float* h_transform, const float* h_range,
                        const float* h_voxel, const float* h_centre_offset, int grid_w, int grid_h, const float* d_pfn_weight,
                        const float* d_pfn_scale, const float* d_pfn_shift, float* d_xyz_t, int32_t* d_pid, float* d_offsets,
                        float* d_image, int image_pitch, void* d_workspace, size_t workspace_bytes, bool incremental = false) {
@@ -560,28 +648,18 @@
     const int cells = (int)grid_cells(grid_w, grid_h);
     if (workspace_bytes < pillar_ws(n, cells) || !aligned16(d_workspace)) return HIMO_ERR_WORKSPACE;
     if (incremental && ((workspace_bytes & 15) || workspace_bytes < pillar_ws(n, cells) + ws_occ(cells))) return HIMO_ERR_WORKSPACE;
-    a = PillarArgs{};
-    a.n = n; a.pts = d_pts; a.stride = pc_stride;
+    a = PillarSweep{};
+    a.n = (int)n; a.pts = d_pts; a.stride = pc_stride;
     for (int i = 0; i < 9; ++i) a.R[i] = h_transform[(i / 3) * 4 + (i % 3)];
     for (int i = 0; i < 3; ++i) a.t[i] = h_transform[i * 4 + 3];
-    a.g.xmin = h_range[0]; a.g.ymin = h_range[1]; a.g.zmin = h_range[2];
-    a.g.vx = h_voxel[0]; a.g.vy = h_voxel[1]; a.g.vz = h_voxel[2];
-    a.g.cx0 = h_centre_offset[0]; a.g.cy0 = h_centre_offset[1]; a.g.cz0 = h_centre_offset[2];
-    a.g.W = grid_w; a.g.H = grid_h;
-    a.pfn_w = d_pfn_weight; a.pfn_scale = d_pfn_scale; a.pfn_shift = d_pfn_shift;
-    a.xyz_t = d_xyz_t; a.pid = d_pid; a.offsets = d_offsets; a.image = d_image; a.image_pitch = image_pitch;
-    char* ws = reinterpret_cast<char*>(d_workspace);
-    a.cell_count = reinterpret_cast<int*>(ws);
-    a.cell_cursor = reinterpret_cast<int*>(ws + ws_cells(cells));
-    a.block_sum = reinterpret_cast<int*>(ws + 2 * ws_cells(cells));
-    a.cell_rec = reinterpret_cast<float4*>(ws + 2 * ws_cells(cells) + ws_blocks(cells));
-    a.order2 = reinterpret_cast<int*>(ws + 2 * ws_cells(cells) + ws_blocks(cells) + 4 * ws_points(n));
-    if (incremental) a.occ = reinterpret_cast<unsigned long long*>(ws + (workspace_bytes - ws_occ(cells)));
-    return HIMO_OK;
-}
-
-static int sweeps_status(int n_sweeps, const himo_sweep* h_sweeps, int image_pitch, int image_split, bool check_shared) {
-    if (n_sweeps < 1 || n_sweeps > kMaxSweeps || !h_sweeps) return HIMO_ERR_INVALID_ARGUMENT;
+    a.xyz_t = d_xyz_t; a.pid = d_pid; a.offsets = d_offsets; a.image = d_image;
+    a.ws = reinterpret_cast<char*>(d_workspace);
+    a.order2 = reinterpret_cast<int*>(a.ws + 2 * ws_cells(cells) + ws_blocks(cells) + 4 * ws_points(n));
+    return HIMO_OK;
+}
+
+static int sweeps_status(int n_sweeps, const himo_sweep* h_sweeps, int image_pitch, int image_split, bool check_shared, bool wide) {
+    if (n_sweeps < 1 || n_sweeps > (wide ? kMaxSweeps : kBaseSweeps) || !h_sweeps) return HIMO_ERR_INVALID_ARGUMENT;
     if (image_split && (image_pitch & 15)) return HIMO_ERR_INVALID_ARGUMENT;
     for (int i = 0; i < n_sweeps; ++i) {
         if (image_split && (reinterpret_cast<uintptr_t>(h_sweeps[i].d_image) & 63)) return HIMO_ERR_INVALID_ARGUMENT;
@@ -591,8 +669,10 @@
     return HIMO_OK;
 }
 
+extern "C" int himo_pillar_max_sweeps(void) { return kMaxSweeps; }
+
 static int pillar_launch(const PillarBatch& m, int count, hipStream_t s) {
-    const int cells = m.s[0].g.W * m.s[0].g.H;
+    const int cells = m.h.g.W * m.h.g.H;
     const int nblk = (cells + kScanBlock - 1) / kScanBlock;
     int64_t nmax = 0;
     for (int i = 0; i < count; ++i)
@@ -637,6 +717,8 @@
     const int st = pillar_args(m.s[0], n, d_pts, pc_stride, h_transform, h_range, h_voxel, h_centre_offset, grid_w, grid_h, d_pfn_weight,
                                d_pfn_scale, d_pfn_shift, d_xyz_t, d_pid, d_offsets, d_image, image_pitch, d_workspace, workspace_bytes);
     if (st != HIMO_OK) return st;
+    pillar_shared(m.h, n, h_range, h_voxel, h_centre_offset, grid_w, grid_h, d_pfn_weight, d_pfn_scale, d_pfn_shift, image_pitch,
+                  workspace_bytes, false);
     return pillar_launch(m, 1, (hipStream_t)stream);
 }
 
@@ -648,23 +730,37 @@
                                    d_pfn_shift, image_pitch, workspace_bytes, 0, stream);
 }
 
-extern "C" int himo_pillarize_multi_ex(int n_sweeps, const himo_sweep* h_sweeps, const float* h_range, const float* h_voxel,
-                                       const float* h_centre_offset, int grid_w, int grid_h, const float* d_pfn_weight,
-                                       const float* d_pfn_scale, const float* d_pfn_shift, int image_pitch, size_t workspace_bytes,
-                                       int image_split, void* stream) {
-    const bool incremental = (image_split & 2) != 0;
-    image_split &= 1;
-    const int st0 = sweeps_status(n_sweeps, h_sweeps, image_pitch, image_split, true);
-    if (st0 != HIMO_OK) return st0;
-    PillarBatch m{};
+static int pillar_batch(PillarBatch& m, int n_sweeps, const himo_sweep* h_sweeps, const float* h_range, const float* h_voxel,
+                        const float* h_centre_offset, int grid_w, int grid_h, const float* d_pfn_weight, const float* d_pfn_scale,
+                        const float* d_pfn_shift, int const_stride, int image_pitch, size_t workspace_bytes, int image_split,
+                        bool incremental) {
     for (int i = 0; i < n_sweeps; ++i) {
         const himo_sweep& w = h_sweeps[i];
         const int st = pillar_args(m.s[i], w.n, w.d_pts, w.pc_stride, w.transform, h_range, h_voxel, h_centre_offset, grid_w, grid_h,
                                    d_pfn_weight, d_pfn_scale, d_pfn_shift, w.d_xyz_t, w.d_pid, w.d_offsets, w.d_image, image_pitch,
                                    w.d_workspace, workspace_bytes, incremental);
         if (st != HIMO_OK) return st;
-        m.s[i].image_split = image_split ? 1 : 0;
-    }
+    }
+    pillar_shared(m.h, 0, h_range, h_voxel, h_centre_offset, grid_w, grid_h, d_pfn_weight, d_pfn_scale, d_pfn_shift, image_pitch,
+                  workspace_bytes, incremental);
+    m.h.image_split = image_split ? 1 : 0;
+    m.h.const_stride = const_stride;
+    return HIMO_OK;
+}
+
+extern "C" int himo_pillarize_multi_ex(int n_sweeps, const himo_sweep* h_sweeps, const float* h_range, const float* h_voxel,
+                                       const float* h_centre_offset, int grid_w, int grid_h, const float* d_pfn_weight,
+                                       const float* d_pfn_scale, const float* d_pfn_shift, int image_pitch, size_t workspace_bytes,
+                                       int image_split, void* stream) {
+    const bool incremental = (image_split & 2) != 0;
+    const bool wide = (image_split & 4) != 0;
+    image_split &= 1;
+    const int st0 = sweeps_status(n_sweeps, h_sweeps, image_pitch, image_split, true, wide);
+    if (st0 != HIMO_OK) return st0;
+    PillarBatch m{};
+    const int st = pillar_batch(m, n_sweeps, h_sweeps, h_range, h_voxel, h_centre_offset, grid_w, grid_h, d_pfn_weight, d_pfn_scale,
+                                d_pfn_shift, 0, image_pitch, workspace_bytes, image_split, incremental);
+    if (st != HIMO_OK) return st;
     return pillar_launch(m, n_sweeps, (hipStream_t)stream);
 }
 
@@ -744,11 +840,11 @@
     if (!d_gamma || !d_beta || !d_scale || !d_shift || !d_mean || !d_invstd || (d_running_mean == nullptr) != (d_running_var == nullptr))
         return HIMO_ERR_INVALID_ARGUMENT;
     if (grid_w < 1 || grid_h < 1) return HIMO_ERR_INVALID_ARGUMENT;
-    if (n_groups > kMaxSweeps * kMaxGroup || grid_status(grid_w, grid_h) != HIMO_OK) return HIMO_ERR_UNSUPPORTED;
+    if (n_groups > kMaxWalkSweeps * kMaxGroup || grid_status(grid_w, grid_h) != HIMO_OK) return HIMO_ERR_UNSUPPORTED;
     const size_t one = himo_pfn_bn_workspace_bytes();
     if (workspace_bytes < one * n_sweeps) return HIMO_ERR_WORKSPACE;
     std::vector<PfnBnArgs> args((size_t)n_sweeps);
-    PfnGroup groups[kMaxSweeps * kMaxGroup];
+    PfnGroup groups[kMaxWalkSweeps * kMaxGroup];
     for (int g = 0; g < n_groups; ++g) groups[g].n = 0;
     for (int i = 0; i < n_sweeps; ++i) {
         const int st = pfn_bn_args(args[i], h_n[i], h_voxel, h_centre_offset, grid_w, grid_h, d_pfn_weight, h_xyz_t[i], h_pillar_workspace[i],
@@ -759,8 +855,8 @@
     }
     hipStream_t s = (hipStream_t)stream;
     ProfScope ps("pfn_bn_stats_kernel", s);
-    for (int lo = 0; lo < n_sweeps; lo += kMaxSweeps) {
-        const int cnt = n_sweeps - lo < kMaxSweeps ? n_sweeps - lo : kMaxSweeps;
+    for (int lo = 0; lo < n_sweeps; lo += kMaxWalkSweeps) {
+        const int cnt = n_sweeps - lo < kMaxWalkSweeps ? n_sweeps - lo : kMaxWalkSweeps;
         PfnBnBatch m{};
         for (int j = 0; j < cnt; ++j) m.s[j] = args[lo + j];
         hipLaunchKernelGGL(pfn_walk_kernel<0>, dim3(kPfnBwdBlocks, cnt), dim3(256), 0, s, m);
@@ -777,7 +873,7 @@
                                        const float* d_pfn_weight, const float* d_gamma, const float* d_beta, float eps, float momentum,
                                        float* d_running_mean, float* d_running_var, float* d_scale, float* d_shift, float* d_mean,
                                        float* d_invstd, void* d_workspace, size_t workspace_bytes, void* stream) {
-    if (n_sweeps > kMaxSweeps) return HIMO_ERR_INVALID_ARGUMENT;
+    if (n_sweeps > kMaxWalkSweeps) return HIMO_ERR_INVALID_ARGUMENT;
     return himo_pfn_bn_stats_groups(n_sweeps, n_sweeps, h_n, h_xyz_t, h_pillar_workspace, h_voxel, h_centre_offset, grid_w, grid_h, d_pfn_weight,
                                     d_gamma, d_beta, eps, momentum, d_running_mean, d_running_var, d_scale, d_shift, d_mean, d_invstd,
                                     d_workspace, workspace_bytes, stream);
@@ -798,19 +894,15 @@
                                           const float* d_scale, const float* d_shift, int image_pitch, size_t workspace_bytes,
                                           int image_split, void* stream) {
     const bool incremental = (image_split & 2) != 0;
+    const bool wide = (image_split & 4) != 0;
     image_split &= 1;
     if (!d_scale || !d_shift) return HIMO_ERR_INVALID_ARGUMENT;
-    const int st0 = sweeps_status(n_sweeps, h_sweeps, image_pitch, image_split, false);
+    const int st0 = sweeps_status(n_sweeps, h_sweeps, image_pitch, image_split, false, wide);
     if (st0 != HIMO_OK) return st0;
     PillarBatch m{};
-    for (int i = 0; i < n_sweeps; ++i) {
-        const himo_sweep& w = h_sweeps[i];
-        const int st = pillar_args(m.s[i], w.n, w.d_pts, w.pc_stride, w.transform, h_range, h_voxel, h_centre_offset, grid_w, grid_h,
-                                   d_pfn_weight, d_scale + 32 * i, d_shift + 32 * i, w.d_xyz_t, w.d_pid, w.d_offsets, w.d_image, image_pitch,
-                                   w.d_workspace, workspace_bytes, incremental);
-        if (st != HIMO_OK) return st;
-        m.s[i].image_split = image_split ? 1 : 0;
-    }
+    const int st = pillar_batch(m, n_sweeps, h_sweeps, h_range, h_voxel, h_centre_offset, grid_w, grid_h, d_pfn_weight, d_scale, d_shift, 32,
+                                image_pitch, workspace_bytes, image_split, incremental);
+    if (st != HIMO_OK) return st;
     hipStream_t s = (hipStream_t)stream;
     const int cells = grid_w * grid_h;
     {
@@ -827,16 +919,16 @@
                                            const float* d_scale, const float* d_shift, const float* d_mean, const float* d_invstd,
                                            float* d_dweight, float* d_dgamma, float* d_dbeta, unsigned flags, void* d_workspace,
                                            size_t workspace_bytes, void* stream) {
-    if (n_sweeps < 1 || n_groups < 1 || n_sweeps % n_groups || n_sweeps / n_groups > kMaxGroup || n_groups > kMaxSweeps * kMaxGroup ||
-        n_sweeps > kMaxSweeps * kMaxGroup || !h_n || !h_xyz_t || !h_pillar_workspace || !h_dimage)
+    if (n_sweeps < 1 || n_groups < 1 || n_sweeps % n_groups || n_sweeps / n_groups > kMaxGroup || n_groups > kMaxWalkSweeps * kMaxGroup ||
+        n_sweeps > kMaxWalkSweeps * kMaxGroup || !h_n || !h_xyz_t || !h_pillar_workspace || !h_dimage)
         return HIMO_ERR_INVALID_ARGUMENT;
     if (!d_scale || !d_shift || !d_mean || !d_invstd || !d_dweight || !d_dgamma || !d_dbeta || image_pitch < 32) return HIMO_ERR_INVALID_ARGUMENT;
     if (grid_w < 1 || grid_h < 1) return HIMO_ERR_INVALID_ARGUMENT;
     if (grid_status(grid_w, grid_h) != HIMO_OK) return HIMO_ERR_UNSUPPORTED;
     const size_t one = himo_pfn_bn_workspace_bytes();
     if (workspace_bytes < one * n_sweeps) return HIMO_ERR_WORKSPACE;
-    static thread_local PfnBnArgs args[kMaxSweeps * kMaxGroup];
-    PfnGroup groups[kMaxSweeps * kMaxGroup];
+    static thread_local PfnBnArgs args[kMaxWalkSweeps * kMaxGroup];
+    PfnGroup groups[kMaxWalkSweeps * kMaxGroup];
     for (int g = 0; g < n_groups; ++g) groups[g].n = 0;
     for (int i = 0; i < n_sweeps; ++i) {
         if (!h_dimage[i]) return HIMO_ERR_INVALID_ARGUMENT;
@@ -854,8 +946,8 @@
     hipStream_t s = (hipStream_t)stream;
     ProfScope ps("pfn_backward_kernel", s);
     auto walk = [&](auto kernel) {
-        for (int lo = 0; lo < n_sweeps; lo += kMaxSweeps) {
-            const int cnt = n_sweeps - lo < kMaxSweeps ? n_sweeps - lo : kMaxSweeps;
+        for (int lo = 0; lo < n_sweeps; lo += kMaxWalkSweeps) {
+            const int cnt = n_sweeps - lo < kMaxWalkSweeps ? n_sweeps - lo : kMaxWalkSweeps;
             PfnBnBatch m{};
             for (int j = 0; j < cnt; ++j) m.s[j] = args[lo + j];
             hipLaunchKernelGGL(kernel, dim3(kPfnBwdBlocks, cnt), dim3(256), 0, s, m);
@@ -881,7 +973,7 @@
                                           int grid_w, int grid_h, const float* d_pfn_weight, const float* d_scale, const float* d_shift,
                                           const float* d_mean, const float* d_invstd, float* d_dweight, float* d_dgamma, float* d_dbeta,
                                           unsigned flags, void* d_workspace, size_t workspace_bytes, void* stream) {
-    if (n_sweeps > kMaxSweeps) return HIMO_ERR_INVALID_ARGUMENT;
+    if (n_sweeps > kMaxWalkSweeps) return HIMO_ERR_INVALID_ARGUMENT;
     return himo_pfn_backward_bn_groups(n_sweeps, n_sweeps, h_n, h_xyz_t, h_pillar_workspace, h_dimage, image_pitch, h_voxel, h_centre_offset,
                                        grid_w, grid_h, d_pfn_weight, d_scale, d_shift, d_mean, d_invstd, d_dweight, d_dgamma, d_dbeta, flags,
                                        d_workspace, workspace_bytes, stream);
diff --git a/himo_amd/seflow/model.py b/himo_amd/seflow/model.py
--- a/himo_amd/seflow/model.py
+++ b/himo_amd/seflow/model.py
@@ -27,10 +27,12 @@
 ACT_SPLIT_IN, ACT_SPLIT_OUT = 1, 2
 ACT_ACCUMULATE = 8
 ACT_STUFFED_2X = 16
+IMAGE_WIDE_GROUP = 4
 
 
 _lib.register({
     "himo_pillar_workspace_bytes": (ctypes.c_size_t, [ctypes.c_int64, ctypes.c_int, ctypes.c_int]),
+    "himo_pillar_max_sweeps": (ctypes.c_int, []),
     "himo_pillar_occupancy_reset": (ctypes.c_int, [ctypes.c_void_p, ctypes.c_size_t, ctypes.c_int, ctypes.c_int, ctypes.c_void_p]),
     "himo_pillarize": (ctypes.c_int, [ctypes.c_int64, ctypes.c_void_p, ctypes.c_int, ctypes.POINTER(ctypes.c_float),
                                       ctypes.POINTER(ctypes.c_float), ctypes.POINTER(ctypes.c_float),
@@ -547,7 +549,9 @@
     def pillarize_all(self, sweeps, transforms):
         self.pillarize_many([(self._sample, sweeps, transforms)])
 
-    MAX_SWEEPS = 12
+    @property
+    def MAX_SWEEPS(self) -> int:
+        return int(self.lib.himo_pillar_max_sweeps())
 
     def pillarize_many(self, jobs):
         for _, sweeps, _ in jobs:
@@ -569,7 +573,8 @@
             status = self.lib.himo_pillarize_multi_ex(len(arr), ctypes.addressof(arr), self._range, self._voxel, self._centre, self.W, self.H,
                                                       self.p["pfn.weight"].data_ptr(), self.p["pfn.scale"].data_ptr(),
                                                       self.p["pfn.shift"].data_ptr(), 32 * self.F, self._pt[0]["ws_slots"][0].numel(),
-                                                      (1 if self.split_acts else 0) | (2 if self.incremental_images else 0), _lib.stream_handle())
+                                                      (1 if self.split_acts else 0) | (2 if self.incremental_images else 0) | IMAGE_WIDE_GROUP,
+                                                      _lib.stream_handle())
             _lib.check(status, "himo_pillarize_multi_ex")
 
     def pillar_features(self, sweeps, transforms, scale: torch.Tensor, shift: torch.Tensor):
diff --git a/himo_amd/seflow/train.py b/himo_amd/seflow/train.py
--- a/himo_amd/seflow/train.py
+++ b/himo_amd/seflow/train.py
@@ -768,10 +768,10 @@
 
     def _pillar_stage(self, jobs, constants=None):
         net, lib, F = self.net, self.lib, self.net.F
-        from .model import HimoSweep, _f32x
+        from .model import HimoSweep, IMAGE_WIDE_GROUP, _f32x
         pitch = 32 * F * self.B
         flat = [(b, slot, pts, T) for b, sweeps, transforms in jobs for slot, (pts, T) in enumerate(zip(sweeps, transforms))]
-        flags = (1 if net.split_acts else 0) | (2 if net.incremental_images else 0)
+        flags = (1 if net.split_acts else 0) | (2 if net.incremental_images else 0) | IMAGE_WIDE_GROUP
         for lo in range(0, len(flat), net.MAX_SWEEPS):
             grp = flat[lo:lo + net.MAX_SWEEPS]
             arr = (HimoSweep * len(grp))()
diff --git a/include/himo_amd.h b/include/himo_amd.h
--- a/include/himo_amd.h
+++ b/include/himo_amd.h
@@ -186,6 +186,8 @@
                          void* stream);
 #define HIMO_IMAGE_SPLIT 1
 #define HIMO_IMAGE_INCREMENTAL 2
+#define HIMO_PILLAR_WIDE_GROUP 4
+int himo_pillar_max_sweeps(void);
 int himo_pillar_occupancy_reset(void* d_workspace, size_t workspace_bytes, int grid_w, int grid_h, void* stream);
 int himo_pillarize_multi_ex(int n_sweeps, const himo_sweep* h_sweeps, const float* h_range, const float* h_voxel,
                          const float* h_centre_offset, int grid_w, int grid_h, const float* d_pfn_weight,
```
